# jzebedee/deltaq

Hardware: AMD Instinct MI355X
Metric: MB of text suffix-sorted per second (bit-exact SA) (higher is better)
Workload: dtype u8 text / u64 keys / int32 SA; 1 GPU; 256 MiB uniform-random bytes per GPU (splitmix64 seed 0x5EED0003+rank), int32 SA; bytes_per_gpu=268435456, residency=text and SA resident in HBM, rounds_after_initial_sort=1

## Files before the change

### deltaq_amd/csrc/dq_flags.h

```cpp
#pragma once

#include <algorithm>
#include <cstdint>
#include <cstdlib>
#include <cstring>
#include <optional>
#include <string>

namespace dq {

struct Flags {
    bool debug = false;
    std::optional<int> trace;
    std::optional<int> hip_device;
    std::optional<int> numa_bind;
    std::optional<std::string> fault;
    std::optional<int> small_n;
    std::optional<int> no_many;
    std::optional<int> mid_many_min;
    std::optional<int> no_large_many;
    std::optional<int> large_many_min;
    std::optional<int> no_diff_many;
    std::optional<int> no_diff_mid_many;
    std::optional<int> diff_mid_many_min;
    std::optional<int> no_diff_large;
    std::optional<int> diff_large_min;
    std::optional<int> diff_large_table;
    std::optional<int> no_index_many;
    std::optional<int> index_many_min;
    std::optional<int> index_many_threads;
    std::optional<int> no_index_large;
    std::optional<int> index_large_min;
    std::optional<int> no_check_many;
    std::optional<int> no_bwt_many;
    std::optional<int> no_mtf_many;
    std::optional<int> no_huff_many;
    std::optional<int> mtf_short_max;
    std::optional<int> unbz2_one_start;
    bool no_list_buffers = false;
    bool text_copy = false;
    bool assume_doubled = false;
    bool no_twins = false;
    bool no_period_hint = false;
    std::optional<int> xcd_group;
    std::optional<int> packed;
    std::optional<int> key_bytes;
    std::optional<int> coded;
    std::optional<int> split;
    bool no_bucket = false;
    std::optional<int> bucket;
    std::optional<int> bucket_keybits;
    std::optional<int> bucket_ext;
    std::optional<int> bucket_tile;
    std::optional<int> bucket_slots;
    std::optional<int> slot_finish;
    std::optional<int> tie_settle;
    std::optional<int> status_zero;
    std::optional<int> hist_loads;
    bool old_first_pass = false;
    bool no_fused_ties = false;
    std::optional<int> sparse;
    std::optional<int> binned_isa;
    bool no_binned_isa = false;
    std::optional<int> runs;
    bool no_small = false;
    bool no_wide_small = false;
    bool no_first_small = false;
    std::optional<int> mid_groups;
    bool no_l_shift = false;
    bool no_upd_words = false;
    std::optional<int> upd_bin;
    std::optional<int> upd_bin_min;
    std::optional<int> upd_window;
    std::optional<int> chain_steps;
    bool no_chain = false;
    bool force_rshift = false;
    std::optional<int> tail_max;
    std::optional<int> pair_chains;
    std::optional<int> pair_chains_min;
    std::optional<int> pair_maxg;
    std::optional<int> late_runs_min;
    bool no_late_runs = false;
    std::optional<int> run_period;
    bool search_wave = false;
    std::optional<int> search_ptab;
    bool no_wave_windows = false;
    bool no_poll = false;
    bool no_second_stage = false;
    std::optional<int> win_min;
    std::optional<int> win_second;
    std::optional<int> walk_on;
    bool no_resume = false;
    std::optional<int> scan_device;
    std::optional<int> scan_groups;
    std::optional<int> scan_groups_cap;
    std::optional<int> scan_chains;
    std::optional<int64_t> scan_min_seg;
    std::optional<int64_t> scan_extra;
    std::optional<int64_t> scan_lane_budget;
    std::optional<int> scan_poll_sleep;
    std::optional<int> scan_spin_log2;
    std::optional<int> scan_slow_group;
    std::optional<int> scan_par_emit;
    std::optional<int64_t> frame_follow_min;
    bool frame_after = false;
};

inline Flags read_flags()
{
    auto on = [](const char *name) { return getenv(name) != nullptr; };
    auto num = [](const char *name, int lo = INT32_MIN, int hi = INT32_MAX) -> std::optional<int> {
        const char *v = getenv(name);
        if (!v) return std::nullopt;
        return std::max(lo, std::min(hi, atoi(v)));
    };
    auto num64 = [](const char *name, int64_t lo) -> std::optional<int64_t> {
        const char *v = getenv(name);
        if (!v) return std::nullopt;
        return std::max<int64_t>(lo, atoll(v));
    };
    Flags f;
    const char *gate = getenv("DQ_DEBUG_FLAGS");
    f.debug = gate && atoi(gate) != 0;
    f.trace = num("DQ_TRACE");
    f.hip_device = num("DQ_HIP_DEVICE");
    f.numa_bind = num("DQ_NUMA_BIND");
    if (!f.debug) return f;

    if (const char *v = getenv("DQ_FAULT")) f.fault = v;
    f.small_n = num("DQ_SMALL_N", 0);
    f.no_many = num("DQ_NO_MANY", 0, 15);
    f.mid_many_min = num("DQ_MID_MANY_MIN", 1);
    f.no_large_many = num("DQ_NO_LARGE_MANY", 0, 1);
    f.large_many_min = num("DQ_LARGE_MANY_MIN", 1);
    f.no_diff_many = num("DQ_NO_DIFF_MANY", 0, 1);
    f.no_diff_mid_many = num("DQ_NO_DIFF_MID_MANY", 0, 1);
    f.diff_mid_many_min = num("DQ_DIFF_MID_MANY_MIN", 1);
    f.no_diff_large = num("DQ_NO_DIFF_LARGE", 0, 1);
    f.diff_large_min = num("DQ_DIFF_LARGE_MIN", 1);
    f.diff_large_table = num("DQ_DIFF_LARGE_TABLE", 0, 1);
    f.no_index_many = num("DQ_NO_INDEX_MANY", 0, 1);
    f.index_many_min = num("DQ_INDEX_MANY_MIN", 1);
    f.index_many_threads = num("DQ_INDEX_MANY_THREADS");
    f.no_index_large = num("DQ_NO_INDEX_LARGE", 0, 1);
    f.index_large_min = num("DQ_INDEX_LARGE_MIN", 1);
    f.no_check_many = num("DQ_NO_CHECK_MANY", 0, 1);
    f.no_bwt_many = num("DQ_NO_BWT_MANY", 0, 1);
    f.no_mtf_many = num("DQ_NO_MTF_MANY", 0, 1);
    f.no_huff_many = num("DQ_NO_HUFF_MANY", 0, 1);
    f.mtf_short_max = num("DQ_MTF_SHORT_MAX", 0);
    f.unbz2_one_start = num("DQ_UNBZ2_ONE_START", 0, 1);
    f.no_list_buffers = on("DQ_NO_LIST_BUFFERS");
    f.text_copy = on("DQ_TEXT_COPY");
    f.assume_doubled = on("DQ_ASSUME_DOUBLED");
    f.no_twins = on("DQ_NO_TWINS");
    f.no_period_hint = on("DQ_NO_PERIOD_HINT");

    f.xcd_group = num("DQ_XCD_GROUP", 0, 64);
    f.packed = num("DQ_PACKED");
    f.key_bytes = num("DQ_KEY_BYTES", 1, 8);
    f.coded = num("DQ_CODED");
    f.split = num("DQ_SPLIT");
    f.no_bucket = on("DQ_NO_BUCKET");
    f.bucket = num("DQ_BUCKET");
    f.bucket_keybits = num("DQ_BUCKET_KEYBITS");
    f.bucket_ext = num("DQ_BUCKET_EXT");
    f.bucket_tile = num("DQ_BUCKET_TILE", 0, 1);
    f.bucket_slots = num("DQ_BUCKET_SLOTS", 0, 1);
    f.slot_finish = num("DQ_SLOT_FINISH", 0, 1);
    f.tie_settle = num("DQ_TIE_SETTLE", 0, 1);
    f.status_zero = num("DQ_STATUS_ZERO", 0, 1);
    f.hist_loads = num("DQ_HIST_LOADS", 1, 4);
    f.old_first_pass = on("DQ_OLD_FIRST_PASS");
    f.no_fused_ties = on("DQ_NO_FUSED_TIES");
    f.sparse = num("DQ_SPARSE");
    f.binned_isa = num("DQ_BINNED_ISA");
    f.no_binned_isa = on("DQ_NO_BINNED_ISA");
    f.runs = num("DQ_RUNS");

    f.no_small = on("DQ_NO_SMALL");
    f.no_wide_small = on("DQ_NO_WIDE_SMALL");
    f.no_first_small = on("DQ_NO_FIRST_SMALL");
    f.mid_groups = num("DQ_MID_GROUPS");
    f.no_l_shift = on("DQ_NO_L_SHIFT");
    f.no_upd_words = on("DQ_NO_UPD_WORDS");
    f.upd_bin = num("DQ_UPD_BIN", 0, 2);
    f.upd_bin_min = num("DQ_UPD_BIN_MIN", 1);
    f.upd_window = num("DQ_UPD_WINDOW");
    f.chain_steps = num("DQ_CHAIN_STEPS");
    f.no_chain = on("DQ_NO_CHAIN");
    f.force_rshift = on("DQ_FORCE_RSHIFT");

    f.tail_max = num("DQ_TAIL_MAX", 0);
    f.pair_chains = num("DQ_PAIR_CHAINS");
    f.pair_chains_min = num("DQ_PAIR_CHAINS_MIN", 1);
    f.pair_maxg = num("DQ_PAIR_MAXG", 2);
    f.late_runs_min = num("DQ_LATE_RUNS_MIN", 1);
    f.no_late_runs = on("DQ_NO_LATE_RUNS");
    f.run_period = num("DQ_RUN_PERIOD", 1);

    f.search_wave = on("DQ_SEARCH_WAVE");
    f.search_ptab = num("DQ_SEARCH_PTAB");
    f.no_wave_windows = on("DQ_NO_WAVE_WINDOWS");
    f.no_poll = on("DQ_NO_POLL");
    f.no_second_stage = on("DQ_NO_SECOND_STAGE");
    f.win_min = num("DQ_WIN_MIN", 16);
    f.win_second = num("DQ_WIN_SECOND", 16);
    f.walk_on = num("DQ_WALK_ON");
    f.no_resume = on("DQ_NO_RESUME");

    f.scan_device = num("DQ_SCAN_DEVICE");
    f.scan_groups = num("DQ_SCAN_GROUPS", 8);
    f.scan_groups_cap = num("DQ_SCAN_GROUPS_CAP", 0);
    f.scan_chains = num("DQ_SCAN_CHAINS", 1);
    f.scan_min_seg = num64("DQ_SCAN_MIN_SEG", 64);
    f.scan_extra = num64("DQ_SCAN_EXTRA", 1);
    f.scan_lane_budget = num64("DQ_SCAN_LANE_BUDGET", 1);
    f.scan_poll_sleep = num("DQ_SCAN_POLL_SLEEP", 1, 32);
    f.scan_spin_log2 = num("DQ_SCAN_SPIN_LOG2", 1, 24);
    f.scan_slow_group = num("DQ_SCAN_SLOW_GROUP", 0, 255);
    f.scan_par_emit = num("DQ_SCAN_PAR_EMIT");
    f.frame_follow_min = num64("DQ_FRAME_FOLLOW_MIN", INT64_MIN);
    f.frame_after = on("DQ_FRAME_AFTER");
    return f;
}

struct FaultPlan {
    int alloc_at = 0, hip_at = 0;
    int alloc_seen = 0, hip_seen = 0;
    bool spin = false;
};
inline thread_local FaultPlan t_fault;

inline FaultPlan parse_fault(const std::optional<std::string> &spec)
{
    FaultPlan p;
    if (!spec) return p;
    const char *f = spec->c_str();
    if (strncmp(f, "alloc:", 6) == 0) p.alloc_at = std::max(1, atoi(f + 6));
    else if (strncmp(f, "hip:", 4) == 0) p.hip_at = std::max(1, atoi(f + 4));
    else if (strcmp(f, "spin") == 0) p.spin = true;
    return p;
}

struct FlagState {
    Flags snap;
    int depth = 0;
};
inline thread_local FlagState t_flags;

struct EnvScope {
    EnvScope()
    {
        if (t_flags.depth++ != 0) return;
        t_flags.snap = read_flags();
        t_fault = parse_fault(t_flags.snap.fault);
    }
    explicit EnvScope(const Flags &adopt)
    {
        if (t_flags.depth++ == 0) t_flags.snap = adopt;
    }
    ~EnvScope() { if (--t_flags.depth == 0) t_fault = FaultPlan{}; }
    EnvScope(const EnvScope &) = delete;
    EnvScope &operator=(const EnvScope &) = delete;
};

inline const Flags &flags()
{
    if (t_flags.depth == 0) t_flags.snap = read_flags();
    return t_flags.snap;
}

template <typename Fn>
auto with_flags(Fn fn)
{
    return [snap = flags(), fn = std::move(fn)](auto &&...args) mutable {
        EnvScope scope(snap);
        return fn(std::forward<decltype(args)>(args)...);
    };
}

}
```

### deltaq_amd/csrc/dq_onesweep.h

```cpp
#pragma once
#include "dq_coded_keys.h"
#include "dq_radix.h"
#include "dq_round0_plan.h"

namespace dq {

constexpr int kHistBlocks = 512;
constexpr int kHistThreads = 1024;
constexpr int kMaxPasses = 8;


template <int kPasses>
__global__ __launch_bounds__(kHistThreads) void radix_hist_kernel(const uint64_t *__restrict__ keys,
                                                            int64_t m, unsigned long long *__restrict__ acc ,
                                                            int shift0 = 0 )
{
    __shared__ uint32_t hist[kPasses][kRadixSize * 4];
    const int tid = threadIdx.x;
    const int lane = lane_id();
    const int sub = tid & 3;
    for (int i = tid; i < kPasses * kRadixSize * 4; i += kHistThreads) (&hist[0][0])[i] = 0;
    __syncthreads();

    const int64_t pairs = m >> 1;
    const ulonglong2 *k2 = reinterpret_cast<const ulonglong2 *>(keys);
    for (int64_t i0 = (int64_t)blockIdx.x * kHistThreads + (tid & ~(kWave - 1)); i0 < pairs;
         i0 += (int64_t)gridDim.x * kHistThreads) {
        const int64_t i = i0 + lane;
        const bool ok = i < pairs;
        const bool full = (i0 + kWave) <= pairs;
        ulonglong2 v;
        v.x = 0; v.y = 0;
        if (ok) v = k2[i];
#pragma unroll
        for (int p = 0; p < kPasses; ++p) {
#pragma unroll
            for (int h = 0; h < 2; ++h) {
                const uint32_t d = digit_of(h ? v.y : v.x, shift0 + p * kRadixBits);
                const uint32_t d0 = __builtin_amdgcn_readfirstlane(d);
                if (full && __all(d == d0)) {
                    if (lane == 0) atomicAdd(&hist[p][d0 << 2], (uint32_t)kWave);
                } else if (ok) {
                    atomicAdd(&hist[p][(d << 2) | sub], 1u);
                }
            }
        }
    }
    if ((m & 1) && blockIdx.x == 0 && tid == 0) {
        const uint64_t k = keys[m - 1];
        for (int p = 0; p < kPasses; ++p) atomicAdd(&hist[p][digit_of(k, shift0 + p * kRadixBits) << 2], 1u);
    }
    __syncthreads();
    for (int i = tid; i < kPasses * kRadixSize; i += kHistThreads) {
        const uint32_t *h4 = &(&hist[0][0])[i * 4];
        const uint32_t c = h4[0] + h4[1] + h4[2] + h4[3];
        if (c) atomicAdd(&acc[i], (unsigned long long)c);
    }
}

static __global__ __launch_bounds__(kHistThreads) void text_coded_hist_kernel(const uint32_t *__restrict__ t32, int64_t n,
                                                                       const uint16_t *__restrict__ codetab,
                                                                       unsigned long long *__restrict__ acc )
{
    __shared__ uint32_t hist[kMaxPasses][kRadixSize * 4];
    __shared__ uint16_t ctab[256];
    const int tid = threadIdx.x;
    const int sub = tid & 3;
    for (int i = tid; i < kMaxPasses * kRadixSize * 4; i += kHistThreads) (&hist[0][0])[i] = 0;
    if (tid < 256) ctab[tid] = codetab[tid];
    __syncthreads();
    const int64_t quads = (n + 3) >> 2;
    for (int64_t q = (int64_t)blockIdx.x * kHistThreads + tid; q < quads; q += (int64_t)gridDim.x * kHistThreads) {
        uint32_t tw[5];
#pragma unroll
        for (int c = 0; c < 5; ++c) tw[c] = t32[q + c];
        uint64_t key[4];
        coded_keys4(tw, ctab, key);
        const int cnt = (n - q * 4) < 4 ? (int)(n - q * 4) : 4;
#pragma unroll
        for (int c = 0; c < 4; ++c) {
            if (c < cnt) {
#pragma unroll
                for (int p = 0; p < kMaxPasses; ++p)
                    atomicAdd(&hist[p][(digit_of(key[c], p * kRadixBits) << 2) | sub], 1u);
            }
        }
    }
    __syncthreads();
    for (int i = tid; i < kMaxPasses * kRadixSize; i += kHistThreads) {
        const uint32_t *h4 = &(&hist[0][0])[i * 4];
        const uint32_t c = h4[0] + h4[1] + h4[2] + h4[3];
        if (c) atomicAdd(&acc[i], (unsigned long long)c);
    }
}

constexpr int kHistScanThreads = kRadixSize;
static __global__ __launch_bounds__(kHistScanThreads) void radix_hist_scan_kernel(const unsigned long long *__restrict__ acc,
                                                                           int64_t *__restrict__ digit_offset)
{
    __shared__ int64_t tmp[kHistScanThreads / kWave];
    const int p = blockIdx.x, d = threadIdx.x;
    int64_t total;
    digit_offset[p * kRadixSize + d] = block_excl_sum((int64_t)acc[p * kRadixSize + d], tmp, &total);
}

template <typename StatusT> struct StatusBits;
template <> struct StatusBits<uint32_t> {
    static constexpr uint32_t kAgg = 1u << 30, kPrefix = 2u << 30, kMask = (1u << 30) - 1;
};
template <> struct StatusBits<uint64_t> {
    static constexpr uint64_t kAgg = 1ull << 62, kPrefix = 2ull << 62, kMask = (1ull << 62) - 1;
};

template <typename StatusT>
__device__ __forceinline__ void status_store(StatusT *p, StatusT v)
{
    __hip_atomic_store(p, v, __ATOMIC_RELAXED, __HIP_MEMORY_SCOPE_AGENT);
}
template <typename StatusT>
__device__ __forceinline__ StatusT status_load(StatusT *p)
{
    return __hip_atomic_load(p, __ATOMIC_RELAXED, __HIP_MEMORY_SCOPE_AGENT);
}

struct OnesweepCtl {
    uint32_t ticket;
    uint32_t error;
};

enum OnesweepMode { kPairs = 0, kText = 1, kTextPacked = 2, kKeys = 3, kKeysLast = 4, kKeysLastTies = 5, kTextPackedExt = 6, kKeysExt = 7 };
constexpr uint64_t kSeamEmpty = ~0ull;

#ifndef DQ_PHASE
#define DQ_PHASE(i) do { } while (0)
#endif

template <typename IdxT, typename StatusT, int kItems, int kMode, int kMinWaves, int kThreads = kBlock,
          bool kEarlyVals = false, bool kLdsMatch = true, int kExchRounds = 1, bool kAtomicBase = false,
          bool kCoded = false, typename ValT = IdxT>
__global__ __launch_bounds__(kThreads, kMinWaves) void radix_rank_kernel(
    const uint64_t *__restrict__ kin, const ValT *__restrict__ vin,
    uint64_t *__restrict__ kout, ValT *__restrict__ vout, int64_t m, int shift, int keybits, int ib,
    const int64_t *__restrict__ digit_offset ,
    StatusT *__restrict__ status , OnesweepCtl *__restrict__ ctl,
    int64_t *__restrict__ sticky_error, uint32_t *__restrict__ ebits = nullptr,
    uint64_t *__restrict__ seam_tab  = nullptr,
    const uint16_t *__restrict__ codetab  = nullptr,
    int xcd_group = 0 ,
    uint32_t spin_limit = kSpinLimit )
{
    constexpr bool kFromText = (kMode == kText || kMode == kTextPacked || kMode == kTextPackedExt);
    constexpr bool kPackedText = (kMode == kTextPacked || kMode == kTextPackedExt);
    static_assert(!kCoded || kMode == kText, "coded keys: first pass of the pair sort only");
    constexpr bool kAtomicRank = kAtomicBase && kPackedText;
    constexpr bool kTies = (kMode == kKeysLastTies);
    constexpr bool kHasVals = (kMode == kPairs || kMode == kText || kMode == kTextPackedExt || kMode == kKeysExt);
    static_assert((kMode != kTextPackedExt && kMode != kKeysExt) || sizeof(ValT) == 1, "the extra key bits travel as bytes");
    static_assert(!kFromText || (kItems % 4) == 0, "text mode packs 4 suffixes per lane");
    static_assert(kThreads % kRadixSize == 0, "threads 0..255 own one digit each");
    constexpr int kWavesB = kThreads / kWave;
    constexpr int kTileN = kThreads * kItems;
    constexpr int kWaveN = kWave * kItems;
    using SB = StatusBits<StatusT>;

    static_assert(kItems % kExchRounds == 0, "exchange rounds split the items evenly");
    constexpr int kExchN = kTileN / kExchRounds;
    __shared__ __attribute__((aligned(16))) uint64_t exch[kExchN];
    __shared__ uint32_t whist[kWavesB][kRadixSize];
    __shared__ uint32_t tile_base[kRadixSize];
    __shared__ IdxT gofs[kRadixSize];
    __shared__ uint32_t wtmp[kRadixSize / kWave];
    __shared__ uint32_t s_tile;
    __shared__ uint16_t ctab[kCoded ? 256 : 1];

    const int tid = threadIdx.x;
    const int w = tid >> 6;
    const int lane = lane_id();
    if (kCoded && tid < 256) ctab[tid] = codetab[tid];

    if (kAtomicBase) {
        if (tid == 0) {
            uint32_t t = blockIdx.x;
            if (xcd_group > 0) {
                const uint32_t grp = 8u * (uint32_t)xcd_group, g = t / grp, r = t % grp;
                if ((g + 1) * grp <= gridDim.x) t = g * grp + (r & 7u) * (uint32_t)xcd_group + (r >> 3);
            }
            s_tile = t;
        }
    } else if (tid == 0) {
        const uint32_t t = atomicAdd(&ctl->ticket, 1u);
        s_tile = t;
    }
    for (int i = tid; i < kWavesB * kRadixSize; i += kThreads) (&whist[0][0])[i] = 0;
    if (kLdsMatch && !kAtomicRank) {
        static_assert(kExchN >= kWavesB * kRadixSize, "exchange buffer must hold the match tables");
        for (int i = tid; i < kWavesB * kRadixSize; i += kThreads) exch[i] = 0;
    }
    __syncthreads();
    DQ_PHASE(0);
    const int64_t tile = s_tile;
    const int64_t base = tile * kTileN;
    const int valid = (m - base) < kTileN ? (int)(m - base) : kTileN;
    const int wbase = w * kWaveN + lane;

    auto elem = [&](int k) -> int {
        return kFromText ? ((k >> 2) * kThreads + tid) * 4 + (k & 3) : wbase + k * kWave;
    };

    uint64_t key[kItems];
    ValT val[kItems];
    uint32_t vpack[kMode == kTextPackedExt ? kItems / 4 : 1];
    auto val_of = [&](int k) -> ValT {
        if (kMode == kTextPackedExt) return (ValT)((vpack[k >> 2] >> (8 * (k & 3))) & 0xffu);
        return val[k];
    };
    if (kFromText) {
        const uint32_t *t32 = reinterpret_cast<const uint32_t *>(kin);
        const int kshift = 64 - keybits;
#pragma unroll
        for (int j = 0; j < kItems / 4; ++j) {
            const int e0 = (j * kThreads + tid) * 4;
            if (kCoded) {
                if (e0 < valid) {
                    const int64_t qd = (base + e0) >> 2;
                    uint32_t tw[5];
#pragma unroll
                    for (int c = 0; c < 5; ++c) tw[c] = t32[qd + c];
                    coded_keys4(tw, ctab, &key[4 * j]);
                } else {
#pragma unroll
                    for (int c = 0; c < 4; ++c) key[4 * j + c] = ~0ull;
                }
            } else if (e0 < valid) {
                const int64_t qd = (base + e0) >> 2;
                const uint32_t w0 = t32[qd], w1 = t32[qd + 1], w2 = t32[qd + 2];
                const uint64_t x = __builtin_bswap64((uint64_t)w0 | ((uint64_t)w1 << 32));
                const uint64_t y = (uint64_t)__builtin_bswap32(w2) << 32;
                const uint64_t x4[4] = {x, (x << 8) | (y >> 56), (x << 16) | (y >> 48), (x << 24) | (y >> 40)};
                if (kMode == kTextPackedExt) vpack[j] = 0;
#pragma unroll
                for (int c = 0; c < 4; ++c) {
                    key[4 * j + c] = x4[c] >> kshift;
                    if (kMode == kTextPackedExt) vpack[j] |= (uint32_t)((x4[c] >> (kshift - 8)) & 0xffu) << (8 * c);
                }
                if (kPackedText) {
#pragma unroll
                    for (int c = 0; c < 4; ++c)
                        key[4 * j + c] = (key[4 * j + c] << ib) | (uint64_t)(base + e0 + c);
                }
            } else {
#pragma unroll
                for (int c = 0; c < 4; ++c) key[4 * j + c] = ~0ull;
                if (kMode == kTextPackedExt) vpack[j] = 0;
            }
        }
    } else if (valid == kTileN) {
#pragma unroll
        for (int k = 0; k < kItems; ++k) key[k] = kin[base + wbase + k * kWave];
    } else {
#pragma unroll
        for (int k = 0; k < kItems; ++k) {
            const int e = wbase + k * kWave;
            key[k] = e < valid ? kin[base + e] : ~0ull;
        }
    }

    auto load_vals = [&]() {
        if (!kHasVals || kMode == kTextPackedExt) {
        } else if (kMode == kText) {
#pragma unroll
            for (int k = 0; k < kItems; ++k) val[k] = (ValT)(base + elem(k));
        } else if (valid == kTileN) {
#pragma unroll
            for (int k = 0; k < kItems; ++k) val[k] = vin[base + wbase + k * kWave];
        } else {
#pragma unroll
            for (int k = 0; k < kItems; ++k) {
                const int e = wbase + k * kWave;
                val[k] = e < valid ? vin[base + e] : (ValT)0;
            }
        }
    };
    if (kEarlyVals) load_vals();
    if (kMode == kPairs || kMode == kKeysExt) { asm volatile("" :: "v"(key[kItems - 1])); }
    DQ_PHASE(1);

    uint32_t pos[kItems];
    uint32_t *myhist = whist[w];
    unsigned long long *mtab = reinterpret_cast<unsigned long long *>(exch) + w * kRadixSize;
    const unsigned long long lanebit = 1ull << lane;
    auto peers_of = [&](uint32_t d) -> uint64_t {
        if (kLdsMatch) {
            __hip_atomic_fetch_or(&mtab[d], lanebit, __ATOMIC_RELAXED, __HIP_MEMORY_SCOPE_WORKGROUP);
            return __hip_atomic_load(&mtab[d], __ATOMIC_RELAXED, __HIP_MEMORY_SCOPE_WORKGROUP);
        }
        return match_digit8(d);
    };
    (void)lanebit;
    if (kAtomicRank) {
#pragma unroll
        for (int k = 0; k < kItems; ++k) {
            const uint32_t d = digit_of(key[k], shift);
            pos[k] = atomicAdd(&whist[0][d], elem(k) < valid ? 1u : 0u);
        }
    } else if (valid == kTileN) {
#pragma unroll
        for (int k = 0; k < kItems; ++k) {
            const uint32_t d = digit_of(key[k], shift);
            const bool uni = kLdsMatch && __all(d == (uint32_t)__builtin_amdgcn_readfirstlane(d));
            const uint64_t peers = uni ? ~0ull : peers_of(d);
            const uint32_t before = myhist[d];
            const int r = mask_rank_lt(peers);
            if (r == 0) {
                myhist[d] = before + (uint32_t)__popcll(peers);
                if (kLdsMatch && !uni) mtab[d] = 0;
            }
            pos[k] = before + (uint32_t)r;
        }
    } else {
#pragma unroll
        for (int k = 0; k < kItems; ++k) {
            const bool ok = elem(k) < valid;
            const uint32_t d = digit_of(key[k], shift);
            pos[k] = 0;
            if (kLdsMatch) {
                if (ok) {
                    const uint64_t peers = peers_of(d);
                    const uint32_t before = myhist[d];
                    const int r = mask_rank_lt(peers);
                    if (r == 0) { myhist[d] = before + (uint32_t)__popcll(peers); mtab[d] = 0; }
                    pos[k] = before + (uint32_t)r;
                }
            } else {
                const uint64_t peers = match_digit8(d) & __ballot(ok);
                if (ok) {
                    const uint32_t before = myhist[d];
                    const int r = mask_rank_lt(peers);
                    if (r == 0) myhist[d] = before + (uint32_t)__popcll(peers);
                    pos[k] = before + (uint32_t)r;
                }
            }
        }
    }
    if (kLdsMatch && !kAtomicRank) __syncthreads();
    DQ_PHASE(2);
    if (!kEarlyVals) load_vals();
    __syncthreads();
    DQ_PHASE(3);

    constexpr int kLookWin = 8;
    uint32_t tot = 0, incl = 0;
    StatusT sw[kLookWin];
    unsigned long long abase = 0;
    StatusT *mine = status + tile * kRadixSize + (tid & (kRadixSize - 1));
    if (tid < kRadixSize) {
#pragma unroll
        for (int i = 0; i < kWavesB; ++i) {
            const uint32_t c = whist[i][tid];
            whist[i][tid] = tot;
            tot += c;
        }
        if (kAtomicBase) {
            abase = atomicAdd(reinterpret_cast<unsigned long long *>(status) + tid, (unsigned long long)tot);
        } else {
        if (tile == 0) status_store<StatusT>(mine, SB::kPrefix | (StatusT)tot);
        else status_store<StatusT>(mine, SB::kAgg | (StatusT)tot);
#pragma unroll
        for (int j = 0; j < kLookWin; ++j)
            sw[j] = (tile - 1 - j >= 0) ? status_load<StatusT>(status + (tile - 1 - j) * kRadixSize + tid)
                                        : SB::kPrefix;
        }
        incl = wave_incl_sum(tot);
        if (lane == kWave - 1) wtmp[w] = incl;
    }
    __syncthreads();
    uint32_t excl_tile = 0;
    if (tid < kRadixSize) {
        uint32_t off = 0;
#pragma unroll
        for (int i = 0; i < kRadixSize / kWave; ++i) if (i < w) off += wtmp[i];
        excl_tile = off + incl - tot;
        tile_base[tid] = excl_tile;
    }
    __syncthreads();
    DQ_PHASE(4);

#pragma unroll
    for (int k = 0; k < kItems; ++k) {
        const uint32_t d = digit_of(key[k], shift);
        pos[k] += kAtomicRank ? tile_base[d] : tile_base[d] + myhist[d];
    }
    if (valid != kTileN) {
#pragma unroll
        for (int k = 0; k < kItems; ++k)
            if (elem(k) >= valid) pos[k] = 0xffffffffu;
    }
    uint64_t skey[kItems];
#pragma unroll
    for (int r = 0; r < kExchRounds; ++r) {
        if (r > 0) __syncthreads();
#pragma unroll
        for (int k = 0; k < kItems; ++k) {
            const uint32_t p = pos[k] - (uint32_t)(r * kExchN);
            if (p < (uint32_t)kExchN) exch[p] = key[k];
        }
        __syncthreads();
#pragma unroll
        for (int k = r * (kItems / kExchRounds); k < (r + 1) * (kItems / kExchRounds); ++k)
            skey[k] = exch[k * kThreads + tid - r * kExchN];
    }
    ValT sval[kItems];
    if (kHasVals) {
        constexpr int kValN = kExchN * (int)(sizeof(uint64_t) / sizeof(ValT));
        constexpr int kValRounds = kTileN / kValN > 0 ? kTileN / kValN : 1;
        constexpr int kValCap = kTileN / kValRounds;
        ValT *exv = reinterpret_cast<ValT *>(exch);
#pragma unroll
        for (int r = 0; r < kValRounds; ++r) {
            __syncthreads();
#pragma unroll
            for (int k = 0; k < kItems; ++k) {
                const uint32_t p = pos[k] - (uint32_t)(r * kValCap);
                if (p < (uint32_t)kValCap) exv[p] = val_of(k);
            }
            __syncthreads();
#pragma unroll
            for (int k = r * (kItems / kValRounds); k < (r + 1) * (kItems / kValRounds); ++k)
                sval[k] = exv[k * kThreads + tid - r * kValCap];
        }
    }
    DQ_PHASE(5);

    if (tid < kRadixSize) {
        StatusT excl = 0;
        if (kAtomicBase) {
            excl = (StatusT)abase;
        } else if (tile > 0) {
            int64_t t = tile - 1;
            uint32_t spins = 0;
            bool done = false;
            {
                int used = 0;
#pragma unroll
                for (int j = 0; j < kLookWin; ++j) {
                    if (!done && used == j) {
                        if (sw[j] & SB::kPrefix) { excl += sw[j] & SB::kMask; done = true; }
                        else if (sw[j] & SB::kAgg) { excl += sw[j] & SB::kMask; used = j + 1; }
                    }
                }
                t -= used;
            }
            constexpr int kLookWin2 = 8;
            while (!done) {
                StatusT s2[kLookWin2];
#pragma unroll
                for (int j = 0; j < kLookWin2; ++j)
                    s2[j] = (t - j >= 0) ? status_load<StatusT>(status + (t - j) * kRadixSize + tid) : SB::kPrefix;
                int used = 0;
#pragma unroll
                for (int j = 0; j < kLookWin2; ++j) {
                    if (!done && used == j) {
                        if (s2[j] & SB::kPrefix) { excl += s2[j] & SB::kMask; done = true; }
                        else if (s2[j] & SB::kAgg) { excl += s2[j] & SB::kMask; used = j + 1; }
                    }
                }
                t -= used;
                if (!done && used == 0) {
                    __builtin_amdgcn_s_sleep(1);
                    if (++spins > spin_limit) { atomicExch(&ctl->error, 1u); *sticky_error = 1; break; }
                }
            }
            status_store<StatusT>(mine, SB::kPrefix | (StatusT)(excl + tot));
        }
        gofs[tid] = (IdxT)(digit_offset[tid] + (int64_t)excl) - (IdxT)excl_tile;
    }
    __syncthreads();
    DQ_PHASE(6);

    if (kTies) {
        uint64_t *edge = exch;
        uint64_t *run_first = exch + kItems * kWavesB;
        uint64_t *run_last = run_first + kRadixSize;
        static_assert(kExchN >= kItems * kWavesB + 2 * kRadixSize, "exchange buffer holds the seam staging");
        if (lane == kWave - 1) {
#pragma unroll
            for (int k = 0; k < kItems; ++k) edge[k * kWavesB + w] = skey[k];
        }
        if (tid < kRadixSize) { run_first[tid] = kSeamEmpty; run_last[tid] = kSeamEmpty; }
        __syncthreads();
        const uint64_t smask = (1ull << ib) - 1;
        static_assert(kItems <= kWave, "one lane per item");
        uint64_t eprev = 0;
        if (lane < kItems) {
            if (w > 0) eprev = edge[lane * kWavesB + w - 1];
            else if (lane > 0) eprev = edge[(lane - 1) * kWavesB + kWavesB - 1];
        }
#pragma unroll
        for (int k = 0; k < kItems; ++k) {
            const int q = k * kThreads + tid;
            const uint32_t plo = (uint32_t)__builtin_amdgcn_update_dpp(0, (int)(uint32_t)skey[k], 0x138, 0xf, 0xf, false);
            const uint32_t phi = (uint32_t)__builtin_amdgcn_update_dpp(0, (int)(uint32_t)(skey[k] >> 32), 0x138, 0xf, 0xf, false);
            uint64_t prev = ((uint64_t)phi << 32) | plo;
            const uint64_t e0 = ((uint64_t)(uint32_t)__builtin_amdgcn_readlane((int)(uint32_t)(eprev >> 32), k) << 32) |
                                (uint32_t)__builtin_amdgcn_readlane((int)(uint32_t)eprev, k);
            if (lane == 0) prev = e0;
            if (q < valid) {
                const uint32_t d = digit_of(skey[k], shift);
                const IdxT o = gofs[d] + (IdxT)q;
                const bool hasprev = q > 0;
                if (hasprev && ((skey[k] ^ prev) >> ib) == 0)
                    atomicOr(&ebits[(uint64_t)o >> 5], 1u << ((uint32_t)o & 31u));
                const uint32_t dp = digit_of(prev, shift);
                if (!hasprev || dp != d) {
                    run_first[d] = skey[k];
                    if (hasprev) run_last[dp] = prev;
                }
                if (q == valid - 1) run_last[d] = skey[k];
                vout[o] = (ValT)(skey[k] & smask);
            }
        }
        __syncthreads();
        if (tid < kRadixSize) {
            seam_tab[(tile * kRadixSize + tid) * 2] = run_first[tid];
            seam_tab[(tile * kRadixSize + tid) * 2 + 1] = run_last[tid];
        }
    } else {
#pragma unroll
    for (int k = 0; k < kItems; ++k) {
        const int q = k * kThreads + tid;
        if (q < valid) {
            const IdxT o = gofs[digit_of(skey[k], shift)] + (IdxT)q;
            kout[o] = skey[k];
            if (kHasVals) vout[o] = sval[k];
            if (kMode == kKeysLast) vout[o] = (ValT)(skey[k] & ((1ull << ib) - 1));
        }
    }
    }
    DQ_PHASE(7);
}

constexpr int kKgramBits = 32768;

__device__ __forceinline__ void sample_kgrams(const uint8_t *__restrict__ text, int64_t n,
                                              unsigned long long *__restrict__ coll, uint32_t *seen ,
                                              uint32_t *cnt)
{
    constexpr int kPer = kKgramSamples / kBlock;
    const int t = threadIdx.x;
    for (int i = t; i < 8 * kKgramBits / 32; i += kBlock) seen[i] = 0;
    if (t < 8) cnt[t] = 0;
    uint64_t key[kPer];
#pragma unroll
    for (int q = 0; q < kPer; ++q) {
        const int64_t p = (int64_t)((__int128)(q * kBlock + t) * n / kKgramSamples);
        uint64_t k = 0;
#pragma unroll
        for (int b = 0; b < 8; ++b) k = (k << 8) | (p + b < n ? (uint64_t)text[p + b] : 0ull);
        key[q] = k;
    }
    __syncthreads();
#pragma unroll
    for (int q = 0; q < kPer; ++q) {
#pragma unroll
        for (int L = 1; L <= 8; ++L) {
            uint64_t x = (key[q] >> (64 - 8 * L)) + 0x9E3779B97F4A7C15ull * (uint64_t)L;
            x = (x ^ (x >> 30)) * 0xBF58476D1CE4E5B9ull;
            x = (x ^ (x >> 27)) * 0x94D049BB133111EBull;
            const uint32_t bit = (uint32_t)(x >> 40) & (kKgramBits - 1);
            const uint32_t old = atomicOr(&seen[(L - 1) * (kKgramBits / 32) + (bit >> 5)], 1u << (bit & 31));
            if (old & (1u << (bit & 31))) atomicAdd(&cnt[L - 1], 1u);
        }
    }
    __syncthreads();
    if (t < 8) coll[t] = (unsigned long long)cnt[t];
}

template <int kLoads>
static __global__ __launch_bounds__(kBlock) void text_hist_kernel(const uint8_t *__restrict__ text, int64_t n,
                                                           unsigned long long *__restrict__ bytehist ,
                                                           unsigned long long *__restrict__ kgram_coll = nullptr,
                                                           uint8_t *__restrict__ copy_out = nullptr ,
                                                           unsigned long long *__restrict__ xcd_hist = nullptr )
{
    static_assert(kBlock == kHistGroupThreads, "hist_chunk() counts in workgroups of kBlock threads");
    __shared__ uint32_t hist[kRadixSize * 4];
    if (kgram_coll && blockIdx.x == 0) {
        __shared__ uint32_t s_seen[8 * kKgramBits / 32];
        sample_kgrams(text, n, kgram_coll, s_seen, hist);
        return;
    }
    const int tid = threadIdx.x;
    const int sub = tid & 3;
    const HistSpan sp = hist_span(n, (int64_t)blockIdx.x - (kgram_coll ? 1 : 0), (int64_t)gridDim.x - (kgram_coll ? 1 : 0),
                                  xcd_hist != nullptr);
    for (int i = tid; i < kRadixSize * 4; i += kBlock) hist[i] = 0;
    __syncthreads();
    const uint4 *t16 = reinterpret_cast<const uint4 *>(text);
    const int64_t chunks = n >> 4;
    bool long_run = false;
    unsigned long long flat_chunks = 0;
    uint4 *o16 = reinterpret_cast<uint4 *>(copy_out);
    auto count = [&](const uint4 &v) {
        const uint32_t wds[4] = {v.x, v.y, v.z, v.w};
        const bool flat = v.x == v.y && v.y == v.z && v.z == v.w && v.x == (v.x & 0xffu) * 0x01010101u;
        const uint64_t fb = __ballot(flat);
        long_run |= (fb & (fb >> 1) & (fb >> 2) & (fb >> 3)) != 0;
        flat_chunks += (unsigned long long)__popcll(fb);
#pragma unroll
        for (int j = 0; j < 4; ++j) {
#pragma unroll
            for (int b = 0; b < 4; ++b) atomicAdd(&hist[(((wds[j] >> (8 * b)) & 0xff) << 2) | sub], 1u);
        }
    };
    const int64_t stride = hist_stride(sp);
    int64_t trip = 0;
    if constexpr (kLoads > 1) {
        const int64_t wave_last = hist_chunk(sp, tid | (kWave - 1), 0);
        for (; wave_last + (trip + kLoads - 1) * stride < sp.c1; trip += kLoads) {
            uint4 v[kLoads];
#pragma unroll
            for (int q = 0; q < kLoads; ++q) v[q] = t16[hist_chunk(sp, tid, trip + q)];
#pragma unroll
            for (int q = 0; q < kLoads; ++q) {
                if (copy_out) o16[hist_chunk(sp, tid, trip + q)] = v[q];
                count(v[q]);
            }
        }
    }
    for (int64_t i = hist_chunk(sp, tid, trip); i < sp.c1; i += stride) {
        const uint4 v = t16[i];
        if (copy_out) o16[i] = v;
        count(v);
    }
    if (sp.member == 0 && sp.eighth == 0) {
        for (int64_t i = (chunks << 4) + tid; i < n; i += kBlock) {
            const uint8_t b = text[i];
            if (copy_out) copy_out[i] = b;
            atomicAdd(&hist[((uint32_t)b << 2) | sub], 1u);
            if (xcd_hist) {
                atomicAdd(&xcd_hist[(i / xcd_eighth(n)) * kRadixSize + b], 1ull);
                atomicAdd(&xcd_hist[b], ~0ull);
            }
        }
    }
    __syncthreads();
    const uint32_t c = hist[tid * 4] + hist[tid * 4 + 1] + hist[tid * 4 + 2] + hist[tid * 4 + 3];
    if (c) {
        atomicAdd(&bytehist[tid], (unsigned long long)c);
        if (xcd_hist) atomicAdd(&xcd_hist[sp.eighth * kRadixSize + tid], (unsigned long long)c);
    }
    if (kgram_coll && long_run && lane_id() == 0) atomicOr(&kgram_coll[8], 1ull);
    if (kgram_coll && flat_chunks && lane_id() == 0) atomicAdd(&kgram_coll[9], flat_chunks);
}

__device__ __forceinline__ void text_digit_offsets_body(int p, const int64_t *__restrict__ bytehist, const uint8_t *__restrict__ text,
                                                        int64_t n, int kb, int64_t *__restrict__ digit_offset,
                                                        const int64_t *__restrict__ xcd_hist, int64_t *__restrict__ sub_offset)
{
    __shared__ int64_t tmp[kWavesPerBlock];
    const int d = threadIdx.x;
    const int64_t off = kb - 1 - p;
    const int64_t lead = off < n ? off : n;
    int64_t c = bytehist[d];
    for (int64_t j = 0; j < lead; ++j) c -= (text[j] == d);
    if (d == 0) c += lead;
    int64_t total;
    const int64_t excl = block_excl_sum(c, tmp, &total);
    digit_offset[p * kRadixSize + d] = excl;
    if (sub_offset && p == 0) {
        const int64_t E = xcd_eighth(n);
        int64_t run = excl;
        for (int e = 0; e < kXcds; ++e) {
            sub_offset[e * kRadixSize + d] = run;
            const int64_t s0 = (int64_t)e * E;
            if (s0 >= n) continue;
            const int64_t s1 = std::min(s0 + E, n);
            int64_t ce = xcd_hist[e * kRadixSize + d];
            for (int64_t j = s0; j < std::min(s0 + off, s1); ++j) ce -= (text[j] == d);
            for (int64_t j = std::max(s0 + off, s1); j < s1 + off; ++j) ce += j < n ? (text[j] == d) : (d == 0);
            run += ce;
        }
    }
}

static __global__ __launch_bounds__(kBlock) void text_digit_offsets_kernel(const int64_t *__restrict__ bytehist,
                                                                    const uint8_t *__restrict__ text,
                                                                    int64_t n, int kb,
                                                                    int64_t *__restrict__ digit_offset,
                                                                    const int64_t *__restrict__ xcd_hist = nullptr ,
                                                                    int64_t *__restrict__ sub_offset = nullptr )
{
    text_digit_offsets_body(blockIdx.x, bytehist, text, n, kb, digit_offset, xcd_hist, sub_offset);
}

struct ZeroRanges {
    uint4 *at[3] = {nullptr, nullptr, nullptr};
    int64_t units[3] = {0, 0, 0};
    bool set(int r, void *p, size_t bytes)
    {
        at[r] = reinterpret_cast<uint4 *>(p);
        units[r] = (int64_t)((bytes + 15) / 16);
        return (reinterpret_cast<uintptr_t>(p) & 15) == 0;
    }
    int64_t total() const { return units[0] + units[1] + units[2]; }
};
static __global__ __launch_bounds__(kBlock) void zero_ranges_kernel(ZeroRanges r)
{
    const uint4 zero = {0u, 0u, 0u, 0u};
    const int64_t stride = (int64_t)gridDim.x * kBlock;
#pragma unroll
    for (int k = 0; k < 3; ++k) {
        uint4 *const p = r.at[k];
        for (int64_t i = (int64_t)blockIdx.x * kBlock + threadIdx.x; i < r.units[k]; i += stride) p[i] = zero;
    }
}

}
```

### deltaq_amd/csrc/dq_round0.h

```cpp
#pragma once
#include "dq_sort_passes.h"
#include "dq_alpha_code.h"
#include "dq_ties.h"
#include "dq_bucket_sort.h"
#include "dq_xcd_rank.h"
#include "dq_slot_rank.h"
#include "dq_slot_finish.h"

namespace dq {
namespace {

constexpr int64_t kSgShortList = 1 << 20;
inline int mid_group_cap(int64_t list_len)
{
    if (const std::optional<int> g = flags().mid_groups) {
        return *g >= 1024 ? 1024 : *g >= 512 ? 512 : *g >= 256 ? 256 : 0;
    }
    return list_len >= kSgShortList ? 512 : 1024;
}
inline bool small_round_usable(int64_t n, int64_t mm, bool third_list_buffer)
{
    const Flags &F = flags();
    return !F.no_small && n < (1ll << 32) && (mm * 2 <= n || (third_list_buffer && !F.no_wide_small));
}

template <typename Fn>
int with_bool(bool on, Fn fn)
{
    return on ? fn(std::true_type{}) : fn(std::false_type{});
}

constexpr int kXcdHistAt = kRadixSize + 16;

template <typename IdxT>
struct Round0Out {
    uint64_t *Kr[2] = {nullptr, nullptr};
    IdxT *Vr[2] = {nullptr, nullptr};
    int64_t m = 0, h = 0;
    int rbits = 0;
    bool dense_built = false;
    bool fin_done = false;
    int64_t fin_cap = 0, fin_left = 0;
    bool shallow_ties = false, keys_ready = false, list_ungrouped = false;
    const uint32_t *first_rank32 = nullptr;
    RunPlan runs;
};

template <typename IdxT>
struct Round0 {
    DeviceCtx &c;
    hipStream_t st;
    Workspace<IdxT> &w;
    int64_t n;
    IdxT *d_sa;
    Launcher &L;
    const uint8_t *text_src;
    int period_hint;
    Round0Out<IdxT> &o;

    static constexpr int64_t wb = (int64_t)sizeof(IdxT);
    TextStats s;
    KeyPlan k;
    Round0Route route;
    int ib = 0;
    bool coded = false;
    uint64_t *K[2] = {w.K0, w.K1};
    IdxT *V[2] = {nullptr, nullptr};

    const uint64_t *text64() const { return reinterpret_cast<const uint64_t *>(w.text); }
    int64_t tie_words() const { return (n + 63) / 64; }

    int digit_tables(int kb, bool coded_keys)
    {
        if (coded_keys) {
            const int hblocks = (int)std::min<int64_t>(kHistBlocks, ((n >> 2) + kHistThreads - 1) / kHistThreads + 1);
            DQ_TRY(L.begin(DQ_K_RADIX_HIST, n, n));
            HIP_TRY(hipMemsetAsync(w.hist_partial, 0, (size_t)kMaxPasses * kRadixSize * 8, st));
            hipLaunchKernelGGL(text_coded_hist_kernel, dim3(hblocks), dim3(kHistThreads), 0, st,
                               reinterpret_cast<const uint32_t *>(w.text), n, (const uint16_t *)w.codetab,
                               reinterpret_cast<unsigned long long *>(w.hist_partial));
            hipLaunchKernelGGL(radix_hist_scan_kernel, dim3(kMaxPasses), dim3(kHistScanThreads), 0, st,
                               (const unsigned long long *)w.hist_partial, w.digit_offset);
            HIP_TRY(hipGetLastError());
            return L.end();
        }
        hipLaunchKernelGGL(text_digit_offsets_kernel, dim3(kb), dim3(kBlock), 0, st,
                           (const int64_t *)w.bytehist, (const uint8_t *)w.text, n, kb, w.digit_offset);
        HIP_TRY(hipGetLastError());
        return DQ_OK;
    }

    int prepare()
    {
        int blocks = (int)std::min<int64_t>(1024, ((n >> 4) + kBlock - 1) / kBlock + 1);
        unsigned long long *xcd_hist = n >= kRound0MinN ? reinterpret_cast<unsigned long long *>(w.bytehist + kXcdHistAt) : nullptr;
        if (xcd_hist) blocks = (blocks + kXcds - 1) / kXcds * kXcds;
        HIP_TRY(hipMemsetAsync(w.bytehist, 0, (size_t)(kXcdHistAt + (xcd_hist ? kXcds * kRadixSize : 0)) * 8, L.st));
        LAUNCH(L, DQ_K_TEXT_HIST, n, n,
               hipLaunchKernelGGL(flags().hist_loads.value_or(kHistLoads) < kHistLoads ? text_hist_kernel<1> : text_hist_kernel<kHistLoads>,
                                  dim3(blocks + 1), dim3(kBlock), 0, L.st,
                                  text_src ? text_src : (const uint8_t *)w.text, n, reinterpret_cast<unsigned long long *>(w.bytehist),
                                  reinterpret_cast<unsigned long long *>(w.bytehist + 256), text_src ? w.text : (uint8_t *)nullptr,
                                  xcd_hist));
        HIP_TRY(hipMemcpyAsync(c.pinned, w.bytehist, (256 + 10) * 8, hipMemcpyDeviceToHost, L.st));
        HIP_TRY(hipEventRecord(c.readback, L.st));
        const Flags &F = flags();
        const int early = early_status_passes(n, F);
        DQ_TRY(prepare_status<IdxT>(L, w, n, early));
        if (n >= kRound0MinN) {
            ZeroRanges z;
            bool aligned = z.set(0, w.Vb, (size_t)(tie_words() + 1) * 8);
            if (early == 0) aligned = z.set(1, w.ctl_status, sizeof(XcdRankCtl)) && aligned;
            aligned = z.set(2, w.hist_partial, sizeof(SlotRankCtl)) && aligned;
            if (!aligned || sizeof(XcdRankCtl) > w.ctl_status_bytes) return fail(DQ_ERR_HIP, "preamble ranges misplaced");
            hipLaunchKernelGGL(zero_ranges_kernel, dim3((unsigned)std::min<int64_t>((z.total() + kBlock - 1) / kBlock, 2048)), dim3(kBlock),
                               0, L.st, z);
            HIP_TRY(hipGetLastError());
        }
        HIP_TRY(hipEventSynchronize(c.readback));
        s = TextStats(c.pinned, n);
        ib = s.ib;
        k = choose_key_bytes(s, F);
        bool hist_deferred = false;
        if (coded_keys_tried(s, F, k)) {
            AlphaCode code;
            if (build_alpha_code(s.hist, &code) && (code.avg_len <= kCodedMaxAvgLen || F.coded)) {
                uint16_t *stage = reinterpret_cast<uint16_t *>(c.pinned + 512);
                memcpy(stage, code.tab, sizeof(code.tab));
                HIP_TRY(hipMemcpyAsync(w.codetab, stage, sizeof(code.tab), hipMemcpyHostToDevice, L.st));
                coded = true;
                hist_deferred = split_round0_wanted(n, k, (int)wb, F);
                if (F.trace) fprintf(stderr, "[dq] coded round 0: %d symbols, %.2f bits per byte\n", code.sigma, code.avg_len);
            }
        }
        route = plan_round0_route(s, F, k, coded, (int)wb, slot_span_words_of(w));
        if (early > 0) DQ_TRY(prepare_status<IdxT>(L, w, n, k.kb, early));
        else DQ_TRY(prepare_status<IdxT>(L, w, n, route.slots ? (route.b.xcd_pass ? 0 : 1) : std::max(k.kb, kEarlyPasses)));
        if (hist_deferred) return DQ_OK;
        if (route.b.applies) return DQ_OK;
        return digit_tables(k.kb, coded);
    }

    int passes(int &cur, uint32_t *ebits = nullptr, uint64_t *seam_tab = nullptr)
    {
        const int kb = k.kb;
        if (k.packed) {
            DQ_TRY(rank_pass<IdxT, kTextPacked>(L, w, text64(), (const IdxT *)nullptr, K[1], (IdxT *)nullptr, n, 0, kb, ib));
            cur = 1;
            for (int p = 1; p < kb; ++p) {
                if (p == kb - 1 && ebits)
                    DQ_TRY(rank_pass<IdxT, kKeysLastTies>(L, w, K[cur], (const IdxT *)nullptr, (uint64_t *)nullptr, d_sa, n, p,
                                                          kb, ib, ebits, seam_tab));
                else if (p == kb - 1)
                    DQ_TRY(rank_pass<IdxT, kKeysLast>(L, w, K[cur], (const IdxT *)nullptr, K[cur ^ 1], d_sa, n, p, kb, ib));
                else
                    DQ_TRY(rank_pass<IdxT, kKeys>(L, w, K[cur], (const IdxT *)nullptr, K[cur ^ 1], (IdxT *)nullptr, n, p, kb, ib));
                cur ^= 1;
            }
            return DQ_OK;
        }
        DQ_TRY(with_bool(coded, [&](auto kCoded) -> int {
            return rank_pass<IdxT, kText, decltype(kCoded)::value>(L, w, text64(), (const IdxT *)nullptr, K[1], V[1], n, 0, kb);
        }));
        cur = 1;
        for (int p = 1; p < kb; ++p) {
            DQ_TRY(rank_pass<IdxT, kPairs>(L, w, K[cur], V[cur], K[cur ^ 1], V[cur ^ 1], n, p, kb));
            cur ^= 1;
        }
        return DQ_OK;
    }

    int collect_ties(uint32_t *ebits, const uint64_t *seam_tab, uint64_t *act_rank, bool *overflow, uint64_t *fin_rank,
                     bool seams = true, int64_t h_fin = -1, bool settle = false)
    {
        if (settle) {
            TieCounters *tctr = reinterpret_cast<TieCounters *>(w.totals + 6);
            unsigned long long *listed = reinterpret_cast<unsigned long long *>(w.totals + 3);
            const int64_t tile = (int64_t)kSettleThreads * kSettleWords;
            const int64_t groups = std::min<int64_t>((tie_words() + tile - 1) / tile, (int64_t)std::max(c.ncu, 1) * 6);
            o.fin_cap = n;
            LAUNCH(L, DQ_K_TIE_COLLECT, n, n / 8,
                   hipLaunchKernelGGL(tie_settle_kernel<IdxT>, dim3((unsigned)groups), dim3(kSettleThreads), 0, L.st,
                                      reinterpret_cast<const uint64_t *>(ebits), tie_words(), n, d_sa, (const uint8_t *)w.text,
                                      h_fin >= 0 ? h_fin : (int64_t)k.kb, act_rank, w.Va, o.fin_cap, tctr, listed));
            DQ_TRY(read_totals<IdxT>(L, c, w, 64, "radix look-back timed out (device spin bound hit)"));
            o.m = c.pinned[6];
            o.fin_left = c.pinned[3];
            *overflow = c.pinned[7] != 0 || o.fin_left > o.fin_cap;
            if (flags().trace)
                fprintf(stderr, "[dq] ties settled from their bits: %lld tied suffixes, %lld of them listed (n=%lld)\n", (long long)o.m,
                        (long long)o.fin_left, (long long)n);
            if (*overflow && flags().trace) fprintf(stderr, "[dq] tie / bucket overflow flags: %lld\n", (long long)c.pinned[7]);
            return DQ_OK;
        }
        using Cfg = RankCfg<IdxT, kKeysLastTies>;
        using CfgS = RankCfg<IdxT, kKeysLastTies, true>;
        const int64_t tile_keys = small_tiles(n) ? CfgS::kThreads * CfgS::kItems : Cfg::kThreads * Cfg::kItems;
        const int64_t ntiles = (n + tile_keys - 1) / tile_keys;
        const int pass = k.kb - 1;
        char *area = w.ctl_status + (size_t)pass * w.ctl_status_stride;
        const int64_t *dofs = w.digit_offset + pass * kRadixSize;
        TieCounters *ctr = reinterpret_cast<TieCounters *>(w.totals + 6);
        if (seams) {
            HIP_TRY(hipMemsetAsync(ctr, 0, sizeof(TieCounters), L.st));
            const unsigned sg = (unsigned)((ntiles * kRadixSize + kBlock - 1) / kBlock);
            DQ_TRY(with_status_word(n, [&](auto word) -> int {
                LAUNCH(L, DQ_K_TIE_SEAM, ntiles * kRadixSize, ntiles * kRadixSize * (16 + (int64_t)sizeof(uint64_t)),
                       hipLaunchKernelGGL(tie_seam_kernel<decltype(word)>, dim3(sg), dim3(kBlock), 0, L.st, seam_tab, ntiles, ib, dofs,
                                          reinterpret_cast<const decltype(word) *>(area + 256), ebits));
                return DQ_OK;
            }));
        }
        LAUNCH(L, DQ_K_TIE_COLLECT, n, n / 8,
               hipLaunchKernelGGL(tie_collect_kernel<IdxT>, dim3((unsigned)((tie_words() + kTieThreads - 1) / kTieThreads)),
                                  dim3(kTieThreads), 0, L.st, reinterpret_cast<const uint64_t *>(ebits), tie_words(), n, (const IdxT *)d_sa,
                                  act_rank, w.Va, ctr));
        unsigned long long *left_over = reinterpret_cast<unsigned long long *>(w.totals + 3);
        o.fin_cap = n / 8;
        LAUNCH(L, DQ_K_SMALL_FINISH, o.fin_cap, 0,
               hipLaunchKernelGGL((small_group_finish_kernel<IdxT, 8, 32>),
                                  dim3((unsigned)std::min<int64_t>((o.fin_cap + kFinishThreads - 1) / kFinishThreads, 256 * 16)),
                                  dim3(kFinishThreads), 0, L.st, (const uint64_t *)act_rank, (const IdxT *)w.Va, (const uint8_t *)w.text,
                                  o.fin_cap, n, h_fin >= 0 ? h_fin : (int64_t)k.kb, d_sa, fin_rank, w.Vb, left_over,
                                  (const unsigned long long *)&ctr->count));
        DQ_TRY(read_totals<IdxT>(L, c, w, 64, "radix look-back timed out (device spin bound hit)"));
        o.m = c.pinned[6];
        *overflow = c.pinned[7] != 0;
        if (*overflow && flags().trace) fprintf(stderr, "[dq] tie / bucket overflow flags: %lld\n", (long long)c.pinned[7]);
        o.fin_left = c.pinned[3];
        if (L.active && !c.pending.empty() && c.pending.back().cat == DQ_K_SMALL_FINISH) {
            const int64_t cnt = std::min<int64_t>(o.m, o.fin_cap);
            c.pending.back().elems = cnt;
            c.pending.back().bytes = cnt * (8 + wb + 64 + wb);
        }
        return DQ_OK;
    }

    int build_isa_binned(uint64_t *keys, uint64_t *P0, int kshift0)
    {
        const int64_t ntiles = (n + kSegFusedTile - 1) / kSegFusedTile;
        const size_t need = 256 + (size_t)3 * ntiles * 8;
        if (need > w.seg_status_bytes) return fail(DQ_ERR_HIP, "seg status buffer too small");
        HIP_TRY(hipMemsetAsync(w.seg_status, 0, need, st));
        const bool rank32_direct = sizeof(IdxT) == 4 && !o.runs.runs_wanted && mid_group_cap(n) > 0;
        const bool third = w.X != nullptr;
        uint32_t *list_rank = (small_round_usable(n, 0, third) && !flags().no_first_small)
                                  ? (rank32_direct ? w.RL : reinterpret_cast<uint32_t *>(w.Vb)) : nullptr;
        LAUNCH(L, DQ_K_SEG_FUSED, n, n * (8 + wb + 8),
               hipLaunchKernelGGL((seg_fused_kernel<IdxT, true, false, false, true>), dim3((unsigned)ntiles),
                                  dim3(kSegThreads), 0, st, (const uint64_t *)keys, (const IdxT *)d_sa, n, ib, kshift0,
                                  d_sa, w.ISA, P0, w.Va, reinterpret_cast<uint64_t *>(w.seg_status + 256), ntiles,
                                  reinterpret_cast<SegCtl *>(w.seg_status), w.totals, w.totals + 1, 0, list_rank, 0, spin_bound()));
        const int rc = read_totals<IdxT>(L, c, w, 16, "device look-back timed out (spin bound hit)");
        o.m = c.pinned[0];
        DQ_TRY(rc);
        DQ_TRY(isa_from_suffix_words<IdxT>(L, c, w, n, ib, k.kb, P0, keys));
        if (list_rank && o.m == 0) return DQ_OK;
        if (list_rank && small_round_usable(n, o.m, third) && rank32_direct) {
            o.first_rank32 = list_rank;
            return DQ_OK;
        }
        if (list_rank && small_round_usable(n, o.m, third)) {
            LAUNCH(L, DQ_K_KEY2_FROM_PAIRS, o.m, o.m * 12,
                   hipLaunchKernelGGL(widen_ranks_kernel, dim3(grid_for(o.m)), dim3(kBlock), 0, st,
                                      (const uint32_t *)list_rank, o.m, keys));
            return DQ_OK;
        }
        const bool with_key2 = !o.runs.runs_wanted;
        const int kbits = bit_length((uint64_t)(n - 1) + (uint64_t)k.kb);
        unsigned long long *cnt = reinterpret_cast<unsigned long long *>(w.totals + 3);
        HIP_TRY(hipMemsetAsync(cnt, 0, 8, st));
        const int64_t per = (int64_t)kPairThreads * kPairItems;
        LAUNCH(L, DQ_K_KEY2_FROM_PAIRS, n, n * 8 + o.m * (wb + 8 + wb),
               hipLaunchKernelGGL(key2_from_pairs_kernel<IdxT>, dim3((unsigned)((n + per - 1) / per)), dim3(kPairThreads),
                                  0, st, (const uint64_t *)P0, n, ib, (const IdxT *)w.ISA, (int64_t)k.kb, kbits, with_key2,
                                  keys, w.Va, cnt));
        o.keys_ready = with_key2;
        o.list_ungrouped = true;
        return DQ_OK;
    }

    int bucketed(bool *done)
    {
        *done = false;
        const Flags &F = flags();
        const BucketPlan &b = route.b;
        if (!b.applies) return DQ_OK;
        const int kb = k.kb, keybits = b.keybits, lowbits = b.lowbits;
        const SlotPlan &sp = route.sp;
        const FinishTiles &ft = route.ft;
        static_assert(sizeof(SlotRankCtl) <= (size_t)kHistBlocks * kMaxPasses * kRadixSize * 4, "the cursors live in the histogram scratch");
        const bool slots = route.slots;
        uint32_t *slot_base = reinterpret_cast<uint32_t *>(w.bkt_bounds), *slot_out = slot_base + kSlotBuckets + 4;
        SlotRankCtl *sctl = reinterpret_cast<SlotRankCtl *>(w.hist_partial);
        const int first = slots ? 0 : 1;
        uint8_t *E[2] = {reinterpret_cast<uint8_t *>(w.Va), reinterpret_cast<uint8_t *>(w.Va) + align_up((size_t)n)};
        uint32_t *ebits = reinterpret_cast<uint32_t *>(w.Vb);
        TieCounters *ctr = reinterpret_cast<TieCounters *>(w.totals + 6);
        BucketFlags *bflags = reinterpret_cast<BucketFlags *>(&ctr->overflow);
        const int64_t *xcd_hist = b.xcd_pass ? (const int64_t *)(w.bytehist + kXcdHistAt) : nullptr;
        int64_t *sub_offset = b.xcd_pass ? w.xcd_offset : nullptr;
        if (slots) {
            if (F.trace)
                fprintf(stderr, "[dq] second pass into bucket slots: %d x %d slots of %lld words (n=%lld)\n", sp.first, sp.second,
                        (long long)b.X, (long long)n);
            hipLaunchKernelGGL(slot_setup_kernel, dim3(b.bbytes + kRadixSize + 1), dim3(kBlock), 0, st, (const int64_t *)w.bytehist,
                               (const uint8_t *)w.text, n, b.bbytes, w.digit_offset, xcd_hist, sub_offset, b.X, slot_base);
        } else {
            hipLaunchKernelGGL(text_digit_offsets_kernel, dim3(b.bbytes), dim3(kBlock), 0, st, (const int64_t *)w.bytehist,
                               (const uint8_t *)w.text, n, b.bbytes, w.digit_offset, xcd_hist, sub_offset);
        }
        HIP_TRY(hipGetLastError());
        if (c.ncu <= 0) {
            int v = 0;
            c.ncu = hipDeviceGetAttribute(&v, hipDeviceAttributeMultiprocessorCount, c.dev) == hipSuccess && v > 0 ? v : 256;
        }
        if (b.xcd_pass) {
            if (F.trace) fprintf(stderr, "[dq] XCD-local first pass (n=%lld, eighths of %lld)\n", (long long)n, (long long)xcd_eighth(n));
            if (sizeof(XcdRankCtl) > w.ctl_status_stride) return fail(DQ_ERR_HIP, "status buffer too small");
            LAUNCH(L, DQ_K_RADIX_RANK, n, n * (1 + 8),
                   hipLaunchKernelGGL(xcd_text_rank_kernel, dim3((unsigned)std::min<int64_t>(c.ncu, (n + kXcdTileN - 1) / kXcdTileN)),
                                      dim3(kXcdRankThreads), 0, st, reinterpret_cast<const uint32_t *>(w.text), K[first], n,
                                      ib + lowbits, keybits, ib, (const int64_t *)w.xcd_offset,
                                      reinterpret_cast<XcdRankCtl *>(w.ctl_status)));
        } else {
            DQ_TRY(b.ext ? rank_pass_ext<IdxT, kTextPackedExt>(L, w, text64(), (const uint8_t *)nullptr, K[1], E[1], n, 0, ib, ib + lowbits, keybits)
                       : rank_pass<IdxT, kTextPacked>(L, w, text64(), (const IdxT *)nullptr, K[first], (IdxT *)nullptr, n, 0, kb, ib,
                                                      nullptr, nullptr, ib + lowbits, keybits));
        }
        if (slots) {
            const int groups = resident_groups(&c.slot_rank_groups, (const void *)slot_rank_kernel, kSlotRankThreads, c.dev);
            LAUNCH(L, DQ_K_RADIX_RANK, n, n * 16,
                   hipLaunchKernelGGL(slot_rank_kernel, dim3((unsigned)std::min<int64_t>(groups, (n + kSlotTileN - 1) / kSlotTileN)),
                                      dim3(kSlotRankThreads), 0, st, (const uint64_t *)K[0], K[1], n, ib + lowbits + 8, ib + lowbits,
                                      (const int64_t *)w.digit_offset, (const uint32_t *)slot_base, sctl, bflags));
        }
        for (int p = 1; p < b.bbytes && !slots; ++p) {
            DQ_TRY(b.ext ? rank_pass_ext<IdxT, kKeysExt>(L, w, K[p & 1], E[p & 1], K[(p & 1) ^ 1], E[(p & 1) ^ 1], n, p, ib, ib + lowbits + 8 * p, keybits)
                       : rank_pass<IdxT, kKeys>(L, w, K[p & 1], (const IdxT *)nullptr, K[(p & 1) ^ 1], (IdxT *)nullptr, n, p, kb, ib,
                                                nullptr, nullptr, ib + lowbits + 8 * p, keybits));
        }
        uint64_t *Ks = slots ? K[1] : K[b.bbytes & 1], *Kfree = slots ? K[0] : K[(b.bbytes & 1) ^ 1];
        const uint8_t *Es = b.ext ? E[b.bbytes & 1] : nullptr;
        if (F.trace)
            fprintf(stderr, "[dq] bucket finish: %s geometry, %lld tiles of up to %lld words cut every %lld %s (n=%lld)\n", ft.fine ? "fine" : "coarse",
                    (long long)ft.ntiles, (long long)ft.cap, (long long)(ft.by_id ? ft.g : ft.Cf), ft.by_id ? "buckets" : "words", (long long)n);
        if ((size_t)ft.ntiles + 1 > finish_bounds_entries(n)) return fail(DQ_ERR_HIP, "tile bounds buffer too small");
        if (slots) {
            LAUNCH(L, DQ_K_BUCKET_SORT, ft.ntiles, ft.ntiles * 16,
                   hipLaunchKernelGGL(slot_out_kernel, dim3(kRadixSize), dim3(kSlotOutThreads), 0, st, sctl->cursor, (uint32_t)b.X,
                                      (const int64_t *)(w.digit_offset + kRadixSize) , n, slot_out, bflags));
            const bool one_exchange = F.slot_finish.value_or(1) != 0 && lowbits <= kSfMaxLowbits && b.X <= kSfCap;
            if (F.trace)
                fprintf(stderr, "[dq] slot finish: %s (n=%lld)\n", one_exchange ? "slot_finish_kernel, one LDS exchange" : "bucket_sort_kernel, two LDS exchanges", (long long)n);
            if (one_exchange) {
                auto kernel = slot_finish_kernel<IdxT>;
                const int groups = resident_groups(&c.slot_finish_groups[sizeof(IdxT) == 8], (const void *)kernel, kSfThreads, c.dev);
                LAUNCH(L, DQ_K_BUCKET_SORT, n, n * (8 + wb) + n / 8,
                       hipLaunchKernelGGL(kernel, dim3((unsigned)std::min<int64_t>(ft.ntiles, groups)), dim3(kSfThreads), 0, st,
                                          (const uint64_t *)Ks, ib, lowbits, ft.ntiles, d_sa, ebits, bflags,
                                          (const uint32_t *)slot_base, (const uint32_t *)sctl->cursor, (const uint32_t *)slot_out));
            } else {
                auto kernel = bucket_sort_kernel<IdxT, false, BktFine, true>;
                const int groups = resident_groups(&c.bkt_slot_groups[sizeof(IdxT) == 8], (const void *)kernel, BktFine::threads, c.dev);
                LAUNCH(L, DQ_K_BUCKET_SORT, n, n * (8 + wb) + n / 8,
                       hipLaunchKernelGGL(kernel, dim3((unsigned)std::min<int64_t>(ft.ntiles, groups)), dim3(BktFine::threads), 0, st,
                                          (const uint64_t *)Ks, ib, lowbits, (const int64_t *)nullptr, ft.ntiles, d_sa, ebits, bflags,
                                          (const uint8_t *)nullptr, (const uint32_t *)slot_base, (const uint32_t *)sctl->cursor, (const uint32_t *)slot_out));
            }
        } else if (ft.by_id) {
            const int64_t nbuckets = (int64_t)1 << (8 * b.bbytes);
            LAUNCH(L, DQ_K_BUCKET_SORT, ft.ntiles, ft.ntiles * 16 * 8,
                   hipLaunchKernelGGL(bucket_bounds_by_id_kernel, dim3((unsigned)((nbuckets + 1 + kBlock - 1) / kBlock)), dim3(kBlock), 0,
                                      st, (const uint64_t *)Ks, n, ib + lowbits, ft.g, b.X, nbuckets, ft.ntiles, w.bkt_bounds, bflags));
        } else {
            LAUNCH(L, DQ_K_BUCKET_SORT, ft.ntiles, ft.ntiles * 16 * 8,
                   hipLaunchKernelGGL(bucket_bounds_kernel, dim3((unsigned)((ft.ntiles + 1 + kBlock - 1) / kBlock)), dim3(kBlock), 0,
                                      st, (const uint64_t *)Ks, n, ib + lowbits, ft.Cf, b.X, ft.ntiles, w.bkt_bounds, bflags));
        }
        auto finish = [&](auto kExt, auto geometry) -> int {
            using G = decltype(geometry);
            auto kernel = bucket_sort_kernel<IdxT, decltype(kExt)::value, G>;
            const int groups = resident_groups(&c.bkt_groups[ft.fine][b.ext][sizeof(IdxT) == 8], (const void *)kernel, G::threads, c.dev);
            LAUNCH(L, DQ_K_BUCKET_SORT, n, n * ((b.ext ? 9 : 8) + wb) + n / 8,
                   hipLaunchKernelGGL(kernel, dim3((unsigned)std::min<int64_t>(ft.ntiles, groups)), dim3(G::threads), 0, st,
                                      (const uint64_t *)Ks, ib, lowbits, (const int64_t *)w.bkt_bounds, ft.ntiles, d_sa, ebits, bflags, Es,
                                      (const uint32_t *)nullptr, (const uint32_t *)nullptr, (const uint32_t *)nullptr));
            return DQ_OK;
        };
        if (slots) {
        } else if (ft.fine) {
            DQ_TRY(finish(std::false_type{}, BktFine{}));
        } else {
            DQ_TRY(with_bool(b.ext, [&](auto kExt) -> int { return finish(kExt, BktCoarse{}); }));
        }
        if (b.ext && F.trace) fprintf(stderr, "[dq] bucketed round 0 with %d + 8 key bits per suffix (n=%lld)\n", keybits, (long long)n);
        bool overflow = false;
        const bool settle = F.tie_settle.value_or(slots ? 1 : 0) != 0;
        DQ_TRY(collect_ties(ebits, nullptr, Kfree, &overflow, Ks, false, b.hb, settle));
        if (overflow) {
            if (F.trace) fprintf(stderr, "[dq] bucketed round 0 gave up (n=%lld): plain digit passes\n", (long long)n);
            DQ_TRY(prepare_status<IdxT>(L, w, n, kMaxPasses));
            HIP_TRY(hipMemsetAsync(w.Vb, 0, (size_t)(tie_words() + 1) * 8, st));
            HIP_TRY(hipMemsetAsync(w.totals, 0, 64, st));
            o.m = 0; o.fin_cap = 0; o.fin_left = 0;
            return digit_tables(kb, false);
        }
        o.fin_done = settle || o.m <= o.fin_cap;
        o.Kr[0] = Kfree; o.Kr[1] = Ks;
        if (settle) {
            o.Kr[0] = Ks; o.Kr[1] = Kfree;
            o.Vr[0] = w.Vb; o.Vr[1] = w.Va;
        }
        o.h = b.hb;
        o.shallow_ties = true;
        *done = true;
        return DQ_OK;
    }

    int split(bool *done)
    {
        *done = false;
        if constexpr (sizeof(IdxT) != 4) {
            return DQ_OK;
        } else {
            if (!w.sp_top || !w.X || !w.RL) return DQ_OK;
            const int64_t cap = std::min<int64_t>(kFinCap, (n + 2) / (kSplitBuckets / 2));
            if (cap < 2) return DQ_OK;
            const uint32_t *t32 = reinterpret_cast<const uint32_t *>(w.text);
            const uint16_t *ctab = (const uint16_t *)w.codetab;
            uint64_t *Ks[2] = {K[0], w.X};
            IdxT *Vs[2] = {w.Vb, w.Xs};
            const int64_t ovf_cap = (n / 2) & ~(int64_t)1;
            uint64_t *ovf_k[2] = {reinterpret_cast<uint64_t *>(w.ISA), K[0]};
            IdxT *ovf_v[2] = {reinterpret_cast<IdxT *>(w.RL), w.Vb};
            const Flags &F = flags();
            const bool dbg = F.trace.value_or(0) >= 2;
            auto phase = [&](const char *what) -> int {
                if (!dbg) return DQ_OK;
                HIP_TRY(hipStreamSynchronize(st));
                fprintf(stderr, "[dq] split round 0: %s done\n", what);
                return DQ_OK;
            };
            const unsigned sgrid = (unsigned)((kSplitSample + kBlock - 1) / kBlock);
            DQ_TRY(with_bool(coded, [&](auto kCoded) -> int {
                LAUNCH(L, DQ_K_SPLIT_AUX, kSplitSample, kSplitSample * ((coded ? 20 : 12) + 8),
                       hipLaunchKernelGGL(sample_keys_kernel<decltype(kCoded)::value>, dim3(sgrid), dim3(kBlock), 0, st, t32, n, ctab, kSplitSample, Ks[0]));
                return DQ_OK;
            }));
            DQ_TRY(phase("sample"));
            int scur = 0;
            DQ_TRY(onesweep_sort_pairs<IdxT>(L, w, Ks, Vs, kSplitSample, 64, scur));
            DQ_TRY(phase("sample sort"));
            HIP_TRY(hipMemsetAsync(w.sp_ctl, 0, sizeof(SplitCtl), st));
            hipLaunchKernelGGL(sample_heavy_kernel, dim3(sgrid), dim3(kBlock), 0, st, (const uint64_t *)Ks[scur], &w.sp_ctl->ovf_count);
            HIP_TRY(hipGetLastError());
            HIP_TRY(hipMemcpyAsync(c.pinned, w.sp_ctl, sizeof(SplitCtl), hipMemcpyDeviceToHost, st));
            HIP_TRY(hipStreamSynchronize(st));
            const int64_t heavy = c.pinned[0];
            if (F.trace)
                fprintf(stderr, "[dq] sample-sort round 0: %.1f %% of the sampled keys are copies of keys too heavy for a bucket%s\n",
                        100.0 * (double)heavy / (double)kSplitSample, heavy * 5 > 2 * kSplitSample ? " -- the digit passes instead" : "");
            if (heavy * 5 > 2 * kSplitSample && F.split.value_or(0) < 2) return DQ_OK;
            HIP_TRY(hipMemsetAsync(w.sp_cursor_b, 0, (size_t)kSplitBuckets * 8, st));
            HIP_TRY(hipMemsetAsync(w.sp_ctl, 0, sizeof(SplitCtl), st));
            const int64_t n_main = n & ~(int64_t)1;
            uint64_t *spill_k = reinterpret_cast<uint64_t *>(d_sa);
            IdxT *spill_v = d_sa + (n / 2 + 1);
            if (n / 8 + 1025 * (int64_t)kSplitTop + 1024 > n / 4) return DQ_OK;
            LAUNCH(L, DQ_K_SPLIT_AUX, kSplitBuckets, (int64_t)kSplitBuckets * 16,
                   hipLaunchKernelGGL(make_splitters_kernel, dim3(kSplitBuckets / kBlock), dim3(kBlock), 0, st, (const uint64_t *)Ks[scur], w.sp_top, w.sp_sub,
                                      w.sp_low, w.sp_pure);
                   hipLaunchKernelGGL(split_estimate_kernel, dim3(1), dim3(kSplitTop), 0, st, (const uint64_t *)Ks[scur], (const uint64_t *)w.sp_top, n, w.sp_off,
                                      w.sp_cursor_a));
            DQ_TRY(phase("splitters, region estimates"));
            const unsigned grid_a = (unsigned)((n + kSplitTileA - 1) / kSplitTileA);
            DQ_TRY(with_bool(coded, [&](auto kCoded) -> int {
                LAUNCH(L, DQ_K_SPLIT_PASS, n, n * (1 + 8 + wb),
                       hipLaunchKernelGGL((split_pass_kernel<IdxT, true, decltype(kCoded)::value>), dim3(grid_a), dim3(kSplitThreads), 0, st, text64(), (const IdxT *)nullptr,
                                          (const uint64_t *)nullptr, (const IdxT *)nullptr, (int64_t)0, n, (const uint64_t *)w.sp_top, w.sp_cursor_a,
                                          (const int64_t *)w.sp_off, (const unsigned long long *)nullptr, (const uint32_t *)w.sp_tile_first, K[1], w.Va, spill_k, spill_v,
                                          n_main, (uint64_t *)nullptr, (IdxT *)nullptr, (int64_t)0, w.sp_ctl, ctab));
                return DQ_OK;
            }));
            DQ_TRY(phase("pass A"));
            const unsigned grid_b = (unsigned)(n / kSplitTileB + kSplitTop);
            LAUNCH(L, DQ_K_SPLIT_PASS, n, n * 2 * (8 + wb),
                   hipLaunchKernelGGL(split_plan_kernel, dim3(1), dim3(kSplitTop), 0, st, (const unsigned long long *)w.sp_cursor_a, (const int64_t *)w.sp_off, w.sp_cnt_a,
                                      w.sp_tile_first, w.sp_ctl);
                   hipLaunchKernelGGL((split_pass_kernel<IdxT, false, false>), dim3(grid_b), dim3(kSplitThreads), 0, st, (const uint64_t *)K[1], (const IdxT *)w.Va,
                                      (const uint64_t *)spill_k, (const IdxT *)spill_v, n_main, n, (const uint64_t *)w.sp_sub, w.sp_cursor_b, (const int64_t *)w.sp_off,
                                      (const unsigned long long *)w.sp_cnt_a, (const uint32_t *)w.sp_tile_first, Ks[0], Vs[0], Ks[1], Vs[1],
                                      cap, ovf_k[0], ovf_v[0], ovf_cap, w.sp_ctl, ctab, (const uint8_t *)w.sp_pure));
            DQ_TRY(phase("pass B"));
            LAUNCH(L, DQ_K_SPLIT_AUX, kSplitBuckets, (int64_t)kSplitBuckets * 36,
                   hipLaunchKernelGGL(bucket_sum_kernel, dim3(kScanBlocks), dim3(kScanThreads), 0, st, (const unsigned long long *)w.sp_cursor_b, cap,
                                      (const uint8_t *)w.sp_pure, w.sp_part);
                   hipLaunchKernelGGL(bucket_scan_kernel, dim3(kScanBlocks), dim3(kScanThreads), 0, st, (const unsigned long long *)w.sp_cursor_b, cap,
                                      (const uint8_t *)w.sp_pure, (const ScanPart *)w.sp_part, w.sp_out_base, w.sp_ovf_src, w.sp_ovf_dst, w.sp_ctl));
            DQ_TRY(phase("bucket scan"));
            const bool two = cap > kFinSmallCap;
            LAUNCH(L, DQ_K_SPLIT_FINISH, n, n * 2 * (8 + wb),
                   if (two || cap <= kFinSmallCap)
                       hipLaunchKernelGGL((bucket_finish_kernel<IdxT, 256, 4>), dim3(kSplitBuckets), dim3(256), 0, st, (const uint64_t *)Ks[0], (const IdxT *)Vs[0],
                                          (const uint64_t *)Ks[1], (const IdxT *)Vs[1], cap, (int64_t)0, (int64_t)kFinSmallCap, !two,
                                          (const unsigned long long *)w.sp_cursor_b, (const int64_t *)w.sp_out_base, K[1], d_sa, ovf_k[0], ovf_v[0], ovf_cap, w.sp_ctl, (const uint8_t *)w.sp_pure);
                   if (cap > kFinSmallCap)
                       hipLaunchKernelGGL((bucket_finish_kernel<IdxT, 256, 8>), dim3(kSplitBuckets), dim3(256), 0, st, (const uint64_t *)Ks[0], (const IdxT *)Vs[0],
                                          (const uint64_t *)Ks[1], (const IdxT *)Vs[1], cap, (int64_t)(two ? kFinSmallCap : 0), (int64_t)kFinCap, true,
                                          (const unsigned long long *)w.sp_cursor_b, (const int64_t *)w.sp_out_base, K[1], d_sa, ovf_k[0], ovf_v[0], ovf_cap, w.sp_ctl, (const uint8_t *)w.sp_pure));
            HIP_TRY(hipMemcpyAsync(c.pinned, w.sp_ctl, sizeof(SplitCtl), hipMemcpyDeviceToHost, st));
            HIP_TRY(hipStreamSynchronize(st));
            const int64_t ovf = c.pinned[0], ovf_buckets = c.pinned[1], npure = c.pinned[4];
            const bool abandon = c.pinned[3] != 0 || ovf + npure > ovf_cap;
            if (flags().trace)
                fprintf(stderr, "[dq] sample-sort round 0 (%s keys, %d buckets of <= %lld): %lld suffixes in %lld oversize buckets, %lld copies of heavy keys placed unsorted%s\n",
                        coded ? "coded" : "raw", kSplitBuckets, (long long)cap, (long long)ovf, (long long)ovf_buckets, (long long)npure,
                        abandon ? " -- overflow lists full, given up" : "");
            if (abandon) return DQ_OK;
            if (npure > 0) {
                LAUNCH(L, DQ_K_SPLIT_AUX, npure, npure * 2 * (8 + wb),
                       hipLaunchKernelGGL(pure_place_kernel<IdxT>, dim3((unsigned)((npure + kBlock - 1) / kBlock)), dim3(kBlock), 0, st, npure, ovf_cap,
                                          (const uint64_t *)ovf_k[0], (const IdxT *)ovf_v[0], (const int64_t *)w.sp_out_base, (const uint64_t *)w.sp_low, K[1], d_sa));
            }
            if (ovf > 0) {
                int xcur = 0;
                DQ_TRY(onesweep_sort_pairs<IdxT>(L, w, ovf_k, ovf_v, ovf, 64, xcur));
                LAUNCH(L, DQ_K_SPLIT_AUX, ovf, ovf * 2 * (8 + wb),
                       hipLaunchKernelGGL(overflow_place_kernel<IdxT>, dim3((unsigned)((ovf + kBlock - 1) / kBlock)), dim3(kBlock), 0, st, ovf, ovf_buckets,
                                          (const int64_t *)w.sp_ovf_src, (const int64_t *)w.sp_ovf_dst,
                                          (const uint64_t *)ovf_k[xcur], (const IdxT *)ovf_v[xcur], K[1], d_sa));
            }
            *done = true;
            return DQ_OK;
        }
    }

    int run()
    {
        const Flags &F = flags();
        int cur = 0;
        DQ_TRY(prepare());
        const int kb = k.kb;
        o.runs = plan_runs(s, F, (int)wb, period_hint);
        V[kb & 1] = d_sa;
        V[(kb & 1) ^ 1] = w.Va;
        o.Vr[0] = w.Va; o.Vr[1] = w.Vb;
        o.rbits = ib;
        o.h = kb;
        bool done = false;
        DQ_TRY(bucketed(&done));
        if (done) return DQ_OK;
        if (fused_ties_wanted(n, k, F)) {
            uint32_t *ebits = reinterpret_cast<uint32_t *>(w.Vb);
            uint64_t *seam_tab = reinterpret_cast<uint64_t *>(reinterpret_cast<char *>(w.Vb) +
                                                              align_up((size_t)(tie_words() + 1) * 8));
            DQ_TRY(passes(cur, ebits, seam_tab));
            bool overflow = false;
            DQ_TRY(collect_ties(ebits, seam_tab, K[cur], &overflow, K[cur ^ 1]));
            o.fin_done = !overflow && o.m <= o.fin_cap;
            if (!overflow) {
                o.Kr[0] = K[cur]; o.Kr[1] = K[cur ^ 1];
                return DQ_OK;
            }
            HIP_TRY(hipMemsetAsync(w.ctl_status + (size_t)(kb - 1) * w.ctl_status_stride, 0, w.ctl_status_stride, st));
            DQ_TRY(rank_pass<IdxT, kKeysLast>(L, w, K[cur ^ 1], (const IdxT *)nullptr, K[cur], d_sa, n, kb - 1, kb, ib));
        } else {
            bool split_done = false;
            const bool split_wanted = split_round0_wanted(n, k, (int)wb, F);
            if (split_wanted && (!o.runs.runs_wanted || F.split)) {
                DQ_TRY(split(&split_done));
            }
            if (split_wanted && !split_done) {
                DQ_TRY(digit_tables(kb, coded));
                DQ_TRY(prepare_status<IdxT>(L, w, n, kb));
            }
            if (split_done) {
                cur = 1;
            } else {
                DQ_TRY(passes(cur));
            }
        }
        const int kshift0 = k.packed ? ib : 0;
        const DenseGuess guess = dense_guess(n, k);
        int64_t tied_pairs = 0;
        if (guess == DenseGuess::kTakeSample) {
            HIP_TRY(hipMemsetAsync(w.totals + 2, 0, 8, st));
            hipLaunchKernelGGL(sample_ties_kernel, dim3(kTieSamples / kBlock), dim3(kBlock), 0, st,
                               (const uint64_t *)K[cur], n, kshift0, kTieSamples, w.totals + 2);
            HIP_TRY(hipGetLastError());
            HIP_TRY(hipMemcpyAsync(c.pinned, w.totals + 2, 8, hipMemcpyDeviceToHost, st));
            HIP_TRY(hipStreamSynchronize(st));
            tied_pairs = c.pinned[0];
        }
        o.dense_built = predict_dense(guess, tied_pairs, F);
        if (o.dense_built && binned_isa_pays(n, F)) {
            o.Kr[0] = K[cur]; o.Kr[1] = K[cur ^ 1];
            return build_isa_binned(K[cur], K[cur ^ 1], kshift0);
        }
        o.Kr[0] = K[cur ^ 1]; o.Kr[1] = K[cur];
        return o.dense_built ? rebucket<IdxT, true, false, true>(L, c, w, K[cur], (const IdxT *)d_sa, n, 0, kshift0, d_sa, o.Kr[0], w.Va, &o.m)
                             : rebucket<IdxT, true, false, false>(L, c, w, K[cur], (const IdxT *)d_sa, n, 0, kshift0, d_sa, o.Kr[0], w.Va, &o.m);
    }
};

}
}
```

### deltaq_amd/csrc/dq_round0_plan.h

```cpp
#pragma once
#include <algorithm>
#include <cmath>
#include <cstddef>
#include <cstdint>

#include "dq_flags.h"

#if defined(__HIPCC__)
#define DQ_HD __host__ __device__
#else
#define DQ_HD
#endif

namespace dq {

constexpr int kKgramSamples = 1024;
constexpr int kBktCap = 12288;
constexpr int kBktCapFine = 6144;
constexpr int64_t kBktMaxX = 5120;
constexpr int kBktMaxBin = 48;
constexpr int kBktArrBits = 6;
constexpr int kSplitTop = 512;
constexpr int kSplitSub = 512;
constexpr int kSplitBuckets = kSplitTop * kSplitSub;
// ... 4 lines not shown
constexpr int kTieSamples = 4096;
constexpr int64_t kRound0MinN = 1 << 16;
constexpr int kSlotBuckets = 1 << 16;
constexpr int kEarlyPasses = 3;

constexpr int kXcds = 8;
constexpr int kXcdTileN = 1024 * 12;
DQ_HD inline int64_t xcd_eighth(int64_t n)
{
    const int64_t e = (n + kXcds - 1) / kXcds;
    return (e + kXcdTileN - 1) / kXcdTileN * kXcdTileN;
}

constexpr int kHistGroupThreads = 256;
constexpr int kHistLoads = 4;
struct HistSpan {
    int64_t c0 = 0, c1 = 0;
    int eighth = 0;
    int64_t member = 0, members = 0;
};
DQ_HD inline HistSpan hist_span(int64_t n, int64_t group, int64_t groups, bool eighths)
{
    HistSpan h;
    h.c1 = n >> 4;
    h.member = group;
    h.members = groups;
    if (eighths) {
        const int64_t per = groups / kXcds, ech = xcd_eighth(n) >> 4;
        h.eighth = (int)(group / per);
        const int64_t lo = h.eighth * ech;
        h.c0 = lo < h.c1 ? lo : h.c1;
        h.c1 = h.c0 + ech < h.c1 ? h.c0 + ech : h.c1;
        h.member = group % per;
        h.members = per;
    }
    return h;
}
DQ_HD inline int64_t hist_stride(const HistSpan &h) { return h.members * kHistGroupThreads; }
DQ_HD inline int64_t hist_chunk(const HistSpan &h, int tid, int64_t trip)
{
    return h.c0 + (h.member + trip * h.members) * kHistGroupThreads + tid;
}

inline int index_bits(int64_t n) { return n <= 1 ? 1 : 64 - __builtin_clzll((uint64_t)(n - 1)); }

struct TextStats {
    int64_t n = 0;
    int ib = 1;
    int64_t hist[256] = {};
    int64_t kgram[8] = {};
    bool long_run = false;
    int64_t run_chunks = 0;
    double h0 = 0;
    int sigma = 0;
    int64_t cmax = 0;

    TextStats() = default;
    TextStats(const int64_t *words, int64_t n_) : n(n_), ib(index_bits(n_)), long_run(words[256 + 8] != 0), run_chunks(words[256 + 9])
    {
        std::copy(words, words + 256, hist);
        std::copy(words + 256, words + 256 + 8, kgram);
        for (int b = 0; b < 256; ++b) {
            cmax = std::max(cmax, hist[b]);
            if (hist[b] > 0) { ++sigma; const double p = (double)hist[b] / (double)n; h0 -= p * std::log2(p); }
        }
    }
};

struct KeyPlan { int kb = 8; bool packed = false; };

inline KeyPlan choose_key_bytes(const TextStats &s, const Flags &F)
{
    const int64_t n = s.n;
    const double need = std::log2((double)std::max<int64_t>(n, 2)) + 10.0;
    int kb = 8;
    if (s.h0 >= 0.25) kb = std::min(8, std::max(3, (int)std::ceil(need / s.h0)));
    const int fit = (64 - s.ib) / 8;
    bool packed = fit >= 2 && (kb <= fit || (double)fit * s.h0 >= std::log2((double)std::max<int64_t>(n, 2)) + 3.0);
    if (n >= kKgramSamples * 8) {
        const int L = packed ? std::min(kb, fit) : kb;
        const int64_t C = s.kgram[std::max(L, 1) - 1];
        const double twins = (double)n * 2.0 * (double)C / ((double)kKgramSamples * (double)kKgramSamples);
        if (C >= kKgramSamples / 16 && twins > 0.25) { packed = false; kb = 8; }
    }
    if (F.packed) packed = *F.packed != 0 && fit >= 2;
    if (packed) kb = std::min(kb, fit);
    if (F.key_bytes) {
        kb = *F.key_bytes;
        if (kb > fit || kb < 2) packed = false;
    }
    return {kb, packed};
}

inline bool coded_keys_tried(const TextStats &s, const Flags &F, KeyPlan k)
{
    bool coded = !k.packed && k.kb == 8 && s.n >= kCodedMinN;
    if (coded) coded = s.h0 <= kCodedMaxAvgLen - 0.25 && (s.sigma <= 128 || s.n >= 2 * kCodedMinN);
    if (F.coded) coded = *F.coded != 0 && !k.packed && k.kb == 8 && s.n >= 64;
    return coded;
}

inline bool split_round0_wanted(int64_t n, KeyPlan k, int idx_bytes, const Flags &F)
{
    if (idx_bytes != 4 || k.packed || k.kb != 8 || n < kSplitMinN || n > (int64_t)kSplitBuckets * (kFinCap / 2)) return false;
    if (F.split) return *F.split != 0;
    if (F.key_bytes || F.no_bucket) return false;
    return n >= (64ll << 20);
}

struct BucketPlan {
    bool applies = false;
    int keybits = 0, bbytes = 0, lowbits = 0;
    int64_t X = 0, C = 0, ntiles = 0;
    bool ext = false;
    bool xcd_pass = false;
    int64_t hb = 0;
};

inline BucketPlan plan_bucketed(const TextStats &s, const Flags &F, KeyPlan k, bool coded, int idx_bytes)
{
    const int64_t n = s.n;
    const int ib = s.ib;
    BucketPlan p;
    if (coded) return p;
    if (F.no_bucket || F.no_fused_ties || F.sparse || F.key_bytes) return p;
    const bool forced = F.bucket.has_value();
    if (ib > 31 || n < kRound0MinN) return p;
    if (!forced && s.long_run) return p;
    int keybits = std::min(64 - ib, 36);
    if (F.bucket_keybits) keybits = std::max(17, std::min(keybits, *F.bucket_keybits));
    const double tied = (double)n * std::exp2(-(double)keybits * s.h0 / 8.0);
    if (!k.packed) {
        if (!forced && (k.kb >= 8 || tied > 0.3)) return p;
    }
    const double pm = (double)s.cmax / (double)n;
    int bbytes = 2;
    double est = (double)n * pm * pm;
    double need = est + 6.0 * std::sqrt(est) + 64.0;
    const bool force3 = forced && *F.bucket == 3;
    if (need > kBktMaxX || (!forced && n < (12 << 20)) || force3) {
        if (keybits - 24 >= 8 && (forced || n >= (12 << 20))) {
            bbytes = 3;
            est *= pm;
            need = est + 6.0 * std::sqrt(est) + 64.0;
        }
        if (need > kBktMaxX || (bbytes == 2 && !forced)) {
            if (!forced) return p;
            need = kBktMaxX;
        }
    }
    p.applies = true;
    p.keybits = keybits;
    p.bbytes = bbytes;
    p.X = std::min<int64_t>(((int64_t)need + 255) / 256 * 256, kBktMaxX);
    p.C = kBktCap - p.X;
    p.lowbits = keybits - 8 * bbytes;
    p.ntiles = (n + p.C - 1) / p.C;
    const bool room = (size_t)2 * (((size_t)n + 255) / 256 * 256) <= (size_t)(n + 2) * (size_t)idx_bytes;
    p.ext = keybits + 8 <= 56 && p.lowbits + 8 <= 18 && tied > 0.02 && room;
    if (F.bucket_ext) p.ext = *F.bucket_ext != 0 && keybits + 8 <= 56 && room;
    p.xcd_pass = !p.ext && !F.old_first_pass;
    p.hb = (keybits + (p.ext ? 8 : 0)) / 8;
    return p;
}

constexpr int64_t kBktFineMinN = 12ll << 20;
struct FinishTiles {
    bool fine = false;
    bool by_id = false;
    int64_t cap = 0;
    int64_t Cf = 0, g = 0;
    int64_t ntiles = 0;
};

inline FinishTiles plan_finish_tiles(const BucketPlan &b, int64_t n, const Flags &F, bool slots_fit = false)
{
    FinishTiles t;
    if (!b.applies) return t;
    const bool can = b.bbytes == 2 && !b.ext;
    t.fine = can && (F.bucket_tile ? *F.bucket_tile != 0 : !F.bucket.has_value() && n >= kBktFineMinN);
    t.cap = t.fine ? kBktCapFine : kBktCap;
    const int64_t Cf = t.cap - b.X;
    const bool force_by_id = t.fine && slots_fit && F.bucket_slots && *F.bucket_slots == 1;
    if (force_by_id) {
        t.by_id = true;
        t.g = 1;
        t.ntiles = (int64_t)1 << (8 * b.bbytes);
    } else if (Cf >= b.X) {
        t.Cf = Cf;
        t.ntiles = (n + Cf - 1) / Cf;
    } else {
        t.by_id = true;
        t.g = std::min<int64_t>(t.cap / b.X, 64);
        const int64_t nbuckets = (int64_t)1 << (8 * b.bbytes);
        t.ntiles = (nbuckets + t.g - 1) / t.g;
    }
    return t;
}

inline int64_t slot_span_words(int64_t n, int idx_bytes) { return (n + 2) * (int64_t)(8 + idx_bytes) / 8; }

struct SlotPlan {
    bool fits = false;
    int first = 0, second = 0;
    int64_t words = 0;
};

inline SlotPlan bucket_slots_fit(const TextStats &s, const BucketPlan &b, int idx_bytes)
{
    SlotPlan p;
    if (!b.applies || b.bbytes != 2 || b.ext) return p;
    p.first = s.sigma;
    p.second = s.sigma + (s.hist[0] == 0 ? 1 : 0);
    p.words = (int64_t)p.first * p.second * b.X;
    p.fits = p.words <= slot_span_words(s.n, idx_bytes) && p.words < ((int64_t)1 << 32);
    return p;
}

inline void slot_bases(const int64_t *hist , int64_t X, uint32_t *base )
{
    int ra[257], rb[257];
    ra[0] = rb[0] = 0;
    for (int d = 0; d < 256; ++d) {
        ra[d + 1] = ra[d] + (hist[d] > 0 ? 1 : 0);
        rb[d + 1] = rb[d] + (hist[d] > 0 || d == 0 ? 1 : 0);
    }
    for (int A = 0; A < 256; ++A)
        for (int B = 0; B < 256; ++B)
            base[A * 256 + B] = (uint32_t)(X * ((int64_t)ra[A] * rb[256] + (hist[A] > 0 ? rb[B] : 0)));
    base[65536] = (uint32_t)(X * ra[256] * rb[256]);
}

inline bool bucket_slots_wanted(const SlotPlan &p, const FinishTiles &t, const Flags &F)
{
    if (F.bucket_slots && *F.bucket_slots == 0) return false;
    return p.fits && t.fine && t.by_id && t.g == 1;
}

inline size_t finish_bounds_entries(int64_t n)
{
    const size_t by_words = (size_t)n / (kBktCapFine / 2) + 4;
    return n < kRound0MinN ? by_words : std::max<size_t>(by_words, 65536 + 4);
}

struct Round0Route {
    BucketPlan b;
    SlotPlan sp;
    FinishTiles ft;
    bool slots = false;
};

inline Round0Route plan_round0_route(const TextStats &s, const Flags &F, KeyPlan k, bool coded, int idx_bytes, uint64_t span_words)
{
    Round0Route r;
    r.b = plan_bucketed(s, F, k, coded, idx_bytes);
    if (!r.b.applies) return r;
    r.sp = bucket_slots_fit(s, r.b, idx_bytes);
    r.ft = plan_finish_tiles(r.b, s.n, F, r.sp.fits);
    r.slots = bucket_slots_wanted(r.sp, r.ft, F) && (uint64_t)r.sp.words <= span_words &&
              (size_t)(2 * kSlotBuckets + 5) * 4 <= finish_bounds_entries(s.n) * 8;
    return r;
}

inline bool uniform_text_cut_by_bucket(int64_t n)
{
    int64_t words[256 + 10] = {};
    for (int d = 0; d < 256; ++d) words[d] = n / 256 + (d < n % 256 ? 1 : 0);
    const TextStats s(words, n);
    const Flags none;
    const KeyPlan k = choose_key_bytes(s, none);
    const BucketPlan b = plan_bucketed(s, none, k, false, 4);
    const FinishTiles t = plan_finish_tiles(b, n, none);
    return b.applies && t.fine && t.by_id && t.g == 1;
}

inline int64_t slots_cut_min_n()
{
    static const int64_t at = [] {
        static_assert(kBktFineMinN % 256 == 0, "the search steps in multiples of 256");
        int64_t lo = kBktFineMinN / 256, hi = lo;
        while (!uniform_text_cut_by_bucket(hi * 256)) {
            lo = hi;
            hi *= 2;
            if (hi * 256 >= (1ll << 31)) return (int64_t)0;
        }
        while (hi - lo > 1) {
            const int64_t mid = lo + (hi - lo) / 2;
            if (uniform_text_cut_by_bucket(mid * 256)) hi = mid; else lo = mid;
        }
        for (int64_t n = std::max<int64_t>((hi - 3) * 256, kBktFineMinN); n < hi * 256; ++n)
            if (uniform_text_cut_by_bucket(n)) return n;
        return hi * 256;
    }();
    return at;
}

inline int early_status_passes(int64_t n, const Flags &F)
{
    if (F.status_zero) return *F.status_zero != 0 ? 0 : kEarlyPasses;
    const int64_t at = slots_cut_min_n();
    return at > 0 && n >= at ? 0 : kEarlyPasses;
}

inline bool fused_ties_wanted(int64_t n, KeyPlan k, const Flags &F)
{
    return k.packed && k.kb >= 2 && n >= kRound0MinN && !F.no_fused_ties && !F.sparse;
}

enum class DenseGuess { kNeither, kGuessDense, kTakeSample };

inline DenseGuess dense_guess(int64_t n, KeyPlan k)
{
    if (n < kRound0MinN || k.packed || k.kb != 8) return DenseGuess::kNeither;
    return n < (8 << 20) ? DenseGuess::kGuessDense : DenseGuess::kTakeSample;
}

inline bool predict_dense(DenseGuess g, int64_t tied_pairs, const Flags &F)
{
    if (F.sparse) return *F.sparse == 0;
    return g == DenseGuess::kGuessDense || (g == DenseGuess::kTakeSample && tied_pairs * 12 > kTieSamples);
}

inline bool binned_isa_pays(int64_t n, const Flags &F)
{
    const bool pays = F.binned_isa ? *F.binned_isa != 0 : n > (32ll << 20);
    return pays && n >= kRound0MinN && 2 * index_bits(n) <= 63 && !F.no_binned_isa;
}

struct RunPlan {
    bool runs_wanted = false;
    bool long_run_seen = false;
    bool late_runs_possible = false;
};

inline RunPlan plan_runs(const TextStats &s, const Flags &F, int idx_bytes, int period_hint)
{
    RunPlan r;
    const bool can = idx_bytes == 4 && s.n >= kRound0MinN;
    r.long_run_seen = can && s.long_run;
    r.runs_wanted = (r.long_run_seen && s.run_chunks * 16 * 16 >= s.n) || (period_hint > 0 && can);
    r.late_runs_possible = can;
    if (F.runs) { r.runs_wanted = idx_bytes == 4 && *F.runs != 0; r.late_runs_possible = r.late_runs_possible && *F.runs != 0; }
    if (F.mid_groups) r.runs_wanted = r.runs_wanted && *F.mid_groups >= 256;
    return r;
}

}
```

### deltaq_amd/csrc/dq_sa_kernels.h

```cpp
#pragma once
#include <stdint.h>

#if defined(__HIPCC__)
#define DQ_HD __host__ __device__
#else
#define DQ_HD
#endif

namespace dq {

template <int kMaxLen>
DQ_HD inline int suffix_window_compare(const uint8_t *text, int64_t n, int64_t h, int64_t a, int64_t b)
{
    static_assert(kMaxLen % 8 == 0, "whole words");
    typedef uint64_t u64_any __attribute__((aligned(1), may_alias));
    const int64_t pa = a + h, pb = b + h;
    uint64_t wa[kMaxLen / 8], wbv[kMaxLen / 8];
#pragma unroll
    for (int k = 0; k < kMaxLen / 8; ++k) {
        wa[k] = *reinterpret_cast<const u64_any *>(text + pa + 8 * k);
        wbv[k] = *reinterpret_cast<const u64_any *>(text + pb + 8 * k);
    }
    int d = kMaxLen;
    bool a_less = false;
#pragma unroll
    for (int k = kMaxLen / 8 - 1; k >= 0; --k) {
        const uint64_t x = __builtin_bswap64(wa[k]), y = __builtin_bswap64(wbv[k]);
        if (x != y) { d = 8 * k + (__builtin_clzll(x ^ y) >> 3); a_less = x < y; }
    }
    const int64_t la = n - pa, lb = n - pb;
    const int64_t lim = la < lb ? (la < kMaxLen ? la : kMaxLen) : (lb < kMaxLen ? lb : kMaxLen);
    if (d < lim) return a_less ? -1 : 1;
    if (lim < kMaxLen) return la < lb ? -1 : 1;
    return 0;
}

}

#if defined(__HIPCC__)
#include "dq_runs.h"
#include "dq_device_utils.h"

namespace dq {

template <typename IdxT>
__global__ __launch_bounds__(kBlock) void gather_key2_kernel(uint64_t *__restrict__ comp,
                                                             const IdxT *__restrict__ suf,
                                                             const IdxT *__restrict__ ISA,
                                                             int64_t m, int64_t n, int64_t h, int kbits,
                                                             int rshift = 0,
                                                             const uint32_t *__restrict__ RL = nullptr ,
                                                             const uint8_t *__restrict__ text = nullptr, int run_order = 0)
{
    for (int64_t j = (int64_t)blockIdx.x * kBlock + threadIdx.x; j < m;
         j += (int64_t)gridDim.x * kBlock) {
        const int64_t s = (int64_t)suf[j];
        int64_t off = h;
        uint64_t k2 = 0;
        bool keyed = false;
        if (RL) {
            const uint32_t r = RL[s];
            if (run_order) { k2 = (int64_t)r >= h ? (uint64_t)run_order_key(text, n, s, r, run_order) : 0ull; keyed = true; }
            else if ((int64_t)r > h) off = (int64_t)r;
        }
        if (!keyed) {
            const int64_t q = s + off;
            k2 = q < n ? (uint64_t)((int64_t)ISA[q] + h) : (off > h ? 0ull : (uint64_t)(n - 1 - s));
        }
        comp[j] = ((comp[j] >> rshift) << kbits) | k2;
    }
}

static __global__ __launch_bounds__(kBlock) void keys_to_ranks_kernel(uint64_t *__restrict__ comp, int64_t m, int kbits)
{
    for (int64_t j = (int64_t)blockIdx.x * kBlock + threadIdx.x; j < m; j += (int64_t)gridDim.x * kBlock)
        comp[j] >>= kbits;
}

template <typename IdxT>
__global__ __launch_bounds__(kBlock) void gather_text_key_kernel(uint64_t *__restrict__ comp,
                                                                 const IdxT *__restrict__ suf,
                                                                 const uint8_t *__restrict__ text,
                                                                 int64_t m, int64_t n, int64_t h, int ebytes)
{
    const int kbits = 8 * ebytes + 3;
    for (int64_t j = (int64_t)blockIdx.x * kBlock + threadIdx.x; j < m;
         j += (int64_t)gridDim.x * kBlock) {
        const int64_t q = (int64_t)suf[j] + h;
        int64_t len = n - q;
        len = len < 0 ? 0 : (len > ebytes ? ebytes : len);
        uint64_t bytes = 0;
        for (int b = 0; b < ebytes; ++b) bytes = (bytes << 8) | (b < len ? (uint64_t)text[q + b] : 0ull);
        comp[j] = (comp[j] << kbits) | (bytes << 3) | (uint64_t)len;
    }
}

constexpr int kFinishThreads = 256;

template <typename IdxT, int kMaxG, int kMaxLen>
__global__ __launch_bounds__(kFinishThreads) void small_group_finish_kernel(
    const uint64_t *__restrict__ rank, const IdxT *__restrict__ suf, const uint8_t *__restrict__ text,
    int64_t m, int64_t n, int64_t h, IdxT *__restrict__ SA, uint64_t *__restrict__ out_rank,
    IdxT *__restrict__ out_suf, unsigned long long *__restrict__ out_count,
    const unsigned long long *__restrict__ m_dev = nullptr)
{
    if (m_dev) {
        const unsigned long long real = m_dev[0];
        if (real > (unsigned long long)m || m_dev[1] != 0) return;
        m = (int64_t)real;
    }
    __shared__ uint32_t wave_tot[kFinishThreads / kWave];
    __shared__ unsigned long long s_base;
    const int lane = lane_id();
    const int w = threadIdx.x >> 6;
    for (int64_t j0 = (int64_t)blockIdx.x * kFinishThreads; j0 < m; j0 += (int64_t)gridDim.x * kFinishThreads) {
    const int64_t j = j0 + threadIdx.x;

    uint32_t emit = 0;
    uint64_t r = 0;
    int g = 1;
    bool head = false;
    if (j < m) {
        r = rank[j];
        int left = 0, right = 0;
#pragma unroll
        for (int i = 1; i <= kMaxG; ++i)
            if (left == i - 1 && j - i >= 0 && rank[j - i] == r) left = i;
#pragma unroll
        for (int i = 1; i <= kMaxG; ++i)
            if (right == i - 1 && j + i < m && rank[j + i] == r) right = i;
        g = left + right + 1;
        if (g > kMaxG) emit = 1;
        else head = left == 0;
    }
    int64_t s[kMaxG];
    if (head) {
#pragma unroll
        for (int i = 0; i < kMaxG; ++i) s[i] = i < g ? (int64_t)suf[j + i] : 0;
        auto cmp = [&](int64_t a, int64_t b) -> int { return suffix_window_compare<kMaxLen>(text, n, h, a, b); };
        bool decided = true;
        if (g == 2) {
            const int c = cmp(s[0], s[1]);
            if (c == 0) decided = false;
            if (c > 0) { const int64_t t = s[0]; s[0] = s[1]; s[1] = t; }
        } else
#pragma unroll
        for (int pass = 0; pass < kMaxG - 1; ++pass) {
#pragma unroll
            for (int i = 0; i < kMaxG - 1; ++i) {
                if (i + 1 < g && i < g - 1 - pass) {
                    const int c = cmp(s[i], s[i + 1]);
                    if (c == 0) decided = false;
                    if (c > 0) { const int64_t t = s[i]; s[i] = s[i + 1]; s[i + 1] = t; }
                }
            }
        }
        if (decided) {
#pragma unroll
            for (int i = 0; i < kMaxG; ++i)
                if (i < g) SA[(int64_t)r + i] = (IdxT)s[i];
        } else {
            emit = (uint32_t)g;
        }
    }
    const uint32_t incl = wave_incl_sum(emit);
    if (lane == kWave - 1) wave_tot[w] = incl;
    __syncthreads();
    uint32_t off = incl - emit, tot = 0;
#pragma unroll
    for (int k = 0; k < kFinishThreads / kWave; ++k) {
        const uint32_t c = wave_tot[k];
        if (k < w) off += c;
        tot += c;
    }
    if (threadIdx.x == 0) s_base = tot ? atomicAdd(out_count, (unsigned long long)tot) : 0ull;
    __syncthreads();
    if (emit != 0) {
        const int64_t o = (int64_t)s_base + off;
        if (head) {
            for (int i = 0; i < g; ++i) { out_rank[o + i] = r; out_suf[o + i] = suf[j + i]; }
        } else {
            out_rank[o] = r;
            out_suf[o] = suf[j];
        }
    }
    __syncthreads();
    }
}

static __global__ __launch_bounds__(kBlock) void sample_ties_kernel(const uint64_t *__restrict__ keys, int64_t m,
                                                             int kshift, int samples, int64_t *__restrict__ count)
{
    const int i = blockIdx.x * kBlock + threadIdx.x;
    bool tie = false;
    if (i < samples && m > 1) {
        const int64_t p = (int64_t)((__int128)i * (m - 1) / samples);
        tie = (keys[p] >> kshift) == (keys[p + 1] >> kshift);
    }
    const uint64_t b = __ballot(tie);
    if (lane_id() == 0 && b) atomicAdd((unsigned long long *)count, (unsigned long long)__popcll(b));
}

template <typename IdxT>
__global__ __launch_bounds__(kBlock) void isa_from_sa_kernel(const IdxT *__restrict__ SA,
                                                             IdxT *__restrict__ ISA, int64_t n)
{
    for (int64_t p = (int64_t)blockIdx.x * kBlock + threadIdx.x; p < n; p += (int64_t)gridDim.x * kBlock)
        ISA[SA[p]] = (IdxT)p;
}

template <typename IdxT>
__global__ __launch_bounds__(kBlock) void sa_words_kernel(const IdxT *__restrict__ SA, int64_t n, int ib,
                                                          uint64_t *__restrict__ words)
{
    for (int64_t p = (int64_t)blockIdx.x * kBlock + threadIdx.x; p < n; p += (int64_t)gridDim.x * kBlock)
        words[p] = ((uint64_t)p << ib) | (uint64_t)SA[p];
}

template <typename IdxT>
__global__ __launch_bounds__(kBlock) void isa_scatter_kernel(const uint64_t *__restrict__ rank,
                                                             const IdxT *__restrict__ suf,
                                                             IdxT *__restrict__ ISA, int64_t m)
{
    for (int64_t j = (int64_t)blockIdx.x * kBlock + threadIdx.x; j < m; j += (int64_t)gridDim.x * kBlock)
        ISA[suf[j]] = (IdxT)rank[j];
}

}
#endif
```

### deltaq_amd/csrc/dq_slot_finish_plan.h

```cpp
#pragma once
#include <cstdint>
#include <vector>

#include "dq_round0_plan.h"

namespace dq {

constexpr int kSfThreads = 512;
constexpr int kSfItems = 10;
constexpr int kSfCap = kSfThreads * kSfItems;
constexpr int kSfBinBits = 13;
constexpr int kSfBins = 1 << kSfBinBits;
constexpr int kSfMaxLowbits = 20;
constexpr int kSfLeft = 4, kSfRight = 4;
static_assert(kSfLeft == kSfRight, "sf_step continues both sides from kSfLeft + 1");
constexpr uint32_t kSfPadFront = 0u, kSfPadBack = 0xffffffffu;
static_assert(kSfCap >= kBktMaxX, "a slot holds at most X words, and a tile is one slot");
static_assert(kSfCap < (1 << 16) && (kSfBins / 2) % kSfThreads == 0, "16-bit starts; whole bin words per thread");
static_assert(kSfMaxLowbits + kBktArrBits <= 32 && kBktMaxBin + 1 < (1 << kBktArrBits), "a unique key fits 32 bits");

DQ_HD inline int sf_bin_shift(int lowbits) { return lowbits > kSfBinBits ? lowbits - kSfBinBits : 0; }
DQ_HD inline uint32_t sf_bin(uint32_t key, int shift) { return key >> shift; }
DQ_HD inline uint32_t sf_unique(uint32_t key, uint32_t arrival) { return (key << kBktArrBits) | ((arrival + 1) & ((1u << kBktArrBits) - 1)); }
DQ_HD inline uint32_t sf_key(uint32_t unique) { return unique >> kBktArrBits; }
DQ_HD inline uint32_t sf_arrival(uint32_t unique) { return (unique & ((1u << kBktArrBits) - 1)) - 1; }
DQ_HD inline bool sf_same_bin(uint32_t a, uint32_t b, int shift) { return ((a ^ b) >> (shift + kBktArrBits)) == 0; }

DQ_HD inline void sf_left(uint32_t mine, uint32_t other, uint32_t &fin, uint32_t &tie)
{
    const uint32_t lo = mine - sf_arrival(mine);
    fin -= other > mine ? 1u : 0u;
    tie |= other - lo < mine - lo ? 1u : 0u;
}
DQ_HD inline void sf_right(uint32_t mine, uint32_t other, uint32_t &fin) { fin += other < mine ? 1u : 0u; }

struct SfRank {
    uint32_t fin = 0, tie = 0;
    bool more = false;
};

template <typename At>
DQ_HD inline SfRank sf_window(At at, int p, int shift)
{
    const uint32_t mine = at(p);
    SfRank r;
    r.fin = (uint32_t)p;
    uint32_t last = mine;
#if defined(__HIPCC__)
#pragma unroll
#endif
    for (int d = 1; d <= kSfLeft; ++d) sf_left(mine, at(p - d), r.fin, r.tie);
#if defined(__HIPCC__)
#pragma unroll
#endif
    for (int d = 1; d <= kSfRight; ++d) {
        last = at(p + d);
        sf_right(mine, last, r.fin);
    }
    r.more = sf_arrival(mine) > (uint32_t)kSfLeft || sf_same_bin(mine, last, shift);
    return r;
}

template <typename At>
DQ_HD inline bool sf_step(At at, int M, int p, int d, int shift, uint32_t mine, SfRank &r)
{
    const uint32_t l = at(p - d >= 0 ? p - d : -1), o = at(p + d < M ? p + d : M);
    sf_left(mine, l, r.fin, r.tie);
    sf_right(mine, o, r.fin);
    return (uint32_t)d < sf_arrival(mine) || sf_same_bin(mine, o, shift);
}

inline SfRank sf_rank_in_bin(const uint32_t *U, int s0, int s1, int p)
{
    SfRank r;
    r.fin = (uint32_t)s0;
    for (int q = s0; q < s1; ++q) {
        if (U[q] < U[p]) ++r.fin;
        if (sf_key(U[q]) == sf_key(U[p]) && sf_arrival(U[q]) < sf_arrival(U[p])) r.tie = 1;
    }
    return r;
}

inline int sf_tile_model(const uint64_t *words, int M, int ib, int lowbits, const uint32_t *order, uint32_t *sa, uint8_t *tie,
                         int *maxbin = nullptr)
{
    const int shift = sf_bin_shift(lowbits);
    const uint32_t lowmask = (uint32_t)((1ull << lowbits) - 1), imask = (uint32_t)((1ull << ib) - 1);
    std::vector<uint32_t> count(kSfBins, 0), start(kSfBins + 1, 0), unique((size_t)M);
    int mx = 0;
    for (int i = 0; i < M; ++i) {
        const uint32_t e = order ? order[i] : (uint32_t)i;
        const uint32_t key = (uint32_t)(words[e] >> ib) & lowmask;
        const uint32_t arrival = count[sf_bin(key, shift)]++;
        unique[e] = sf_unique(key, arrival);
        mx = std::max(mx, (int)arrival + 1);
    }
    if (maxbin) *maxbin = mx;
    if (mx > kBktMaxBin) return 8;
    for (int b = 0; b < kSfBins; ++b) start[b + 1] = start[b] + count[b];
    std::vector<uint32_t> U((size_t)(kSfLeft + M + kSfRight), kSfPadFront), S((size_t)M);
    for (int d = 0; d < kSfRight; ++d) U[(size_t)(kSfLeft + M + d)] = kSfPadBack;
    for (int e = 0; e < M; ++e) {
        const uint32_t s = start[sf_bin(sf_key(unique[e]), shift)] + sf_arrival(unique[e]);
        U[kSfLeft + s] = unique[e];
        S[s] = (uint32_t)words[e] & imask;
    }
    const auto at = [&](int i) { return U.at((size_t)(kSfLeft + i)); };
    for (int p = 0; p < M; ++p) {
        SfRank r = sf_window(at, p, shift);
        for (int d = kSfLeft + 1; r.more && d < (1 << kBktArrBits); ++d) r.more = sf_step(at, M, p, d, shift, at(p), r);
        sa[r.fin] = S[p];
        tie[r.fin] = (uint8_t)r.tie;
    }
    return 0;
}

}
```

### deltaq_amd/csrc/dq_slot_rank.h

```cpp
#pragma once
#include "dq_bucket_sort.h"
#include "dq_xcd_rank.h"

namespace dq {

struct SlotRankCtl {
    uint32_t ticket[kXcds];
    uint32_t pad[64 - kXcds];
    uint32_t cursor[kSlotBuckets];
};

__device__ __forceinline__ void slot_plan_body(int A, const int64_t *__restrict__ bytehist, int64_t X, uint32_t *__restrict__ slot_base )
{
    __shared__ int tmp[kWavesPerBlock];
    __shared__ int s_rank, s_present;
    const int d = threadIdx.x;
    const int pa = bytehist[d] > 0 ? 1 : 0, pb = (pa || d == 0) ? 1 : 0;
    int na, nb;
    const int ra = block_excl_sum(pa, tmp, &na);
    __syncthreads();
    const int rb = block_excl_sum(pb, tmp, &nb);
    if (A == kRadixSize) {
        if (d == 0) slot_base[kSlotBuckets] = (uint32_t)(X * na * nb);
        return;
    }
    if (d == A) { s_rank = ra; s_present = pa; }
    __syncthreads();
    slot_base[A * kRadixSize + d] = (uint32_t)(X * ((int64_t)s_rank * nb + (s_present ? rb : 0)));
}

static __global__ __launch_bounds__(kBlock) void slot_plan_kernel(const int64_t *__restrict__ bytehist, int64_t X,
                                                           uint32_t *__restrict__ slot_base )
{
    slot_plan_body(blockIdx.x, bytehist, X, slot_base);
}

static __global__ __launch_bounds__(kBlock) void slot_setup_kernel(const int64_t *__restrict__ bytehist, const uint8_t *__restrict__ text,
                                                            int64_t n, int places, int64_t *__restrict__ digit_offset,
                                                            const int64_t *__restrict__ xcd_hist, int64_t *__restrict__ sub_offset,
                                                            int64_t X, uint32_t *__restrict__ slot_base )
{
    const int g = blockIdx.x;
    if (g < places) text_digit_offsets_body(g, bytehist, text, n, places, digit_offset, xcd_hist, sub_offset);
    else slot_plan_body(g - places, bytehist, X, slot_base);
}

constexpr int kSlotOutThreads = kRadixSize;
static __global__ __launch_bounds__(kSlotOutThreads) void slot_out_kernel(uint32_t *__restrict__ count , uint32_t X,
                                                                   const int64_t *__restrict__ first_offset , int64_t n,
                                                                   uint32_t *__restrict__ out ,
                                                                   BucketFlags *__restrict__ flags)
{
    static_assert(kSlotOutThreads == kBlock, "block_excl_sum scans kBlock values");
    __shared__ uint32_t tmp[kWavesPerBlock];
    const int A = blockIdx.x, B = threadIdx.x;
    int64_t lo = first_offset[A], hi = A + 1 < kRadixSize ? first_offset[A + 1] : n;
    lo = lo < 0 ? 0 : (lo > n ? n : lo);
    hi = hi < lo ? lo : (hi > n ? n : hi);
    const uint32_t room = (uint32_t)(hi - lo);
    const uint32_t raw = count[A * kRadixSize + B];
    const uint32_t c = min(raw, X);
    uint32_t total;
    const uint32_t excl = block_excl_sum(c, tmp, &total);
    const uint32_t place = min(excl, room);
    const uint32_t kept = min(c, room - place);
    if (kept != raw) {
        atomicOr(&flags->overflow, 2ull);
        count[A * kRadixSize + B] = kept;
    }
    out[A * kRadixSize + B] = (uint32_t)lo + place;
    if (A == kRadixSize - 1 && B == kRadixSize - 1) out[kSlotBuckets] = (uint32_t)n;
}

#ifdef DQ_SLOT_PHASE_TIMING
__device__ long long *g_slot_ts = nullptr;
__device__ unsigned int g_slot_ts_next = 0;
#define DQ_SLOT_PHASE(i) do { if (threadIdx.x == 0 && g_slot_ts) g_slot_ts[(long long)ts_row * 8 + (i)] = clock64(); } while (0)
#else
#define DQ_SLOT_PHASE(i) do { } while (0)
#endif

constexpr int kSlotRankThreads = 1024;
constexpr int kSlotRankItems = 12;
constexpr int kSlotTileN = kSlotRankThreads * kSlotRankItems;

static __global__ __launch_bounds__(kSlotRankThreads, 1) void slot_rank_kernel(
    const uint64_t *__restrict__ kin , uint64_t *__restrict__ wout, int64_t n,
    int shift , int bshift ,
    const int64_t *__restrict__ region , const uint32_t *__restrict__ slot_base ,
    SlotRankCtl *__restrict__ ctl, BucketFlags *__restrict__ flags)
{
    constexpr int kThreads = kSlotRankThreads, kItems = kSlotRankItems, kTileN = kSlotTileN;
    constexpr int kPerXcd = kRadixSize / kXcds;
    __shared__ __attribute__((aligned(16))) uint64_t exch[kTileN];
    __shared__ uint32_t cnt[kRadixSize];
    __shared__ uint32_t tile_base[kRadixSize];
    __shared__ uint32_t gofs[kRadixSize];
    __shared__ uint32_t glim[kRadixSize];
    __shared__ uint32_t wtmp[kRadixSize / kWave];
    __shared__ uint32_t r_lo[kRadixSize], r_hi[kRadixSize], r_tiles[kRadixSize];
    __shared__ uint32_t xs[kXcds][kPerXcd + 1];
    __shared__ uint32_t s_lo, s_cnt;

    const int tid = threadIdx.x;
    const int w = tid >> 6;
    const int lane = lane_id();
    const uint32_t xcd = hw_xcc_id();

    if (tid < kRadixSize) {
        const int64_t lo = region[tid], hi = tid + 1 < kRadixSize ? region[tid + 1] : n;
        r_lo[tid] = (uint32_t)lo;
        r_hi[tid] = (uint32_t)hi;
        r_tiles[tid] = (uint32_t)((hi - lo + kTileN - 1) / kTileN);
        cnt[tid] = 0;
    }
    __syncthreads();
    if (tid < kXcds) {
        uint32_t run = 0;
        for (int j = 0; j < kPerXcd; ++j) { xs[tid][j] = run; run += r_tiles[tid + kXcds * j]; }
        xs[tid][kPerXcd] = run;
    }
    __syncthreads();

    int tried = 0;
    int32_t pend_e = -1;
    uint32_t pend_t = 0;
    auto issue = [&]() {
        pend_e = -1;
        for (; tried < kXcds; ++tried) {
            const int32_t e = (int32_t)((xcd + (uint32_t)tried) & (kXcds - 1));
            if (xs[e][kPerXcd] > 0) { pend_e = e; pend_t = atomicAdd(&ctl->ticket[e], 1u); return; }
        }
    };
    auto resolve = [&]() {
        while (pend_e >= 0) {
            if (pend_t < xs[pend_e][kPerXcd]) {
                int j = 0;
                while (xs[pend_e][j + 1] <= pend_t) ++j;
                const int B = pend_e + kXcds * j;
                const uint32_t lo = r_lo[B] + (pend_t - xs[pend_e][j]) * (uint32_t)kTileN;
                const uint32_t left = r_hi[B] - lo;
                s_lo = lo;
                s_cnt = left < (uint32_t)kTileN ? left : (uint32_t)kTileN;
                return;
            }
            ++tried;
            issue();
        }
        s_cnt = 0;
    };

    if (tid == 0) { issue(); resolve(); issue(); }
    __syncthreads();
    uint32_t lo = s_lo, valid = s_cnt;

    uint64_t nw[kItems];
    auto load_words = [&](uint32_t at, uint32_t m) {
        if (m == 0) return;
        const uint64_t *src = kin + at;
#pragma unroll
        for (int k = 0; k < kItems; ++k) {
            const uint32_t q = (uint32_t)(k * kThreads + tid);
            nw[k] = src[q < m ? q : m - 1];
        }
    };
    load_words(lo, valid);
#ifdef DQ_SLOT_PHASE_TIMING
    __shared__ uint32_t s_row;
#endif

    while (valid > 0) {
#ifdef DQ_SLOT_PHASE_TIMING
        if (tid == 0) s_row = g_slot_ts ? atomicAdd(&g_slot_ts_next, 1u) : 0u;
#endif
        uint64_t key[kItems];
#pragma unroll
        for (int k = 0; k < kItems; ++k) key[k] = nw[k];
        const uint32_t B = digit_of(key[0], bshift);
        uint32_t sbase = 0, room = 0;
        if (tid < kRadixSize) {
            const uint32_t b = (uint32_t)tid * kRadixSize + B;
            sbase = slot_base[b];
            room = slot_base[b + 1] - sbase;
        }
        if (tid == 0) { resolve(); issue(); }
        __syncthreads();
#ifdef DQ_SLOT_PHASE_TIMING
        const uint32_t ts_row = s_row;
#endif
        DQ_SLOT_PHASE(0);
        const uint32_t next_lo = s_lo, next_valid = s_cnt;
        load_words(next_lo, next_valid);

        uint32_t pos[kItems];
#pragma unroll
        for (int k = 0; k < kItems; ++k)
            pos[k] = atomicAdd(&cnt[digit_of(key[k], shift)], (uint32_t)(k * kThreads + tid) < valid ? 1u : 0u);
        __syncthreads();
        DQ_SLOT_PHASE(1);

        uint32_t tot = 0, incl = 0, abase = 0;
        if (tid < kRadixSize) {
            tot = cnt[tid];
            cnt[tid] = 0;
            if (tot && room) abase = atomicAdd(&ctl->cursor[(uint32_t)tid * kRadixSize + B], tot);
            incl = wave_incl_sum(tot);
            if (lane == kWave - 1) wtmp[w] = incl;
        }
        __syncthreads();
        uint32_t excl_tile = 0;
        if (tid < kRadixSize) {
            uint32_t off = 0;
#pragma unroll
            for (int i = 0; i < kRadixSize / kWave; ++i) if (i < w) off += wtmp[i];
            excl_tile = off + incl - tot;
            tile_base[tid] = excl_tile;
        }
        __syncthreads();

#pragma unroll
        for (int k = 0; k < kItems; ++k)
            if ((uint32_t)(k * kThreads + tid) < valid) exch[pos[k] + tile_base[digit_of(key[k], shift)]] = key[k];
        if (tid < kRadixSize) {
            gofs[tid] = sbase + abase - excl_tile;
            glim[tid] = excl_tile + (abase < room ? room - abase : 0u);
            if (tot && abase + tot > room) atomicOr(&flags->overflow, 2ull);
        }
        __syncthreads();
        DQ_SLOT_PHASE(2);
#pragma unroll
        for (int k = 0; k < kItems; ++k) key[k] = exch[k * kThreads + tid];

#pragma unroll
        for (int k = 0; k < kItems; ++k) {
            const uint32_t q = (uint32_t)(k * kThreads + tid);
            const uint32_t d = digit_of(key[k], shift);
            if (q < valid && q < glim[d]) wout[gofs[d] + q] = key[k];
        }
        DQ_SLOT_PHASE(3);
        lo = next_lo;
        valid = next_valid;
    }
}

}
```

### deltaq_amd/csrc/dq_sorter_impl.h

```cpp
#pragma once
#include "dq_runtime.h"
#include "dq_alpha_code.h"
#include "dq_onesweep.h"
#include "dq_radix.h"
#include "dq_sa_kernels.h"
#include "dq_seg_fused.h"
#include "dq_small.h"
#include "dq_small_groups.h"
#include "dq_mid_groups.h"
#include "dq_runs.h"
#include "dq_ties.h"
#include "dq_isa_pairs.h"
#include "dq_bucket_sort.h"
#include "dq_xcd_rank.h"
#include "dq_pair_chains.h"
#include "dq_tail.h"
#include "dq_split_round0.h"
#include "dq_round0.h"

namespace dq {
namespace {

constexpr int kPairChainTries = 3;
constexpr int64_t kPairChainMinM = 1 << 23;
// ... 205 lines not shown
            return DQ_OK;
        }
        LAUNCH(L, DQ_K_ISA_UPDATE, cnt, cnt * (8 + wb),
               hipLaunchKernelGGL(isa_update_words_kernel<IdxT>, dim3(grid_for(cnt)), dim3(kBlock), 0, st, binned, cnt, u_ib, n, w.ISA));
        return DQ_OK;
    }

    int doubling_round_small(int kbits)
    {
        uint64_t *A = Kr[rcur], *B = Kr[rcur ^ 1];
        IdxT *As = Vr[rcur], *Bs = Vr[rcur ^ 1];
        const RoundLayout lay = round_layout(m, A, As, B, Bs);
        SmallGroupCounters *ctr = reinterpret_cast<SmallGroupCounters *>(w.totals + 4);
        HIP_TRY(hipMemsetAsync(ctr, 0, sizeof(SmallGroupCounters), st));
        const bool cap32 = m < kSgShortList;
        const int mid_g = mid_group_cap(m);
        const bool use_mid = mid_g > 0;
        const int l_shift = (use_mid && !flags().no_l_shift) ? (mid_g >= 1024 ? 10 : mid_g >= 512 ? 9 : 8) : 0;
        if (use_mid) {
            int rc = launch_mid_round(mid_g, m, A, As, lay, h, kbits, ctr, nullptr, m * (8 + wb + wb + wb + 8 + wb), l_shift);
            if (rc != DQ_OK) return rc;
            first_rank32 = nullptr;
        } else if (cap32) {
            constexpr int kTile = sg_tile<kSgMaxGShort>();
            LAUNCH(L, DQ_K_SMALL_ROUND, m, m * (8 + wb + wb + wb + 8 + wb),
                   hipLaunchKernelGGL((small_group_round_kernel<IdxT, kSgMaxGShort>), dim3((unsigned)((m + kTile - 1) / kTile)),
                                      dim3(kSgThreads), 0, st, (const uint64_t *)A, (const IdxT *)As,
                                      (const IdxT *)w.ISA, m, n, h, kbits, d_sa, lay.t_rank, lay.t_suf, lay.l_key, lay.l_suf, lay.u_end,
                                      lay.u_suf_end, ctr, (const SmallGroupCounters *)nullptr));
        } else {
            constexpr int kTile = sg_tile<kSgMaxG>();
            LAUNCH(L, DQ_K_SMALL_ROUND, m, m * (8 + wb + wb + wb + 8 + wb),
                   hipLaunchKernelGGL((small_group_round_kernel<IdxT, kSgMaxG>), dim3((unsigned)((m + kTile - 1) / kTile)),
                                      dim3(kSgThreads), 0, st, (const uint64_t *)A, (const IdxT *)As,
                                      (const IdxT *)w.ISA, m, n, h, kbits, d_sa, lay.t_rank, lay.t_suf, lay.l_key, lay.l_suf, lay.u_end,
                                      lay.u_suf_end, ctr, (const SmallGroupCounters *)nullptr));
        }
        HIP_TRY(hipMemcpyAsync(c.pinned, ctr, sizeof(SmallGroupCounters), hipMemcpyDeviceToHost, st));
        HIP_TRY(hipStreamSynchronize(st));
        const int64_t m1 = c.pinned[0] & 0xffffffffll, mU = (int64_t)((uint64_t)c.pinned[0] >> 32), mL = c.pinned[1];
        if (flags().trace)
            fprintf(stderr, "[dq] %s round h=%lld m=%lld%s -> tied %lld, to radix %lld, moved %lld\n",
                    use_mid ? "mid-group" : "small", (long long)h,
                    (long long)m, wide_list(m) ? " (wide)" : "", (long long)m1, (long long)mL, (long long)mU);
        if (mU > 0) {
            const int rc = apply_rank_updates(A, As, lay.u_end, lay.u_suf_end, mU, use_mid ? upd_ib() : 0);
            if (rc != DQ_OK) return rc;
        }
        int64_t mLs = 0;
        if (mL > 0) {
            uint64_t *Kx[2] = {lay.l_key, lay.l_partner};
            IdxT *Vx[2] = {lay.l_suf, lay.l_partner_suf};
            int xcur = 0;
            int rc = onesweep_sort_pairs<IdxT>(L, w, Kx, Vx, mL, std::max(1, kbits + rbits - l_shift), xcur, l_shift);
            if (rc != DQ_OK) return rc;
            rc = rebucket<IdxT, false, true, true>(L, c, w, Kx[xcur], (const IdxT *)Vx[xcur], mL, kbits, l_shift, d_sa,
                                                   B + m1, Bs + m1, &mLs, 0, l_shift);
            if (rc != DQ_OK) return rc;
        }
        rcur ^= 1;
        m = m1 + mLs;
        if (mL == 0) small_cap = use_mid ? mid_g : cap32 ? kSgMaxGShort : kSgMaxG;
        only_small_groups = mL == 0;
        prev_large = last_large;
        last_large = mL;
        return DQ_OK;
    }

    int chain_len = kSgChain;
    bool tail_behind_chain = false;
    int spec_misses = 0;
    int doubling_rounds_small_chain()
    {
        return small_cap > kSgMaxGShort ? small_chain<0>() : small_cap == kSgMaxGShort ? small_chain<kSgMaxGShort>() : small_chain<kSgMaxG>();
    }

    static constexpr int kChainSteps = 3;
    int launch_mid_round(int g, int64_t mm, const uint64_t *A, const IdxT *As, const RoundLayout &lay, int64_t hh, int kbits,
                         SmallGroupCounters *ctr, const SmallGroupCounters *prev, int64_t alg_bytes, int l_shift = 0, int steps = 1)
    {
        const int64_t tile = g == 256 ? mg_tile<256>() : g == 512 ? mg_tile<512>() : mg_tile<1024>();
        const dim3 grid((unsigned)((mm + tile - 1) / tile));
        auto go = [&](auto kern) -> int {
            LAUNCH(L, DQ_K_MID_ROUND, mm, alg_bytes,
                   hipLaunchKernelGGL(kern, grid, dim3(kMgThreads), 0, st, A, As, (const IdxT *)w.ISA, mm, n, hh, kbits, d_sa, lay.t_rank, lay.t_suf,
                                      lay.l_key, lay.l_suf, lay.u_end, lay.u_suf_end, ctr, prev, rl(), (const uint8_t *)w.text, run_order,
                                      first_rank32, upd_ib(), l_shift));
            return DQ_OK;
        };
        if constexpr (sizeof(IdxT) == 4) {
            if (steps == kChainSteps)
                return g == 256 ? go(mid_group_round_kernel<IdxT, 256, kChainSteps>) : g == 512 ? go(mid_group_round_kernel<IdxT, 512, kChainSteps>)
                                                                                                 : go(mid_group_round_kernel<IdxT, 1024, kChainSteps>);
        }
        return g == 256 ? go(mid_group_round_kernel<IdxT, 256>) : g == 512 ? go(mid_group_round_kernel<IdxT, 512>)
                                                                            : go(mid_group_round_kernel<IdxT, 1024>);
    }

    template <int kCap>
    int small_chain()
    {
        const int64_t m_in = m;
        HIP_TRY(hipMemsetAsync(w.sg_ctr, 0, (kSgChain + 2) * sizeof(SmallGroupCounters), st));
        int64_t hr = h;
        int steps = (kCap == 0 && sizeof(IdxT) == 4 && m_in < kSgShortList && !runs_on) ? kChainSteps : 1;
        if (const std::optional<int> v = flags().chain_steps) steps = (*v >= kChainSteps && kCap == 0 && sizeof(IdxT) == 4 && !runs_on) ? kChainSteps : 1;
        for (int r = 0; r < chain_len; ++r) {
            uint64_t *A = Kr[rcur], *B = Kr[rcur ^ 1];
            IdxT *As = Vr[rcur], *Bs = Vr[rcur ^ 1];
            const RoundLayout lay = round_layout(m_in, A, As, B, Bs);
            const int kbits = std::min(bit_length((uint64_t)(n - 1) + (uint64_t)hr), 64 - rbits);
            if constexpr (kCap == 0) {
                const int rc = launch_mid_round(small_cap, m_in, A, As, lay, hr, kbits, w.sg_ctr + r,
                                                r == 0 ? (const SmallGroupCounters *)nullptr : w.sg_ctr + r - 1, 0, 0, steps);
                if (rc != DQ_OK) return rc;
            } else {
                constexpr int kTile = sg_tile<kCap>();
                LAUNCH(L, DQ_K_SMALL_ROUND, m_in, 0,
                       hipLaunchKernelGGL((small_group_round_kernel<IdxT, kCap>), dim3((unsigned)((m_in + kTile - 1) / kTile)),
                                          dim3(kSgThreads), 0, st, (const uint64_t *)A, (const IdxT *)As,
                                          (const IdxT *)w.ISA, m_in, n, hr, kbits, d_sa, lay.t_rank, lay.t_suf, lay.l_key, lay.l_suf, lay.u_end,
                                          lay.u_suf_end, w.sg_ctr + r, r == 0 ? (const SmallGroupCounters *)nullptr : w.sg_ctr + r - 1));
            }
            LAUNCH(L, DQ_K_ISA_UPDATE, m_in, 0,
                   hipLaunchKernelGGL(isa_update_kernel<IdxT>, dim3(grid_for(m_in)), dim3(kBlock), 0, st,
                                      (const uint64_t *)lay.u_end, (const IdxT *)lay.u_suf_end, (int64_t)0, w.ISA,
                                      (const SmallGroupCounters *)(w.sg_ctr + r), kCap == 0 ? upd_ib() : 0));
            rcur ^= 1;
            hr *= (kCap == 0 ? steps + 1 : 2);
        }
        TailResult *res = reinterpret_cast<TailResult *>(w.sg_ctr + kSgChain);
        const bool spec_tail = tail_behind_chain;
        if (spec_tail) {
            if (flags().trace) fprintf(stderr, "[dq] tail kernel launched behind a chain of %d at h=%lld\n", chain_len, (long long)hr);
            LAUNCH(L, DQ_K_SMALL_ROUND, m_in, 0,
                   launch_tail((const uint64_t *)Kr[rcur], (const IdxT *)Vr[rcur], (int)0, hr, res,
                               (const unsigned long long *)&w.sg_ctr[chain_len - 1].tied_moved));
        }
        HIP_TRY(hipMemcpyAsync(c.pinned, w.sg_ctr, (kSgChain + 2) * sizeof(SmallGroupCounters), hipMemcpyDeviceToHost, st));
        HIP_TRY(hipStreamSynchronize(st));
        int64_t cur_m = m_in;
        for (int r = 0; r < chain_len; ++r) {
            if (c.pinned[2 * r + 1] != 0) return fail(DQ_ERR_HIP, "chained small-group round met a large group");
            if (cur_m > 0) count_rounds(cur_m);
            cur_m = c.pinned[2 * r] & 0xffffffffll;
        }
        m = cur_m;
        h = hr;
        if (spec_tail && cur_m > 0) {
            const int64_t rounds = c.pinned[2 * kSgChain], entries = c.pinned[2 * kSgChain + 1], left = c.pinned[2 * kSgChain + 2];
            if (cur_m <= kTailMax) {
                if (flags().trace)
                    fprintf(stderr, "[dq] tail behind a chain of %d: %lld tied suffixes from h=%lld on, %lld rounds (%lld list entries in all)\n",
                            chain_len, (long long)cur_m, (long long)hr, (long long)rounds, (long long)entries);
                if (left != 0) return fail(DQ_ERR_HIP, "tail rounds did not finish (round bound hit)");
                count_rounds(entries, rounds);
                m = 0;
            }
        }
        return DQ_OK;
    }

    int pair_chain_phase(int *outcome, bool forced)
    {
        *outcome = 1;
        uint64_t *A = Kr[rcur], *B = Kr[rcur ^ 1];
        IdxT *As = Vr[rcur], *Bs = Vr[rcur ^ 1];
        const int ib = bit_length((uint64_t)(n - 1));
        const int64_t ntiles = (m + kPcTile - 1) / kPcTile;
        const size_t scratch = (size_t)kHistBlocks * kMaxPasses * kRadixSize * 4;
        int maxg = m >= kSgShortList ? 2 : (m * 3 <= n ? kPcMaxG : (m * 2 <= n ? 3 : 2));
        if (const std::optional<int> v = flags().pair_maxg) maxg = std::min(maxg >= 3 ? maxg : 2, *v);
        const int xbits = maxg == 2 ? (ib + 7) / 8 * 8 : ib;
        uint32_t *tile_cnt = w.pc_tiles;
        PairCounters *ctr = reinterpret_cast<PairCounters *>(w.totals + 4);
        const int64_t m_in = m;
        int rc = L.begin(DQ_K_PAIR_CHAINS, m, m * 2 * (8 + wb));
        if (rc != DQ_OK) return rc;
        hipLaunchKernelGGL((pair_split_kernel<IdxT, false>), dim3((unsigned)ntiles), dim3(kPcThreads), 0, st,
                           (const uint64_t *)A, (const IdxT *)As, m, xbits, maxg, tile_cnt, (uint64_t *)nullptr, (IdxT *)nullptr,
                           (uint64_t *)nullptr, (IdxT *)nullptr);
        hipLaunchKernelGGL(pair_scan_kernel, dim3(1), dim3(kPcScanThreads), 0, st, tile_cnt, ntiles, ctr);
        HIP_TRY(hipGetLastError());
        rc = L.end();
        if (rc != DQ_OK) return rc;
        HIP_TRY(hipMemcpyAsync(c.pinned, ctr, sizeof(PairCounters), hipMemcpyDeviceToHost, st));
        HIP_TRY(hipStreamSynchronize(st));
        const int64_t cnt = c.pinned[0], copied = c.pinned[1];
        const int64_t half = std::max(sg_half(), (m + 1) & ~(int64_t)1);
        if (cnt == 0 || half + cnt > n || (!forced && copied * 5 > m * 3)) {
            if (flags().trace)
                fprintf(stderr, "[dq] pair chains h=%lld m=%lld: given up, %lld entries in groups > %d\n", (long long)h, (long long)m,
                        (long long)copied, maxg);
            *outcome = 0;
            return DQ_OK;
        }
        count_rounds(m_in);
        LAUNCH(L, DQ_K_PAIR_CHAINS, m, m * (8 + wb) + cnt * (8 + wb) + copied * (8 + wb),
               hipLaunchKernelGGL((pair_split_kernel<IdxT, true>), dim3((unsigned)ntiles), dim3(kPcThreads), 0, st,
                                  (const uint64_t *)A, (const IdxT *)As, m, xbits, maxg, tile_cnt, B + half, Bs + half, B, Bs));
        const int64_t rtiles = (cnt + kPcTile - 1) / kPcTile;
        if (2 * align_up((size_t)rtiles) * 4 > scratch) { *outcome = 0; return DQ_OK; }
        uint64_t *Kx[2] = {B + half, A + half};
        IdxT *Vx[2] = {Bs + half, As + half};
        int xcur = 0;
        rc = onesweep_sort_pairs<IdxT>(L, w, Kx, Vx, cnt, maxg == 2 ? xbits : 2 * ib, xcur);
        const uint64_t sort_mask = maxg == 2 ? (1ull << xbits) - 1 : ~0ull;
        if (rc != DQ_OK) return rc;
        uint32_t *nt = reinterpret_cast<uint32_t *>(Kx[xcur ^ 1]);
        uint8_t *tstat = reinterpret_cast<uint8_t *>(nt + cnt);
        uint8_t *answer = tstat + cnt;
        uint32_t *far = reinterpret_cast<uint32_t *>(Vx[xcur ^ 1]);
        uint32_t *tile_head = w.hist_partial;
        uint32_t *carry = tile_head + align_up((size_t)rtiles);
        rc = L.begin(DQ_K_PAIR_CHAINS, cnt, cnt * (2 * (8 + wb) + 4 * wb));
        if (rc != DQ_OK) return rc;
        const unsigned rgrid = (unsigned)((cnt + kPcThreads - 1) / kPcThreads);
        hipLaunchKernelGGL(pair_link_kernel<IdxT>, dim3((unsigned)rtiles), dim3(kPcThreads), 0, st,
                           (const uint64_t *)Kx[xcur], cnt, xbits, sort_mask, (const IdxT *)w.ISA, n, h, nt, tstat, far, tile_head);
        hipLaunchKernelGGL(pair_carry_kernel, dim3(1), dim3(kPcScanThreads), 0, st, (const uint32_t *)tile_head, rtiles, carry);
        for (int r = 0; r < kPcResolveRounds; ++r)
            hipLaunchKernelGGL(pair_resolve_kernel, dim3(rgrid), dim3(kPcThreads), 0, st, (const uint32_t *)nt,
                               (const uint32_t *)carry, cnt, tstat, far);
        if (maxg == 2) {
            hipLaunchKernelGGL(pair_emit_kernel<IdxT>, dim3(rgrid), dim3(kPcThreads), 0, st, (const uint64_t *)Kx[xcur],
                               (const IdxT *)Vx[xcur], cnt, xbits, (const uint32_t *)nt, (const uint32_t *)carry,
                               (const uint8_t *)tstat, d_sa, w.ISA, B, Bs, ctr);
        } else {
            hipLaunchKernelGGL(pair_answer_kernel<IdxT>, dim3(rgrid), dim3(kPcThreads), 0, st, (const IdxT *)Vx[xcur], cnt,
                               (const uint32_t *)nt, (const uint32_t *)carry, (const uint8_t *)tstat, answer);
            hipLaunchKernelGGL(pair_finish_kernel<IdxT>, dim3((unsigned)ntiles), dim3(kPcThreads), 0, st, (const uint64_t *)A,
                               (const IdxT *)As, m_in, maxg, (const uint32_t *)tile_cnt, (const uint8_t *)answer, d_sa, w.ISA,
                               B, Bs, ctr);
        }
        HIP_TRY(hipGetLastError());
        rc = L.end();
        if (rc != DQ_OK) return rc;
        HIP_TRY(hipMemcpyAsync(c.pinned, ctr, sizeof(PairCounters), hipMemcpyDeviceToHost, st));
        HIP_TRY(hipStreamSynchronize(st));
        rcur ^= 1;
        m = c.pinned[1];
        if ((m_in - m) * 2 >= m_in) *outcome = 2;
        if (flags().trace)
            fprintf(stderr, "[dq] pair chains h=%lld m=%lld (groups <= %d): %lld pair records, %lld entries in larger groups, %lld entries left\n",
                    (long long)h, (long long)m_in, maxg, (long long)cnt, (long long)copied, (long long)m);
        return DQ_OK;
    }

    void launch_tail(const uint64_t *rank, const IdxT *suf, int mm, int64_t hh, TailResult *res, const unsigned long long *m_dev)
    {
        const std::optional<int> forced = flags().chain_steps;
        const bool three = sizeof(IdxT) == 4 && !runs_on && !(forced && *forced < kChainSteps);
        if constexpr (sizeof(IdxT) == 4) {
            if (three) {
                hipLaunchKernelGGL((tail_rounds_kernel<IdxT, uint32_t, kChainSteps>), dim3(1), dim3(kTailThreads), 0, st, rank, suf, mm, n, hh,
                                   w.ISA, d_sa, (const uint32_t *)nullptr, res, m_dev);
                return;
            }
        }
        (void)three;
        hipLaunchKernelGGL((tail_rounds_kernel<IdxT, uint64_t, 1>), dim3(1), dim3(kTailThreads), 0, st, rank, suf, mm, n, hh, w.ISA, d_sa,
                           rl(), res, m_dev);
    }

    int tail_rounds()
    {
        TailResult *res = reinterpret_cast<TailResult *>(w.sg_ctr + kSgChain);
        static_assert(sizeof(TailResult) <= 2 * sizeof(SmallGroupCounters), "the result sits behind the chain counters");
        HIP_TRY(hipMemsetAsync(res, 0, sizeof(TailResult), st));
        LAUNCH(L, DQ_K_SMALL_ROUND, m, m * (8 + wb + wb + 64),
               launch_tail((const uint64_t *)Kr[rcur], (const IdxT *)Vr[rcur], (int)m, h, res, (const unsigned long long *)nullptr));
        HIP_TRY(hipMemcpyAsync(c.pinned, res, sizeof(TailResult), hipMemcpyDeviceToHost, st));
        HIP_TRY(hipStreamSynchronize(st));
        const int64_t rounds = c.pinned[0], entries = c.pinned[1], left = c.pinned[2];
        if (flags().trace)
            fprintf(stderr, "[dq] tail: %lld tied suffixes from h=%lld on, %lld rounds in one launch (%lld list entries in all)\n",
                    (long long)m, (long long)h, (long long)rounds, (long long)entries);
        if (left != 0) return fail(DQ_ERR_HIP, "tail rounds did not finish (round bound hit)");
        count_rounds(entries, rounds);
        m = 0;
        return DQ_OK;
    }

    int compute_run_lengths(int period = 1)
    {
        if constexpr (sizeof(IdxT) != 4) {
            return fail(DQ_ERR_HIP, "run lengths: int32 indices only");
        } else {
            const int64_t nchunks = (n + kRunChunk - 1) / kRunChunk;
            LAUNCH(L, DQ_K_RUNS, n, 2 * n + 4 * n,
                   hipLaunchKernelGGL(runlen_chunk_kernel<false>, dim3((unsigned)nchunks), dim3(kRunThreads), 0, st,
                                      (const uint8_t *)w.text, n, w.run_lead, w.run_link, (const uint32_t *)nullptr, (uint32_t *)nullptr, period);
                   hipLaunchKernelGGL(runlen_carry_kernel, dim3(1), dim3(kRunScanThreads), 0, st, (const uint32_t *)w.run_lead,
                                      (const uint8_t *)w.run_link, nchunks, w.run_carry);
                   hipLaunchKernelGGL(runlen_chunk_kernel<true>, dim3((unsigned)nchunks), dim3(kRunThreads), 0, st,
                                      (const uint8_t *)w.text, n, (uint32_t *)nullptr, (uint8_t *)nullptr,
                                      (const uint32_t *)w.run_carry, w.RL, period));
            return DQ_OK;
        }
    }

    int64_t twin_half = 0;
    const uint8_t *text_src = nullptr;
    int period_hint = 0;
    int twin_pairs_step(bool *done)
    {
        *done = false;
        static_assert(kTwTile == 2048, "w.pc_tiles holds two counters per 2048 list entries");
        const int64_t ntiles = (m + kTwTile - 1) / kTwTile;
        uint32_t *tile_cnt = w.pc_tiles;
        PairCounters *ctr = reinterpret_cast<PairCounters *>(w.totals + 4);
        int rc = L.begin(DQ_K_SMALL_ROUND, m, m * (8 + wb));
        if (rc != DQ_OK) return rc;
        hipLaunchKernelGGL(twin_mark_kernel<IdxT>, dim3((unsigned)ntiles), dim3(kTwThreads), 0, st, (const uint64_t *)Kr[rcur],
                           (const uint32_t *)first_rank32, (const IdxT *)Vr[rcur], m, twin_half, d_sa, w.ISA, tile_cnt);
        hipLaunchKernelGGL(pair_scan_kernel, dim3(1), dim3(kPcScanThreads), 0, st, tile_cnt, ntiles, ctr);
        HIP_TRY(hipGetLastError());
        rc = L.end();
        if (rc != DQ_OK) return rc;
        HIP_TRY(hipMemcpyAsync(c.pinned, ctr, sizeof(PairCounters), hipMemcpyDeviceToHost, st));
        HIP_TRY(hipStreamSynchronize(st));
        const int64_t groups = c.pinned[0], kept = c.pinned[1];
        if (flags().trace)
            fprintf(stderr, "[dq] doubled text at h=%lld: %lld of %lld tied suffixes in pairs (i, i + n/2), %lld other groups\n", (long long)h,
                    (long long)(m - kept), (long long)m, (long long)groups);
        if (kept == 0) { *done = true; return DQ_OK; }
        if (kept == m) return DQ_OK;
        LAUNCH(L, DQ_K_SMALL_ROUND, m, m * (8 + wb) + kept * (8 + wb),
               hipLaunchKernelGGL(twin_compact_kernel<IdxT>, dim3((unsigned)ntiles), dim3(kTwThreads), 0, st, (const uint64_t *)Kr[rcur],
                                  (const uint32_t *)first_rank32, (const IdxT *)Vr[rcur], m, twin_half, (const uint32_t *)tile_cnt,
                                  Kr[rcur ^ 1], Vr[rcur ^ 1]));
        rcur ^= 1;
        first_rank32 = nullptr;
        m = kept;
        return DQ_OK;
    }

    void adopt(const Round0Out<IdxT> &r0)
    {
        for (int i = 0; i < 2; ++i) { Kr[i] = r0.Kr[i]; Vr[i] = r0.Vr[i]; }
        rcur = 0;
        m = r0.m; h = r0.h; rbits = r0.rbits;
        fin_done = r0.fin_done; fin_cap = r0.fin_cap; fin_left = r0.fin_left;
        shallow_ties = r0.shallow_ties; keys_ready = r0.keys_ready; list_ungrouped = r0.list_ungrouped;
        first_rank32 = r0.first_rank32;
        runs_wanted = r0.runs.runs_wanted; long_run_seen = r0.runs.long_run_seen; late_runs_possible = r0.runs.late_runs_possible;
    }

    int run()
    {
        const Flags &F = flags();
        t_sort_info = {};
        HIP_TRY(hipMemsetAsync(w.totals, 0, 64, st));
        Round0Out<IdxT> r0;
        int rc = Round0<IdxT>{c, st, w, n, d_sa, L, text_src, period_hint, r0}.run();
        if (rc != DQ_OK) return rc;
        adopt(r0);
        t_sort_info.initial_active = m;
        if (F.trace)
            fprintf(stderr, "[dq] after round 0: n=%lld, %d index bits, %lld tied suffixes, third list buffer %s\n", (long long)n,
                    bit_length((uint64_t)(n - 1)), (long long)m, w.X ? "carved" : "left out");
        if (m == 0) return flush_profile(c);

        bool sparse = m * 6 <= n || shallow_ties;
        if (F.sparse) sparse = *F.sparse != 0;
        if (keys_ready || list_ungrouped || first_rank32) sparse = false;
        if (sparse) rc = finish_sparse();
        else if (!r0.dense_built) rc = build_isa(Kr[rcur], Vr[rcur], m);
        if (rc != DQ_OK) return rc;

        if (runs_wanted && m > 0 && 32 + rbits <= 64 && ((uses_small_round(m) && !list_ungrouped) ? mid_group_cap(m) > 0 : true)) {
            int period = period_hint > 0 ? period_hint : 1;
            if (F.run_period) period = *F.run_period;
            if (period > h || period > 64) period = 1;
            rc = compute_run_lengths(period);
            if (rc != DQ_OK) return rc;
            runs_on = true;
            run_order = period;
            count_rounds(m);
            if (F.trace)
                fprintf(stderr, "[dq] run-order round (period %d) at h=%lld on %lld tied suffixes\n", period, (long long)h, (long long)m);
            rc = (uses_small_round(m) && !list_ungrouped) ? doubling_round_small(32) : doubling_round_radix(32, 0);
            run_order = 0;
            if (rc != DQ_OK) return rc;
        }

        int64_t m_before = 0;
        int pair_tries = 0, pair_aborts = 0;
        bool pair_paid = true;
        int64_t pair_h = 0;
        int64_t abort_h = 0, abort_m = 0;
        const int64_t tail_max = F.tail_max ? std::min(kTailMax, *F.tail_max) : kTailMax;
        while (m > 0) {
            if (m <= tail_max && fits32() && !keys_ready && !list_ungrouped && !first_rank32 && !run_order) {
                rc = tail_rounds();
                if (rc != DQ_OK) return rc;
                break;
            }
            if (twin_half > 0 && !keys_ready && !list_ungrouped && !run_order) {
                bool done = false;
                rc = twin_pairs_step(&done);
                if (rc != DQ_OK) return rc;
                if (done) break;
            }
            const bool stagnant = m_before > 0 && m * 5 > m_before * 3;
            const std::optional<int> pc = F.pair_chains;
            const int64_t pair_chain_min = F.pair_chains_min ? *F.pair_chains_min : kPairChainMinM;
            const bool after_abort = abort_h == 0 || m * 2 <= abort_m || h >= 16 * abort_h;
            const bool want = pc ? *pc != 0 && (m_before > 0 || *pc > 1)
                                 : m_before > 0 && m >= pair_chain_min && after_abort &&
                                   (pair_tries == 0 || (pair_paid ? stagnant : h >= 16 * pair_h));
            if (want && pair_tries < kPairChainTries && pair_aborts < 2 * kPairChainTries && !F.no_small && fits32() &&
                m < n && !keys_ready && !list_ungrouped && !first_rank32) {
                int outcome = 0;
                m_before = 0;
                const int64_t m_try = m;
                rc = pair_chain_phase(&outcome, pc.has_value());
                if (rc != DQ_OK) return rc;
                if (outcome == 0) { ++pair_aborts; abort_h = h; abort_m = m_try; }
                else { ++pair_tries; pair_paid = outcome == 2; pair_h = h; abort_h = 0; }
                continue;
            }
            const int64_t late_min = F.late_runs_min.value_or(1 << 15);
            const int64_t late_share = F.late_runs_min ? (int64_t)1 << 30 : 64;
            if (late_runs_possible && !runs_on && !runs_late_tried && !run_order && last_large >= late_min && prev_large > 0 &&
                last_large * late_share >= n && last_large * 8 >= prev_large * 7 && h >= 32 && 32 + rbits <= 64 && uses_small_round(m) && !keys_ready &&
                !list_ungrouped && !first_rank32 && mid_group_cap(m) > 0 && !F.no_late_runs) {
                runs_late_tried = true;
                int period = 1;
                while (period * 2 <= 64 && period * 2 <= h) period *= 2;
                if (F.run_period) period = std::min<int>((int)std::min<int64_t>(h, 1 << 20), *F.run_period);
                rc = compute_run_lengths(period);
                if (rc != DQ_OK) return rc;
                runs_on = true;
                run_order = period;
                count_rounds(m);
                if (F.trace)
                    fprintf(stderr, "[dq] late run-order round (period %d) at h=%lld on %lld tied suffixes (%lld in large groups, %lld the round before)\n",
                            period, (long long)h, (long long)m, (long long)last_large, (long long)prev_large);
                rc = doubling_round_small(32);
                run_order = 0;
                if (rc != DQ_OK) return rc;
                m_before = 0;
                continue;
            }
            m_before = m;
            if (only_small_groups && uses_small_round(m) && !keys_ready && !list_ungrouped && (twin_half == 0 || m < (1 << 16)) &&
                !F.no_chain) {
                tail_behind_chain = tail_max >= kTailMax && m <= 4 * tail_max && fits32();
                chain_len = tail_behind_chain ? std::min(kSgChain, 2 << std::min(spec_misses, 2)) : kSgChain;
                if (tail_behind_chain) ++spec_misses;
                rc = doubling_rounds_small_chain();
                if (rc != DQ_OK) return rc;
                continue;
            }
            count_rounds(m);
            const int kbits = bit_length((uint64_t)(n - 1) + (uint64_t)h);
            const int rshift = (kbits + rbits > 64 || (F.force_rshift && !first_rank32)) ? 1 : 0;
            if (rshift && first_rank32) return fail(DQ_ERR_HIP, "rank-shift round on a list with 32-bit ranks");
            if (kbits + rbits - rshift > 64) return fail(DQ_ERR_TOO_LARGE, "composite key exceeds 64 bits");
            if (rshift && F.trace)
                fprintf(stderr, "[dq] rank-shift round at h=%lld on %lld tied suffixes (kbits %d + rbits %d)%s\n", (long long)h,
                        (long long)m, kbits, rbits, kbits + rbits > 64 ? "" : " (forced)");
            if (rshift && keys_ready) {
                LAUNCH(L, DQ_K_GATHER_KEY2, m, m * 16,
                       hipLaunchKernelGGL(keys_to_ranks_kernel, dim3(grid_for(m)), dim3(kBlock), 0, st, Kr[rcur], m, kbits));
                keys_ready = false;
            }
            rc = (uses_small_round(m) && !keys_ready && !rshift && !list_ungrouped) ? doubling_round_small(kbits)
                                                                 : doubling_round_radix(kbits, rshift);
            if (rc != DQ_OK) return rc;
            h *= 2;
        }
        HIP_TRY(hipStreamSynchronize(st));
        return flush_profile(c);
    }
};

template <typename IdxT>
int sufsort_device(DeviceCtx &c, hipStream_t st, Workspace<IdxT> &w, int64_t n, IdxT *d_sa, SortHints hints = SortHints(),
                   const uint8_t *text_src = nullptr)
{
    SuffixSorter<IdxT> sorter(c, st, w, n, d_sa);
    const Flags &F = flags();
    if ((hints.doubled || F.assume_doubled) && n % 2 == 0 && !F.no_twins) sorter.twin_half = n / 2;
    if (hints.run_period > 0 && !F.no_period_hint) sorter.period_hint = hints.run_period;
    sorter.text_src = text_src;
    return sorter.run();
}

template <typename IdxT>
int sufsort_small(DeviceCtx &c, hipStream_t st, const uint8_t *text, int64_t n, IdxT *sa)
{
    Launcher L{c, st, g_prof_on.load()};
    t_sort_info = {};
    LAUNCH(L, DQ_K_SMALL_SORT, n, n * (1 + (int64_t)sizeof(IdxT)),
           hipLaunchKernelGGL(small_sufsort_kernel<IdxT>, dim3(1), dim3(kSmallThreads), 0, st, text, (int)n, sa));
    HIP_TRY(hipStreamSynchronize(st));
    return flush_profile(c);
}

template <typename IdxT>
bool choose_list_buffers(DeviceCtx &c, int64_t n, bool with_sa)
{
    const Flags &F = flags();
    bool lists = n < (1ll << 32) && !F.no_list_buffers;
    size_t free_b = 0, total_b = 0;
    if (lists && c.ws_bytes < carve<IdxT>(nullptr, n, with_sa, true).bytes && hipMemGetInfo(&free_b, &total_b) == hipSuccess) {
        const uint64_t avail = (uint64_t)free_b + c.ws_bytes;
        lists = with_list_buffers<IdxT>(n, with_sa, avail > kWsReserve ? avail - kWsReserve : 0);
    }
    if (F.trace && !lists)
        fprintf(stderr, "[dq] workspace without the third list buffer (n=%lld; %.1f GB free, %.1f GB cached)\n", (long long)n,
                free_b / 1e9, c.ws_bytes / 1e9);
    return lists;
}

template <typename IdxT>
int check_args(const void *text, int64_t n, const void *sa)
{
    if (n < 0) return fail(DQ_ERR_BAD_ARGS, "negative length");
    if (n > 0 && (!text || !sa)) return fail(DQ_ERR_BAD_ARGS, "null buffer");
    if (sizeof(IdxT) == 4 && n > 0x7fffffffLL)
        return fail(DQ_ERR_TOO_LARGE, "n exceeds 2^31-1; use the i64 entry point");
    if (n > (1ll << 32))
        return fail(DQ_ERR_TOO_LARGE, "n exceeds 2^32: the 64-bit entry points take texts of up to 4 GiB");
    return DQ_OK;
}

}

template <typename IdxT>
int sufsort_host(const uint8_t *text, int64_t n, IdxT *sa, int32_t device, SortHints hints)
{
    int rc = check_args<IdxT>(text, n, sa);
    if (rc != DQ_OK) return rc;
    int dev = 0;
    rc = resolve_device(device, &dev);
    if (rc != DQ_OK) return rc;
    if (n == 0) return DQ_OK;
    if (n == 1) { sa[0] = 0; return DQ_OK; }
    if (n == 2) {
        const bool lt = text[0] < text[1];
        sa[0] = lt ? 0 : 1; sa[1] = lt ? 1 : 0;
        return DQ_OK;
    }
    SlotLease lease(dev, n);
    DeviceCtx &c = *lease.c;
    rc = init_ctx(c, dev);
    if (rc != DQ_OK) return rc;
    if (n <= small_limit()) {
        IdxT *io_sa = reinterpret_cast<IdxT *>(c.pinned_io + kSmallTextArea);
        memcpy(c.pinned_io, text, (size_t)n);
        rc = sufsort_small<IdxT>(c, c.stream, c.pinned_io, n, io_sa);
        if (rc != DQ_OK) { drop_pending(c, c.stream); return rc; }
        memcpy(sa, io_sa, (size_t)n * sizeof(IdxT));
        return DQ_OK;
    }
    const bool lists = choose_list_buffers<IdxT>(c, n, true);
    Workspace<IdxT> w = carve<IdxT>(nullptr, n, true, lists);
    rc = ensure_ws(c, w.bytes);
    if (rc != DQ_OK) return rc;
    w = carve<IdxT>(c.ws, n, true, lists);
    hipStream_t st = c.stream;
    HIP_TRY(hipMemcpyAsync(w.text, text, (size_t)n, hipMemcpyHostToDevice, st));
    HIP_TRY(hipMemsetAsync(w.text + n, 0, 64, st));
    rc = sufsort_device<IdxT>(c, st, w, n, w.SAbuf, hints);
    if (rc != DQ_OK) { drop_pending(c, st); return rc; }
    auto copy_out = [&]() -> hipError_t {
        const hipError_t e = hipMemcpyAsync(sa, w.SAbuf, (size_t)n * sizeof(IdxT), hipMemcpyDeviceToHost, st);
        const hipError_t e2 = hipStreamSynchronize(st);
        return e != hipSuccess ? e : e2;
    };
    HIP_TRY(copy_out());
    return DQ_OK;
}

template <typename IdxT>
int sufsort_dev(const void *d_text, int64_t n, void *d_sa, int32_t device, void *stream)
{
    int rc = check_args<IdxT>(d_text, n, d_sa);
    if (rc != DQ_OK) return rc;
    int dev = 0;
    rc = resolve_device(device, &dev);
    if (rc != DQ_OK) return rc;
    if (n == 0) return DQ_OK;
    SlotLease lease(dev, n);
    DeviceCtx &c = *lease.c;
    rc = init_ctx(c, dev);
    if (rc != DQ_OK) return rc;
    if (n <= small_limit()) {
        hipStream_t sst = stream ? (hipStream_t)stream : c.stream;
        rc = sufsort_small<IdxT>(c, sst, (const uint8_t *)d_text, n, (IdxT *)d_sa);
        if (rc != DQ_OK) drop_pending(c, sst);
        return rc;
    }
    const bool lists = choose_list_buffers<IdxT>(c, n, false);
    Workspace<IdxT> w = carve<IdxT>(nullptr, n, false, lists);
    rc = ensure_ws(c, w.bytes);
    if (rc != DQ_OK) return rc;
    w = carve<IdxT>(c.ws, n, false, lists);
    hipStream_t st = stream ? (hipStream_t)stream : c.stream;
    const bool fused_copy = (reinterpret_cast<uintptr_t>(d_text) & 15) == 0 && !flags().text_copy;
    if (!fused_copy) HIP_TRY(hipMemcpyAsync(w.text, d_text, (size_t)n, hipMemcpyDeviceToDevice, st));
    HIP_TRY(hipMemsetAsync(w.text + n, 0, 64, st));
    rc = sufsort_device<IdxT>(c, st, w, n, (IdxT *)d_sa, SortHints(), fused_copy ? (const uint8_t *)d_text : nullptr);
    if (rc != DQ_OK) { drop_pending(c, st); return rc; }
    HIP_TRY(hipStreamSynchronize(st));
    return DQ_OK;
}

template <typename IdxT> int64_t sufsort_workspace_bytes(int64_t n) { return (int64_t)carve<IdxT>(nullptr, n, false, n < (1ll << 32)).bytes; }
template <typename IdxT> int64_t sufsort_workspace_plan(int64_t n, bool host_entry, int64_t avail)
{
    return (int64_t)carve<IdxT>(nullptr, n, host_entry, with_list_buffers<IdxT>(n, host_entry, (uint64_t)std::max<int64_t>(avail, 0))).bytes;
}

}
```

### deltaq_amd/csrc/dq_ties.h

```cpp
#pragma once
#include "dq_onesweep.h"
#include "dq_sa_kernels.h"

namespace dq {

constexpr int kTieMaxRun = 4096;
constexpr int kTieThreads = 1024;

template <typename StatusT>
__global__ __launch_bounds__(kBlock) void tie_seam_kernel(const uint64_t *__restrict__ seam_tab, int64_t ntiles,
                                                          int ib, const int64_t *__restrict__ digit_offset,
                                                          const StatusT *__restrict__ status,
                                                          uint32_t *__restrict__ ebits)
{
    using SB = StatusBits<StatusT>;
    const int64_t idx = (int64_t)blockIdx.x * kBlock + threadIdx.x;
    if (idx >= ntiles * kRadixSize) return;
    const int64_t t = idx / kRadixSize;
    const int d = (int)(idx % kRadixSize);
    const uint64_t first = seam_tab[idx * 2];
    if (first == kSeamEmpty || t == 0) return;
    int64_t tp = t - 1;
    while (tp >= 0 && seam_tab[(tp * kRadixSize + d) * 2] == kSeamEmpty) --tp;
    if (tp < 0) return;
    const uint64_t last = seam_tab[(tp * kRadixSize + d) * 2 + 1];
    if ((last >> ib) != (first >> ib)) return;
    const int64_t o = digit_offset[d] + (int64_t)(status[(t - 1) * kRadixSize + d] & SB::kMask);
    atomicOr(&ebits[(uint64_t)o >> 5], 1u << ((uint32_t)o & 31u));
}

struct TieCounters {
    unsigned long long count;
    unsigned long long overflow;
};

template <typename IdxT>
__global__ __launch_bounds__(kTieThreads) void tie_collect_kernel(const uint64_t *__restrict__ ebits, int64_t nwords,
                                                                  int64_t n, const IdxT *__restrict__ SA,
                                                                  uint64_t *__restrict__ act_rank,
                                                                  IdxT *__restrict__ act_suf,
                                                                  TieCounters *__restrict__ ctr)
{
    __shared__ uint32_t wave_tot[kTieThreads / kWave];
    __shared__ unsigned long long s_base;
    const int lane = lane_id();
    const int w = threadIdx.x >> 6;
    const int64_t i = (int64_t)blockIdx.x * kTieThreads + threadIdx.x;

    uint64_t E = 0, own = 0;
    uint32_t tail = 0;
    bool over = false;
    if (i < nwords) {
        E = ebits[i];
        const uint64_t next0 = (i + 1 < nwords) ? (ebits[i + 1] & 1ull) : 0ull;
        const uint64_t A = E | (E >> 1) | (next0 << 63);
        const int lead = (E & 1ull) ? (E == ~0ull ? 64 : __builtin_ctzll(~E)) : 0;
        own = lead >= 64 ? 0ull : (A & (~0ull << lead));
        if (own >> 63 && next0) {
            int64_t j = i + 1;
            for (;;) {
                const uint64_t F = j < nwords ? ebits[j] : 0ull;
                const int c = F == ~0ull ? 64 : __builtin_ctzll(~F);
                tail += (uint32_t)c;
                if (c < 64) break;
                if (tail > (uint32_t)kTieMaxRun) { over = true; break; }
                ++j;
            }
        }
    }
    if (over) { atomicExch(&ctr->overflow, 1ull); tail = 0; own = 0; }
    const uint32_t cnt = (uint32_t)__popcll(own) + tail;
    const uint32_t incl = wave_incl_sum(cnt);
    if (lane == kWave - 1) wave_tot[w] = incl;
    __syncthreads();
    uint32_t off = incl - cnt, tot = 0;
#pragma unroll
    for (int k = 0; k < kTieThreads / kWave; ++k) {
        const uint32_t c = wave_tot[k];
        if (k < w) off += c;
        tot += c;
    }
    if (threadIdx.x == 0) s_base = tot ? atomicAdd(&ctr->count, (unsigned long long)tot) : 0ull;
    __syncthreads();
    const int64_t out = (int64_t)s_base + off;
    const uint32_t wave_members = __shfl(incl, kWave - 1, kWave);
    if (wave_members < 512u) {
        int64_t o = out, head = 0;
        uint64_t rest = own;
        while (rest) {
            const int b = __builtin_ctzll(rest);
            rest &= rest - 1;
            const int64_t p = i * 64 + b;
            if (!((E >> b) & 1ull)) head = p;
            act_rank[o] = (uint64_t)head;
            act_suf[o] = SA[p];
            ++o;
        }
        for (uint32_t k = 0; k < tail; ++k) {
            act_rank[o] = (uint64_t)head;
            act_suf[o] = SA[(i + 1) * 64 + k];
            ++o;
        }
        return;
    }
    uint64_t todo = __ballot(cnt != 0);
    const uint64_t lbit = 1ull << lane;
    while (todo) {
        const int j = __builtin_ctzll(todo);
        todo &= todo - 1;
        const uint64_t own_j = ((uint64_t)(uint32_t)__builtin_amdgcn_readlane((int)(uint32_t)(own >> 32), j) << 32) |
                               (uint32_t)__builtin_amdgcn_readlane((int)(uint32_t)own, j);
        const uint64_t E_j = ((uint64_t)(uint32_t)__builtin_amdgcn_readlane((int)(uint32_t)(E >> 32), j) << 32) |
                             (uint32_t)__builtin_amdgcn_readlane((int)(uint32_t)E, j);
        const int64_t out_j = (int64_t)(((uint64_t)(uint32_t)__builtin_amdgcn_readlane((int)(uint32_t)((uint64_t)out >> 32), j) << 32) |
                                        (uint32_t)__builtin_amdgcn_readlane((int)(uint32_t)(uint64_t)out, j));
        const uint32_t tail_j = (uint32_t)__builtin_amdgcn_readlane((int)tail, j);
        const int64_t p0 = (i - lane + j) * 64;
        if (own_j & lbit) {
            const uint64_t below = lbit - 1;
            const int64_t p = p0 + lane;
            const int64_t head = (E_j & lbit) ? p0 + (63 - __builtin_clzll(~E_j & below)) : p;
            const int64_t o = out_j + __popcll(own_j & below);
            act_rank[o] = (uint64_t)head;
            act_suf[o] = SA[p];
        }
        if (tail_j) {
            const int64_t head = p0 + (63 - __builtin_clzll(~E_j));
            const int64_t o0 = out_j + __popcll(own_j);
            for (uint32_t k = (uint32_t)lane; k < tail_j; k += kWave) {
                act_rank[o0 + k] = (uint64_t)head;
                act_suf[o0 + k] = SA[p0 + 64 + k];
            }
        }
    }
    (void)n;
}

constexpr int kSettleThreads = 256;
constexpr int kSettleWords = 8;
constexpr int kSettleQueue = 256;
constexpr int kSettleMaxG = 8, kSettleLen = 32;

template <typename IdxT>
__device__ __forceinline__ bool settle_group(IdxT *SA, const uint8_t *__restrict__ text, int64_t n, int64_t h, int64_t head, int g, bool *bad)
{
    uint32_t place = 0;
    bool decided = true;
#pragma unroll 1
    for (int i = 0; i + 1 < g && decided; ++i) {
        const int64_t si = (int64_t)SA[head + i];
#pragma unroll 1
        for (int j = i + 1; j < g && decided; ++j) {
            const int64_t sj = (int64_t)SA[head + j];
            if (!((uint64_t)si < (uint64_t)n && (uint64_t)sj < (uint64_t)n)) { *bad = true; return false; }
            const int c = suffix_window_compare<kSettleLen>(text, n, h, si, sj);
            if (c == 0) decided = false;
            place += c > 0 ? 1u << (4 * i) : 1u << (4 * j);
        }
    }
    if (!decided) return false;
    IdxT s[kSettleMaxG];
#pragma unroll
    for (int i = 0; i < kSettleMaxG; ++i) s[i] = i < g ? SA[head + i] : (IdxT)0;
#pragma unroll
    for (int i = 0; i < kSettleMaxG; ++i)
        if (i < g) SA[head + (int64_t)((place >> (4 * i)) & 15u)] = s[i];
    return true;
}

template <typename IdxT>
__global__ __launch_bounds__(kSettleThreads, 6) void tie_settle_kernel(
    const uint64_t *__restrict__ ebits, int64_t nwords, int64_t n, IdxT *SA, const uint8_t *__restrict__ text, int64_t h,
    uint64_t *__restrict__ list_rank, IdxT *__restrict__ list_suf, int64_t list_cap ,
    TieCounters *__restrict__ ctr , unsigned long long *__restrict__ list_count )
{
    constexpr int kW = kSettleWords, kWaves = kSettleThreads / kWave;
    constexpr int64_t kWaveWords = (int64_t)kWave * kW, kTile = kWaveWords * kWaves;
    static_assert(kWaveWords <= 1024 && kSettleQueue % kWave == 0, "a queue entry has 10 bits for the word");
    if (ctr->overflow != 0 || n < 2) return;
    __shared__ unsigned long long s_seen;
    __shared__ uint32_t s_queue[kWaves][kSettleQueue];
    if (threadIdx.x == 0) s_seen = 0;
    __syncthreads();
    const int lane = lane_id(), wv = threadIdx.x >> 6;
    uint32_t *queue = s_queue[wv];
    unsigned long long seen = 0;
    bool over = false;
    for (int64_t t0 = (int64_t)blockIdx.x * kTile; t0 < nwords; t0 += (int64_t)gridDim.x * kTile) {
        const int64_t w0 = t0 + (int64_t)wv * kWaveWords;
        uint32_t P = 0, total = 0;
        do {
            uint64_t E[kW];
            uint32_t first = 0;
#pragma unroll
            for (int k = 0; k < kW; ++k) {
                const int64_t i = w0 + k * kWave + lane;
                E[k] = i < nwords ? ebits[i] : 0ull;
            }
            const int64_t behind = w0 + kWaveWords;
            const uint32_t last = behind < nwords ? (uint32_t)(ebits[behind] & 1ull) : 0u;
#pragma unroll
            for (int k = 0; k < kW; ++k) first |= (uint32_t)(E[k] & 1ull) << k;
            const uint32_t lane0 = (uint32_t)__builtin_amdgcn_readfirstlane((int)first);
            const uint32_t up = (uint32_t)__shfl_down((int)first, 1, kWave);
            const uint32_t goes = lane == kWave - 1 ? ((lane0 >> 1) | (last << (kW - 1))) : up;
            uint32_t mine = 0;
#pragma unroll
            for (int k = 0; k < kW; ++k) mine += (uint32_t)__popcll(((E[k] >> 1) | ((uint64_t)((goes >> k) & 1u) << 63)) & ~E[k]);
            const uint32_t incl = wave_incl_sum(mine);
            total = (uint32_t)__shfl((int)incl, kWave - 1, kWave);
            if (total == 0) break;
            uint32_t idx = incl - mine;
#pragma unroll
            for (int k = 0; k < kW; ++k) {
                uint64_t heads = ((E[k] >> 1) | ((uint64_t)((goes >> k) & 1u) << 63)) & ~E[k];
                while (heads != 0) {
                    const int b = __builtin_ctzll(heads);
                    heads &= heads - 1;
                    if (idx - P < (uint32_t)kSettleQueue) {
                        const int run = b < 63 ? __builtin_ctzll(~(E[k] >> (b + 1))) : 0;
                        const uint32_t on = (b + run == 63) ? ((goes >> k) & 1u) : 0u;
                        queue[idx - P] = (uint32_t)(k * kWave + lane) | ((uint32_t)b << 10) | ((uint32_t)(run + 1) << 16) | (on << 23);
                    }
                    ++idx;
                }
            }
            __builtin_amdgcn_wave_barrier();
            const uint32_t cnt = min(total - P, (uint32_t)kSettleQueue);
            for (uint32_t q0 = 0; q0 < cnt; q0 += kWave) {
                const uint32_t q = q0 + (uint32_t)lane;
                const uint32_t e = q < cnt ? queue[q] : 0u;
                uint32_t g = (e >> 16) & 127u;
                const int64_t i = w0 + (int64_t)(e & 1023u);
                const int64_t head = i * 64 + (int64_t)((e >> 10) & 63u);
                bool bad = false;
                if ((e >> 23) & 1u) {
                    uint32_t tail = 0;
                    for (int64_t j = i + 1;; ++j) {
                        const uint64_t F = j < nwords ? ebits[j] : 0ull;
                        const int c = F == ~0ull ? 64 : __builtin_ctzll(~F);
                        tail += (uint32_t)c;
                        if (c < 64) break;
                        if (tail > (uint32_t)kTieMaxRun) { bad = true; break; }
                    }
                    g += tail;
                }
                if (g != 0 && (bad || head + (int64_t)g > n)) { over = true; g = 0; }
                const int64_t p = g != 0 ? head : 0;
                const int64_t s0 = (int64_t)SA[p], s1 = (int64_t)SA[p + 1];
                if (g != 0 && !((uint64_t)s0 < (uint64_t)n && (uint64_t)s1 < (uint64_t)n)) { over = true; g = 0; }
                seen += g;
                const bool small = g != 0 && g <= (uint32_t)kSettleMaxG;
                const int c = suffix_window_compare<kSettleLen>(text, n, h, small ? s0 : 0, small ? s1 : 0);
                bool left = g > (uint32_t)kSettleMaxG || (small && c == 0);
                if (g == 2u) {
                    if (c > 0) { SA[head] = (IdxT)s1; SA[head + 1] = (IdxT)s0; }
                } else if (small && c != 0) {
                    bool bad_entry = false;
                    if (!settle_group<IdxT>(SA, text, n, h, head, (int)g, &bad_entry)) left = true;
                    if (bad_entry) { over = true; left = false; }
                }
                const uint32_t emit = left ? g : 0u;
                if (__any(emit != 0)) {
                    const uint32_t upto = wave_incl_sum(emit);
                    const uint32_t tot = (uint32_t)__shfl((int)upto, kWave - 1, kWave);
                    unsigned long long base = 0;
                    if (lane == kWave - 1) base = atomicAdd(list_count, (unsigned long long)tot);
                    base = (unsigned long long)__shfl((long long)base, kWave - 1, kWave);
                    if (emit != 0 && base + tot <= (unsigned long long)list_cap) {
                        int64_t o = (int64_t)base + (upto - emit);
                        for (uint32_t j = 0; j < g; ++j, ++o) {
                            list_rank[o] = (uint64_t)head;
                            list_suf[o] = SA[head + j];
                        }
                    }
                }
            }
            __builtin_amdgcn_wave_barrier();
            P += (uint32_t)kSettleQueue;
        } while (P < total);
    }
    if (over) atomicOr(&ctr->overflow, 1ull);
    seen = wave_sum(seen);
    if (lane == 0 && seen) atomicAdd(&s_seen, seen);
    __syncthreads();
    if (threadIdx.x == 0 && s_seen) atomicAdd(&ctr->count, s_seen);
}

}
```

### deltaq_amd/csrc/dq_xcd_rank.h

```cpp
#pragma once
#include "dq_onesweep.h"

namespace dq {

struct XcdRankCtl {
    uint32_t ticket[kXcds];
    uint32_t cursor[kXcds][kRadixSize];
};

__device__ __forceinline__ uint32_t hw_xcc_id()
{
    uint32_t x;
    asm volatile("s_getreg_b32 %0, hwreg(HW_REG_XCC_ID, 0, 4)" : "=s"(x));
    return x & (kXcds - 1);
}

constexpr int kXcdRankThreads = 1024;
constexpr int kXcdRankItems = 12;
static_assert(kXcdRankThreads * kXcdRankItems == kXcdTileN, "the eighths are cut in tiles of this pass");

static __global__ __launch_bounds__(kXcdRankThreads, 1) void xcd_text_rank_kernel(
    const uint32_t *__restrict__ t32 , uint64_t *__restrict__ kout, int64_t n,
    int shift, int keybits, int ib, const int64_t *__restrict__ sub_offset , XcdRankCtl *__restrict__ ctl)
{
    constexpr int kThreads = kXcdRankThreads, kItems = kXcdRankItems, kTileN = kXcdTileN;
    constexpr int kExchN = kTileN;
    __shared__ __attribute__((aligned(16))) uint64_t exch[kExchN];
    __shared__ uint32_t cnt[kRadixSize];
    __shared__ uint32_t tile_base[kRadixSize];
    __shared__ uint32_t gofs[kRadixSize];
    __shared__ uint32_t wtmp[kRadixSize / kWave];
    __shared__ int32_t s_next;

    const int tid = threadIdx.x;
    const int w = tid >> 6;
    const int lane = lane_id();
    const int64_t E = xcd_eighth(n);
    const int32_t per8 = (int32_t)(E / kTileN);
    const uint32_t xcd = hw_xcc_id();
    int tried = 0;
    int32_t pend_e = -1;
    uint32_t pend_t = 0;
    auto tiles_of = [&](int32_t e) -> int64_t {
        const int64_t left = n - (int64_t)e * E;
        return left <= 0 ? 0 : (std::min(left, E) + kTileN - 1) / kTileN;
    };
    auto issue = [&]() {
        pend_e = -1;
        for (; tried < kXcds; ++tried) {
            const int32_t e = (int32_t)((xcd + (uint32_t)tried) & (kXcds - 1));
            if (tiles_of(e) > 0) { pend_e = e; pend_t = atomicAdd(&ctl->ticket[e], 1u); return; }
        }
    };
    auto resolve = [&]() -> int32_t {
        while (pend_e >= 0) {
            if ((int64_t)pend_t < tiles_of(pend_e)) return pend_e * per8 + (int32_t)pend_t;
            ++tried;
            issue();
        }
        return -1;
    };

    if (tid < kRadixSize) cnt[tid] = 0;
    if (tid == 0) { issue(); s_next = resolve(); issue(); }
    __syncthreads();
    int32_t tile = s_next;

    uint32_t nw[kItems / 4][3];
    auto load_text = [&](int32_t t) {
        if (t < 0) return;
        const int64_t base = (int64_t)t * kTileN;
#pragma unroll
        for (int j = 0; j < kItems / 4; ++j) {
            const int64_t e0 = base + (int64_t)(j * kThreads + tid) * 4;
            if (e0 < n) { nw[j][0] = t32[e0 >> 2]; nw[j][1] = t32[(e0 >> 2) + 1]; nw[j][2] = t32[(e0 >> 2) + 2]; }
        }
    };
    load_text(tile);

    const int kshift = 64 - keybits;
    while (tile >= 0) {
        const int64_t base = (int64_t)tile * kTileN;
        const int valid = (n - base) < kTileN ? (int)(n - base) : kTileN;
        const int e8 = tile / per8;
        auto elem = [&](int k) -> int { return ((k >> 2) * kThreads + tid) * 4 + (k & 3); };

        uint64_t key[kItems];
#pragma unroll
        for (int j = 0; j < kItems / 4; ++j) {
            const int e0 = (j * kThreads + tid) * 4;
            if (e0 < valid) {
                const uint64_t x = __builtin_bswap64((uint64_t)nw[j][0] | ((uint64_t)nw[j][1] << 32));
                const uint64_t y = (uint64_t)__builtin_bswap32(nw[j][2]) << 32;
                const uint64_t x4[4] = {x, (x << 8) | (y >> 56), (x << 16) | (y >> 48), (x << 24) | (y >> 40)};
#pragma unroll
                for (int c = 0; c < 4; ++c) key[4 * j + c] = ((x4[c] >> kshift) << ib) | (uint64_t)(base + e0 + c);
            } else {
#pragma unroll
                for (int c = 0; c < 4; ++c) key[4 * j + c] = ~0ull;
            }
        }
        if (tid == 0) { s_next = resolve(); issue(); }
        __syncthreads();
        const int32_t next = s_next;
        load_text(next);

        uint32_t pos[kItems];
#pragma unroll
        for (int k = 0; k < kItems; ++k)
            pos[k] = atomicAdd(&cnt[digit_of(key[k], shift)], elem(k) < valid ? 1u : 0u);
        __syncthreads();

        uint32_t tot = 0, incl = 0, abase = 0;
        if (tid < kRadixSize) {
            tot = cnt[tid];
            cnt[tid] = 0;
            abase = atomicAdd(&ctl->cursor[e8][tid], tot);
            incl = wave_incl_sum(tot);
            if (lane == kWave - 1) wtmp[w] = incl;
        }
        __syncthreads();
        uint32_t excl_tile = 0;
        if (tid < kRadixSize) {
            uint32_t off = 0;
#pragma unroll
            for (int i = 0; i < kRadixSize / kWave; ++i) if (i < w) off += wtmp[i];
            excl_tile = off + incl - tot;
            tile_base[tid] = excl_tile;
        }
        __syncthreads();

#pragma unroll
        for (int k = 0; k < kItems; ++k)
            if (elem(k) < valid) exch[pos[k] + tile_base[digit_of(key[k], shift)]] = key[k];
        uint64_t skey[kItems];
        if (tid < kRadixSize) gofs[tid] = (uint32_t)sub_offset[e8 * kRadixSize + tid] + abase - excl_tile;
        __syncthreads();
#pragma unroll
        for (int k = 0; k < kItems; ++k) skey[k] = exch[k * kThreads + tid];

#pragma unroll
        for (int k = 0; k < kItems; ++k) {
            const int q = k * kThreads + tid;
            if (q < valid) kout[gofs[digit_of(skey[k], shift)] + (uint32_t)q] = skey[k];
        }
        tile = next;
    }
}

}
```

Before: 105,900 MB/s.

## Read text in place from caller buffer with a small tail block instead of copying

Adds a TextView that reads the caller's text buffer directly and redirects only the last bytes to a small padded tail block, which the histogram pass fills. This lets the slots route skip copying the whole text into the work buffer. A late copy kernel runs whenever a later stage needs the full padded text (other routes, fallback, leftover ties, doubling rounds). It also adds a templated split hi/lo output variant of the slot rank kernel, but only the unsplit variant is launched. Each text access now carries an extra compare and select, and a late copy may still happen.

```diff
diff --git a/deltaq_amd/csrc/dq_flags.h b/deltaq_amd/csrc/dq_flags.h
--- a/deltaq_amd/csrc/dq_flags.h
+++ b/deltaq_amd/csrc/dq_flags.h
@@ -56,6 +56,7 @@
     std::optional<int> slot_finish;
     std::optional<int> tie_settle;
     std::optional<int> status_zero;
+    std::optional<int> text_in_place;
     std::optional<int> hist_loads;
     bool old_first_pass = false;
     bool no_fused_ties = false;
@@ -170,6 +171,7 @@
     f.slot_finish = num("DQ_SLOT_FINISH", 0, 1);
     f.tie_settle = num("DQ_TIE_SETTLE", 0, 1);
     f.status_zero = num("DQ_STATUS_ZERO", 0, 1);
+    f.text_in_place = num("DQ_TEXT_IN_PLACE", 0, 1);
     f.hist_loads = num("DQ_HIST_LOADS", 1, 4);
     f.old_first_pass = on("DQ_OLD_FIRST_PASS");
     f.no_fused_ties = on("DQ_NO_FUSED_TIES");
diff --git a/deltaq_amd/csrc/dq_onesweep.h b/deltaq_amd/csrc/dq_onesweep.h
--- a/deltaq_amd/csrc/dq_onesweep.h
+++ b/deltaq_amd/csrc/dq_onesweep.h
@@ -2,6 +2,7 @@
 #include "dq_coded_keys.h"
 #include "dq_radix.h"
 #include "dq_round0_plan.h"
+#include "dq_text_view.h"
 
 namespace dq {
 
@@ -580,9 +581,11 @@
                                                            unsigned long long *__restrict__ bytehist ,
                                                            unsigned long long *__restrict__ kgram_coll = nullptr,
                                                            uint8_t *__restrict__ copy_out = nullptr ,
-                                                           unsigned long long *__restrict__ xcd_hist = nullptr )
+                                                           unsigned long long *__restrict__ xcd_hist = nullptr ,
+                                                           uint8_t *__restrict__ tail_out = nullptr )
 {
     static_assert(kBlock == kHistGroupThreads, "hist_chunk() counts in workgroups of kBlock threads");
+    static_assert(kTextTailBytes <= kBlock, "one thread per byte of the tail block");
     __shared__ uint32_t hist[kRadixSize * 4];
     if (kgram_coll && blockIdx.x == 0) {
         __shared__ uint32_t s_seen[8 * kKgramBits / 32];
@@ -642,6 +645,7 @@
                 atomicAdd(&xcd_hist[b], ~0ull);
             }
         }
+        if (tail_out && tid < kTextTailBytes) tail_out[tid] = text_tail_byte(text, n, tid);
     }
     __syncthreads();
     const uint32_t c = hist[tid * 4] + hist[tid * 4 + 1] + hist[tid * 4 + 2] + hist[tid * 4 + 3];
@@ -653,7 +657,21 @@
     if (kgram_coll && flat_chunks && lane_id() == 0) atomicAdd(&kgram_coll[9], flat_chunks);
 }
 
-__device__ __forceinline__ void text_digit_offsets_body(int p, const int64_t *__restrict__ bytehist, const uint8_t *__restrict__ text,
+static __global__ __launch_bounds__(kBlock) void text_copy_kernel(const uint8_t *__restrict__ src, uint8_t *__restrict__ dst, int64_t n)
+{
+    const uint4 *s16 = reinterpret_cast<const uint4 *>(src);
+    uint4 *d16 = reinterpret_cast<uint4 *>(dst);
+    const int64_t chunks = n >> 4;
+    for (int64_t i = (int64_t)blockIdx.x * kBlock + threadIdx.x; i < chunks; i += (int64_t)gridDim.x * kBlock) d16[i] = s16[i];
+    if (blockIdx.x == 0)
+        for (int64_t i = (chunks << 4) + threadIdx.x; i < n; i += kBlock) dst[i] = src[i];
+}
+
+__device__ __forceinline__ uint8_t text_byte(const uint8_t *text, int64_t j) { return text[j]; }
+__device__ __forceinline__ uint8_t text_byte(const TextView &text, int64_t j) { return *text.at(j); }
+
+template <typename Text>
+__device__ __forceinline__ void text_digit_offsets_body(int p, const int64_t *__restrict__ bytehist, const Text &text,
                                                         int64_t n, int kb, int64_t *__restrict__ digit_offset,
                                                         const int64_t *__restrict__ xcd_hist, int64_t *__restrict__ sub_offset)
 {
@@ -662,7 +680,7 @@
     const int64_t off = kb - 1 - p;
     const int64_t lead = off < n ? off : n;
     int64_t c = bytehist[d];
-    for (int64_t j = 0; j < lead; ++j) c -= (text[j] == d);
+    for (int64_t j = 0; j < lead; ++j) c -= (text_byte(text, j) == d);
     if (d == 0) c += lead;
     int64_t total;
     const int64_t excl = block_excl_sum(c, tmp, &total);
@@ -676,8 +694,8 @@
             if (s0 >= n) continue;
             const int64_t s1 = std::min(s0 + E, n);
             int64_t ce = xcd_hist[e * kRadixSize + d];
-            for (int64_t j = s0; j < std::min(s0 + off, s1); ++j) ce -= (text[j] == d);
-            for (int64_t j = std::max(s0 + off, s1); j < s1 + off; ++j) ce += j < n ? (text[j] == d) : (d == 0);
+            for (int64_t j = s0; j < std::min(s0 + off, s1); ++j) ce -= (text_byte(text, j) == d);
+            for (int64_t j = std::max(s0 + off, s1); j < s1 + off; ++j) ce += j < n ? (text_byte(text, j) == d) : (d == 0);
             run += ce;
         }
     }
diff --git a/deltaq_amd/csrc/dq_round0.h b/deltaq_amd/csrc/dq_round0.h
--- a/deltaq_amd/csrc/dq_round0.h
+++ b/deltaq_amd/csrc/dq_round0.h
@@ -57,6 +57,7 @@
     const uint8_t *text_src;
     int period_hint;
     Round0Out<IdxT> &o;
+    bool &text_missing;
 
     static constexpr int64_t wb = (int64_t)sizeof(IdxT);
     TextStats s;
@@ -68,6 +69,20 @@
     IdxT *V[2] = {nullptr, nullptr};
 
     const uint64_t *text64() const { return reinterpret_cast<const uint64_t *>(w.text); }
+    TextView view() const { return text_missing ? text_in_place(text_src, w.text, n) : text_copied(w.text, n); }
+    bool settles(const Flags &F) const { return F.tie_settle.value_or(route.slots ? 1 : 0) != 0; }
+    bool view_route(const Flags &F) const { return route.slots && route.b.xcd_pass && settles(F); }
+
+    int need_text(const char *why)
+    {
+        if (!text_missing) return DQ_OK;
+        text_missing = false;
+        if (flags().trace) fprintf(stderr, "[dq] text: copied late, %s (n=%lld)\n", why, (long long)n);
+        LAUNCH(L, DQ_K_TEXT_HIST, n, 2 * n,
+               hipLaunchKernelGGL(text_copy_kernel, dim3((unsigned)std::min<int64_t>(((n >> 4) + kBlock - 1) / kBlock + 1, 4096)), dim3(kBlock), 0,
+                                  L.st, text_src, w.text, n));
+        return DQ_OK;
+    }
     int64_t tie_words() const { return (n + 63) / 64; }
 
     int digit_tables(int kb, bool coded_keys)
@@ -96,12 +111,16 @@
         unsigned long long *xcd_hist = n >= kRound0MinN ? reinterpret_cast<unsigned long long *>(w.bytehist + kXcdHistAt) : nullptr;
         if (xcd_hist) blocks = (blocks + kXcds - 1) / kXcds * kXcds;
         HIP_TRY(hipMemsetAsync(w.bytehist, 0, (size_t)(kXcdHistAt + (xcd_hist ? kXcds * kRadixSize : 0)) * 8, L.st));
+        text_missing = text_in_place_wanted(n, text_src != nullptr, kTextViewMinN, flags());
+        if (flags().trace)
+            fprintf(stderr, "[dq] text: %s (n=%lld)\n", text_missing ? "in place, the caller's buffer and a tail block" :
+                    text_src ? "copied by the histogram pass" : "copied in front of the sort", (long long)n);
         LAUNCH(L, DQ_K_TEXT_HIST, n, n,
                hipLaunchKernelGGL(flags().hist_loads.value_or(kHistLoads) < kHistLoads ? text_hist_kernel<1> : text_hist_kernel<kHistLoads>,
                                   dim3(blocks + 1), dim3(kBlock), 0, L.st,
                                   text_src ? text_src : (const uint8_t *)w.text, n, reinterpret_cast<unsigned long long *>(w.bytehist),
-                                  reinterpret_cast<unsigned long long *>(w.bytehist + 256), text_src ? w.text : (uint8_t *)nullptr,
-                                  xcd_hist));
+                                  reinterpret_cast<unsigned long long *>(w.bytehist + 256), text_src && !text_missing ? w.text : (uint8_t *)nullptr,
+                                  xcd_hist, text_missing ? w.text : (uint8_t *)nullptr));
         HIP_TRY(hipMemcpyAsync(c.pinned, w.bytehist, (256 + 10) * 8, hipMemcpyDeviceToHost, L.st));
         HIP_TRY(hipEventRecord(c.readback, L.st));
         const Flags &F = flags();
@@ -134,6 +153,7 @@
             }
         }
         route = plan_round0_route(s, F, k, coded, (int)wb, slot_span_words_of(w));
+        if (!view_route(F)) DQ_TRY(need_text("the route is not the slots route"));
         if (early > 0) DQ_TRY(prepare_status<IdxT>(L, w, n, k.kb, early));
         else DQ_TRY(prepare_status<IdxT>(L, w, n, route.slots ? (route.b.xcd_pass ? 0 : 1) : std::max(k.kb, kEarlyPasses)));
         if (hist_deferred) return DQ_OK;
@@ -181,7 +201,7 @@
             o.fin_cap = n;
             LAUNCH(L, DQ_K_TIE_COLLECT, n, n / 8,
                    hipLaunchKernelGGL(tie_settle_kernel<IdxT>, dim3((unsigned)groups), dim3(kSettleThreads), 0, L.st,
-                                      reinterpret_cast<const uint64_t *>(ebits), tie_words(), n, d_sa, (const uint8_t *)w.text,
+                                      reinterpret_cast<const uint64_t *>(ebits), tie_words(), n, d_sa, view(),
                                       h_fin >= 0 ? h_fin : (int64_t)k.kb, act_rank, w.Va, o.fin_cap, tctr, listed));
             DQ_TRY(read_totals<IdxT>(L, c, w, 64, "radix look-back timed out (device spin bound hit)"));
             o.m = c.pinned[6];
@@ -305,7 +325,7 @@
                 fprintf(stderr, "[dq] second pass into bucket slots: %d x %d slots of %lld words (n=%lld)\n", sp.first, sp.second,
                         (long long)b.X, (long long)n);
             hipLaunchKernelGGL(slot_setup_kernel, dim3(b.bbytes + kRadixSize + 1), dim3(kBlock), 0, st, (const int64_t *)w.bytehist,
-                               (const uint8_t *)w.text, n, b.bbytes, w.digit_offset, xcd_hist, sub_offset, b.X, slot_base);
+                               view(), n, b.bbytes, w.digit_offset, xcd_hist, sub_offset, b.X, slot_base);
         } else {
             hipLaunchKernelGGL(text_digit_offsets_kernel, dim3(b.bbytes), dim3(kBlock), 0, st, (const int64_t *)w.bytehist,
                                (const uint8_t *)w.text, n, b.bbytes, w.digit_offset, xcd_hist, sub_offset);
@@ -320,7 +340,7 @@
             if (sizeof(XcdRankCtl) > w.ctl_status_stride) return fail(DQ_ERR_HIP, "status buffer too small");
             LAUNCH(L, DQ_K_RADIX_RANK, n, n * (1 + 8),
                    hipLaunchKernelGGL(xcd_text_rank_kernel, dim3((unsigned)std::min<int64_t>(c.ncu, (n + kXcdTileN - 1) / kXcdTileN)),
-                                      dim3(kXcdRankThreads), 0, st, reinterpret_cast<const uint32_t *>(w.text), K[first], n,
+                                      dim3(kXcdRankThreads), 0, st, view(), K[first], n,
                                       ib + lowbits, keybits, ib, (const int64_t *)w.xcd_offset,
                                       reinterpret_cast<XcdRankCtl *>(w.ctl_status)));
         } else {
@@ -329,10 +349,10 @@
                                                       nullptr, nullptr, ib + lowbits, keybits));
         }
         if (slots) {
-            const int groups = resident_groups(&c.slot_rank_groups, (const void *)slot_rank_kernel, kSlotRankThreads, c.dev);
+            const int groups = resident_groups(&c.slot_rank_groups, (const void *)slot_rank_kernel<false>, kSlotRankThreads, c.dev);
             LAUNCH(L, DQ_K_RADIX_RANK, n, n * 16,
-                   hipLaunchKernelGGL(slot_rank_kernel, dim3((unsigned)std::min<int64_t>(groups, (n + kSlotTileN - 1) / kSlotTileN)),
-                                      dim3(kSlotRankThreads), 0, st, (const uint64_t *)K[0], K[1], n, ib + lowbits + 8, ib + lowbits,
+                   hipLaunchKernelGGL(slot_rank_kernel<false>, dim3((unsigned)std::min<int64_t>(groups, (n + kSlotTileN - 1) / kSlotTileN)),
+                                      dim3(kSlotRankThreads), 0, st, (const uint64_t *)K[0], K[1], n, ib + lowbits + 8, ib + lowbits, ib,
                                       (const int64_t *)w.digit_offset, (const uint32_t *)slot_base, sctl, bflags));
         }
         for (int p = 1; p < b.bbytes && !slots; ++p) {
@@ -400,12 +420,14 @@
         DQ_TRY(collect_ties(ebits, nullptr, Kfree, &overflow, Ks, false, b.hb, settle));
         if (overflow) {
             if (F.trace) fprintf(stderr, "[dq] bucketed round 0 gave up (n=%lld): plain digit passes\n", (long long)n);
+            DQ_TRY(need_text("the bucketed round 0 gave up"));
             DQ_TRY(prepare_status<IdxT>(L, w, n, kMaxPasses));
             HIP_TRY(hipMemsetAsync(w.Vb, 0, (size_t)(tie_words() + 1) * 8, st));
             HIP_TRY(hipMemsetAsync(w.totals, 0, 64, st));
             o.m = 0; o.fin_cap = 0; o.fin_left = 0;
             return digit_tables(kb, false);
         }
+        if (o.fin_left > 0) DQ_TRY(need_text("ties are left behind the settle"));
         o.fin_done = settle || o.m <= o.fin_cap;
         o.Kr[0] = Kfree; o.Kr[1] = Ks;
         if (settle) {
diff --git a/deltaq_amd/csrc/dq_round0_plan.h b/deltaq_amd/csrc/dq_round0_plan.h
--- a/deltaq_amd/csrc/dq_round0_plan.h
+++ b/deltaq_amd/csrc/dq_round0_plan.h
@@ -330,6 +330,14 @@
     return at > 0 && n >= at ? 0 : kEarlyPasses;
 }
 
+inline bool text_in_place_wanted(int64_t n, bool device_text_aligned, int64_t min_view_n, const Flags &F)
+{
+    if (!device_text_aligned || n < min_view_n) return false;
+    if (F.text_in_place) return *F.text_in_place != 0;
+    const int64_t at = slots_cut_min_n();
+    return at > 0 && n >= at;
+}
+
 inline bool fused_ties_wanted(int64_t n, KeyPlan k, const Flags &F)
 {
     return k.packed && k.kb >= 2 && n >= kRound0MinN && !F.no_fused_ties && !F.sparse;
diff --git a/deltaq_amd/csrc/dq_sa_kernels.h b/deltaq_amd/csrc/dq_sa_kernels.h
--- a/deltaq_amd/csrc/dq_sa_kernels.h
+++ b/deltaq_amd/csrc/dq_sa_kernels.h
@@ -1,5 +1,7 @@
 #pragma once
 #include <stdint.h>
+
+#include "dq_text_view.h"
 
 #if defined(__HIPCC__)
 #define DQ_HD __host__ __device__
@@ -9,17 +11,21 @@
 
 namespace dq {
 
-template <int kMaxLen>
-DQ_HD inline int suffix_window_compare(const uint8_t *text, int64_t n, int64_t h, int64_t a, int64_t b)
+DQ_HD inline const uint8_t *text_window(const uint8_t *text, int64_t p, int) { return text + p; }
+DQ_HD inline const uint8_t *text_window(const TextView &text, int64_t p, int len) { return text.window(p, len); }
+
+template <int kMaxLen, typename Text>
+DQ_HD inline int suffix_window_compare(const Text &text, int64_t n, int64_t h, int64_t a, int64_t b)
 {
     static_assert(kMaxLen % 8 == 0, "whole words");
     typedef uint64_t u64_any __attribute__((aligned(1), may_alias));
     const int64_t pa = a + h, pb = b + h;
+    const uint8_t *ta = text_window(text, pa, kMaxLen), *tb = text_window(text, pb, kMaxLen);
     uint64_t wa[kMaxLen / 8], wbv[kMaxLen / 8];
 #pragma unroll
     for (int k = 0; k < kMaxLen / 8; ++k) {
-        wa[k] = *reinterpret_cast<const u64_any *>(text + pa + 8 * k);
-        wbv[k] = *reinterpret_cast<const u64_any *>(text + pb + 8 * k);
+        wa[k] = *reinterpret_cast<const u64_any *>(ta + 8 * k);
+        wbv[k] = *reinterpret_cast<const u64_any *>(tb + 8 * k);
     }
     int d = kMaxLen;
     bool a_less = false;
diff --git a/deltaq_amd/csrc/dq_slot_finish_plan.h b/deltaq_amd/csrc/dq_slot_finish_plan.h
--- a/deltaq_amd/csrc/dq_slot_finish_plan.h
+++ b/deltaq_amd/csrc/dq_slot_finish_plan.h
@@ -25,6 +25,19 @@
 DQ_HD inline uint32_t sf_key(uint32_t unique) { return unique >> kBktArrBits; }
 DQ_HD inline uint32_t sf_arrival(uint32_t unique) { return (unique & ((1u << kBktArrBits) - 1)) - 1; }
 DQ_HD inline bool sf_same_bin(uint32_t a, uint32_t b, int shift) { return ((a ^ b) >> (shift + kBktArrBits)) == 0; }
+
+struct SlotHalves { uint32_t hi; uint16_t lo; };
+DQ_HD inline bool slot_split_applies(int ib, int lowbits) { return ib >= 1 && ib <= 31 && lowbits >= 1 && lowbits <= 16 + 32 - ib; }
+DQ_HD inline SlotHalves slot_split_pack(uint64_t word, int ib, int lowbits)
+{
+    const uint32_t key = (uint32_t)(word >> ib) & (uint32_t)((1ull << lowbits) - 1);
+    const uint32_t imask = (uint32_t)((1ull << ib) - 1);
+    return SlotHalves{((uint32_t)word & imask) | (uint32_t)((uint64_t)(key >> 16) << ib), (uint16_t)(key & 0xffffu)};
+}
+DQ_HD inline uint32_t slot_split_key(uint32_t hi, uint32_t lo, int ib) { return ((hi >> ib) << 16) | lo; }
+DQ_HD inline uint32_t slot_split_suf(uint32_t hi, int ib) { return hi & (uint32_t)((1ull << ib) - 1); }
+DQ_HD inline uint64_t slot_split_lo_at(uint32_t end) { return ((uint64_t)end * 4 + 15) & ~(uint64_t)15; }
+DQ_HD inline bool slot_split_fits(uint32_t end) { return slot_split_lo_at(end) + (uint64_t)end * 2 <= (uint64_t)end * 8; }
 
 DQ_HD inline void sf_left(uint32_t mine, uint32_t other, uint32_t &fin, uint32_t &tie)
 {
diff --git a/deltaq_amd/csrc/dq_slot_rank.h b/deltaq_amd/csrc/dq_slot_rank.h
--- a/deltaq_amd/csrc/dq_slot_rank.h
+++ b/deltaq_amd/csrc/dq_slot_rank.h
@@ -1,6 +1,7 @@
 #pragma once
 #include "dq_bucket_sort.h"
 #include "dq_xcd_rank.h"
+#include "dq_slot_finish_plan.h"
 
 namespace dq {
 
@@ -35,7 +36,7 @@
     slot_plan_body(blockIdx.x, bytehist, X, slot_base);
 }
 
-static __global__ __launch_bounds__(kBlock) void slot_setup_kernel(const int64_t *__restrict__ bytehist, const uint8_t *__restrict__ text,
+static __global__ __launch_bounds__(kBlock) void slot_setup_kernel(const int64_t *__restrict__ bytehist, const TextView text,
                                                             int64_t n, int places, int64_t *__restrict__ digit_offset,
                                                             const int64_t *__restrict__ xcd_hist, int64_t *__restrict__ sub_offset,
                                                             int64_t X, uint32_t *__restrict__ slot_base )
@@ -84,9 +85,10 @@
 constexpr int kSlotRankItems = 12;
 constexpr int kSlotTileN = kSlotRankThreads * kSlotRankItems;
 
+template <bool kSplit>
 static __global__ __launch_bounds__(kSlotRankThreads, 1) void slot_rank_kernel(
     const uint64_t *__restrict__ kin , uint64_t *__restrict__ wout, int64_t n,
-    int shift , int bshift ,
+    int shift , int bshift , int ib ,
     const int64_t *__restrict__ region , const uint32_t *__restrict__ slot_base ,
     SlotRankCtl *__restrict__ ctl, BucketFlags *__restrict__ flags)
 {
@@ -231,11 +233,27 @@
 #pragma unroll
         for (int k = 0; k < kItems; ++k) key[k] = exch[k * kThreads + tid];
 
-#pragma unroll
-        for (int k = 0; k < kItems; ++k) {
-            const uint32_t q = (uint32_t)(k * kThreads + tid);
-            const uint32_t d = digit_of(key[k], shift);
-            if (q < valid && q < glim[d]) wout[gofs[d] + q] = key[k];
+        if constexpr (kSplit) {
+            uint32_t *__restrict__ H = reinterpret_cast<uint32_t *>(wout);
+            uint16_t *__restrict__ Lo = reinterpret_cast<uint16_t *>(reinterpret_cast<uint8_t *>(wout) + slot_split_lo_at(slot_base[kSlotBuckets]));
+#pragma unroll
+            for (int k = 0; k < kItems; ++k) {
+                const uint32_t q = (uint32_t)(k * kThreads + tid);
+                const uint32_t d = digit_of(key[k], shift);
+                const SlotHalves h = slot_split_pack(key[k], ib, bshift - ib);
+                if (q < valid && q < glim[d]) {
+                    const uint32_t at = gofs[d] + q;
+                    H[at] = h.hi;
+                    Lo[at] = h.lo;
+                }
+            }
+        } else {
+#pragma unroll
+            for (int k = 0; k < kItems; ++k) {
+                const uint32_t q = (uint32_t)(k * kThreads + tid);
+                const uint32_t d = digit_of(key[k], shift);
+                if (q < valid && q < glim[d]) wout[gofs[d] + q] = key[k];
+            }
         }
         DQ_SLOT_PHASE(3);
         lo = next_lo;
diff --git a/deltaq_amd/csrc/dq_sorter_impl.h b/deltaq_amd/csrc/dq_sorter_impl.h
--- a/deltaq_amd/csrc/dq_sorter_impl.h
+++ b/deltaq_amd/csrc/dq_sorter_impl.h
@@ -531,6 +531,7 @@
 
     int64_t twin_half = 0;
     const uint8_t *text_src = nullptr;
+    bool text_missing = false;
     int period_hint = 0;
     int twin_pairs_step(bool *done)
     {
@@ -582,7 +583,8 @@
         t_sort_info = {};
         HIP_TRY(hipMemsetAsync(w.totals, 0, 64, st));
         Round0Out<IdxT> r0;
-        int rc = Round0<IdxT>{c, st, w, n, d_sa, L, text_src, period_hint, r0}.run();
+        Round0<IdxT> round0{c, st, w, n, d_sa, L, text_src, period_hint, r0, text_missing};
+        int rc = round0.run();
         if (rc != DQ_OK) return rc;
         adopt(r0);
         t_sort_info.initial_active = m;
@@ -594,6 +596,10 @@
         bool sparse = m * 6 <= n || shallow_ties;
         if (F.sparse) sparse = *F.sparse != 0;
         if (keys_ready || list_ungrouped || first_rank32) sparse = false;
+        if (!(sparse && fin_done && fin_left == 0)) {
+            rc = round0.need_text("the doubling rounds read it");
+            if (rc != DQ_OK) return rc;
+        }
         if (sparse) rc = finish_sparse();
         else if (!r0.dense_built) rc = build_isa(Kr[rcur], Vr[rcur], m);
         if (rc != DQ_OK) return rc;
diff --git a/deltaq_amd/csrc/dq_text_view.h b/deltaq_amd/csrc/dq_text_view.h
--- /dev/null
+++ b/deltaq_amd/csrc/dq_text_view.h
@@ -0,0 +1,43 @@
+#pragma once
+#include <cstdint>
+
+#if defined(__HIPCC__)
+#define DQ_HD __host__ __device__
+#else
+#define DQ_HD
+#endif
+
+namespace dq {
+
+constexpr int kTextLoadMax = 16;
+constexpr int kTextTailLead = 32;
+constexpr int kTextTailBytes = kTextTailLead + 96;
+constexpr int64_t kTextViewMinN = 128;
+
+DQ_HD inline int64_t text_tail_start(int64_t n) { return (n - 16) & ~(int64_t)15; }
+
+struct TextView {
+    const uint8_t *lo;
+    const uint8_t *hi;
+    int64_t t0, n;
+    DQ_HD const uint8_t *at(int64_t p) const { return (p < t0 ? lo : hi) + p; }
+    DQ_HD const uint8_t *window(int64_t p, int len) const { return (p + len <= t0 ? lo : hi) + p; }
+};
+
+DQ_HD inline TextView text_in_place(const uint8_t *src, const uint8_t *tail, int64_t n)
+{
+    const int64_t t0 = text_tail_start(n);
+    return TextView{src, tail + ((int64_t)kTextTailLead - t0), t0, n};
+}
+DQ_HD inline TextView text_copied(const uint8_t *text, int64_t n)
+{
+    return TextView{text, text, n, n};
+}
+
+DQ_HD inline uint8_t text_tail_byte(const uint8_t *text, int64_t n, int i)
+{
+    const int64_t p = text_tail_start(n) - kTextTailLead + i;
+    return p >= 0 && p < n ? text[p] : (uint8_t)0;
+}
+
+}
diff --git a/deltaq_amd/csrc/dq_ties.h b/deltaq_amd/csrc/dq_ties.h
--- a/deltaq_amd/csrc/dq_ties.h
+++ b/deltaq_amd/csrc/dq_ties.h
@@ -140,9 +140,10 @@
 constexpr int kSettleWords = 8;
 constexpr int kSettleQueue = 256;
 constexpr int kSettleMaxG = 8, kSettleLen = 32;
+static_assert(kSettleLen <= kTextTailLead, "a comparison's window is placed as a whole (TextView::window)");
 
 template <typename IdxT>
-__device__ __forceinline__ bool settle_group(IdxT *SA, const uint8_t *__restrict__ text, int64_t n, int64_t h, int64_t head, int g, bool *bad)
+__device__ __forceinline__ bool settle_group(IdxT *SA, const TextView &text, int64_t n, int64_t h, int64_t head, int g, bool *bad)
 {
     uint32_t place = 0;
     bool decided = true;
@@ -170,7 +171,7 @@
 
 template <typename IdxT>
 __global__ __launch_bounds__(kSettleThreads, 6) void tie_settle_kernel(
-    const uint64_t *__restrict__ ebits, int64_t nwords, int64_t n, IdxT *SA, const uint8_t *__restrict__ text, int64_t h,
+    const uint64_t *__restrict__ ebits, int64_t nwords, int64_t n, IdxT *SA, const TextView text , int64_t h,
     uint64_t *__restrict__ list_rank, IdxT *__restrict__ list_suf, int64_t list_cap ,
     TieCounters *__restrict__ ctr , unsigned long long *__restrict__ list_count )
 {
diff --git a/deltaq_amd/csrc/dq_xcd_rank.h b/deltaq_amd/csrc/dq_xcd_rank.h
--- a/deltaq_amd/csrc/dq_xcd_rank.h
+++ b/deltaq_amd/csrc/dq_xcd_rank.h
@@ -20,7 +20,7 @@
 static_assert(kXcdRankThreads * kXcdRankItems == kXcdTileN, "the eighths are cut in tiles of this pass");
 
 static __global__ __launch_bounds__(kXcdRankThreads, 1) void xcd_text_rank_kernel(
-    const uint32_t *__restrict__ t32 , uint64_t *__restrict__ kout, int64_t n,
+    const TextView text , uint64_t *__restrict__ kout, int64_t n,
     int shift, int keybits, int ib, const int64_t *__restrict__ sub_offset , XcdRankCtl *__restrict__ ctl)
 {
     constexpr int kThreads = kXcdRankThreads, kItems = kXcdRankItems, kTileN = kXcdTileN;
@@ -73,7 +73,10 @@
 #pragma unroll
         for (int j = 0; j < kItems / 4; ++j) {
             const int64_t e0 = base + (int64_t)(j * kThreads + tid) * 4;
-            if (e0 < n) { nw[j][0] = t32[e0 >> 2]; nw[j][1] = t32[(e0 >> 2) + 1]; nw[j][2] = t32[(e0 >> 2) + 2]; }
+            if (e0 < n) {
+                const uint32_t *t32 = reinterpret_cast<const uint32_t *>(text.at(e0));
+                nw[j][0] = t32[0]; nw[j][1] = t32[1]; nw[j][2] = t32[2];
+            }
         }
     };
     load_text(tile);
```

After: 107,500 MB/s, median of 6. 1.5% higher.
